# OFA-Sys/OFASys

Hardware: AMD Instinct MI355X
Metric: multimodal tokens/sec (enc+dec train step) (higher is better)
Workload: dtype bf16

## Files before the change

include/ofasys_amd.h:

```cpp
#ifndef OFASYS_AMD_H
#define OFASYS_AMD_H

#include <stdint.h>

#ifdef __cplusplus
extern "C" {
#endif

typedef enum { OFA_F32 = 0, OFA_BF16 = 1, OFA_F16 = 2 } ofa_dtype;

enum {
  OFA_OK = 0,
  OFA_ERR_INVALID = 1,
  OFA_ERR_UNSUPPORTED = 2,
  OFA_ERR_LAUNCH = 3
};

enum {
  OFA_GEMM_BIAS_COL = 1,
  OFA_GEMM_BIAS_ROW = 2,
  OFA_GEMM_ACCUM = 4,
  OFA_GEMM_FORCE_SIMPLE = 8,
  OFA_GEMM_OUT_F32 = 16,
  OFA_GEMM_A_KPAD_ZERO = 32,
  OFA_GEMM_NO_LDS_DMA = 64,
  OFA_GEMM_DEFER_REDUCE = 128
};

int ofa_version(void);
const char* ofa_last_error(void);

int ofa_layernorm_fwd(const void* x, const void* gamma, const void* beta, void* y, float* mean, float* rstd,
                      int64_t rows, int cols, float eps, int dtype, void* stream);
int ofa_layernorm_bwd_ws_rows(void);
int ofa_layernorm_bwd(const void* dy, const void* x, const void* gamma, const float* mean, const float* rstd,
                      const void* dres, void* dx, void* dgamma, void* dbeta, float* ws, int64_t rows, int cols,
                      int accumulate, int dtype, void* stream);
int ofa_gelu_layernorm_fwd(const void* h, const void* gamma, const void* beta, void* y, float* mean, float* rstd,
                           int64_t rows, int cols, float eps, int dtype, void* stream);
int ofa_gelu_layernorm_bwd(const void* dy, const void* h, const void* gamma, const float* mean, const float* rstd,
                           void* dh, void* dgamma, void* dbeta, void* dbias, float* ws, int64_t rows, int cols,
                           int accumulate, int dtype, void* stream);

int64_t ofa_join_keep_bytes(int64_t rows, int cols, int dtype);
int ofa_join_fwd(const void* x, const void* residual, const void* gamma_a, const void* beta_a, const void* gamma_b,
                 const void* beta_b, void* y, void* z, float* stats, uint8_t* keep_bits, int64_t rows, int cols, float eps, float p,
                 uint64_t seed, uint64_t offset, const int64_t* offset_base, int dtype, void* stream);
int ofa_join_bwd_slots(int64_t rows, int cols, int dtype);
int ofa_join_bwd(const void* dy, const void* dz, const void* x, const void* y, const void* gamma_a, const void* gamma_b,
                 const float* stats, const uint8_t* keep_bits, void* dres, void* dx, float* ws, int64_t rows, int cols, float p,
                 uint64_t seed, uint64_t offset, const int64_t* offset_base, int want_dx_colsum, int dtype, void* stream);

int ofa_gemm(const void* A, const void* B, void* C, const void* bias, int M, int N, int K, int transA, int transB,
             int64_t lda, int64_t ldb, int64_t ldc, int batch, int64_t strideA, int64_t strideB, int64_t strideC,
             int batch_inner, int64_t strideA2, int64_t strideB2, int64_t strideC2,
             float alpha, int flags, int dtype, void* ws, int64_t ws_bytes, void* stream);

int ofa_gemm_colstat(const void* A, const void* B, void* C, const void* bias, int M, int N, int K, int transA, int transB,
                     int64_t lda, int64_t ldb, int64_t ldc, float alpha, int flags, int dtype, void* ws, int64_t ws_bytes,
                     double* partial, int max_groups, int* groups, void* stream);

typedef struct ofa_gemm_group_item {
  const void* a;
  const void* b;
  float* slabs;
  int64_t lda, ldb;
  int32_t m, n, k;
  int32_t splits;
  void* out;
  int64_t ldo;
  float out_alpha;
} ofa_gemm_group_item;
int ofa_gemm_group_plan(ofa_gemm_group_item* items, int n, int dtype);
int ofa_gemm_group_tn(const ofa_gemm_group_item* items, int n, int dtype, void* stream);

int ofa_scaled_softmax_fwd(const void* x, void* y, float scale, int b, int np, int sq, int sk, int dtype, void* stream);
int ofa_scaled_softmax_bwd(const void* dy, const void* y, void* dx, float scale, int b, int np, int sq, int sk,
                           int dtype, void* stream);
int ofa_scaled_masked_softmax_fwd(const void* x, const uint8_t* mask, void* y, float scale, int b, int np, int sq,
                                  int sk, int mask_b, int dtype, void* stream);
int ofa_scaled_masked_softmax_bwd(const void* dy, const void* y, void* dx, float scale, int b, int np, int sq, int sk,
                                  int dtype, void* stream);
int ofa_scaled_upper_triang_masked_softmax_fwd(const void* x, void* y, float scale, int attn_batches, int sq,
                                               int dtype, void* stream);
int ofa_scaled_upper_triang_masked_softmax_bwd(const void* dy, const void* y, void* dx, float scale, int attn_batches,
                                               int sq, int dtype, void* stream);
int ofa_get_batch_per_block(int sq, int sk, int b, int np);

int ofa_attn_softmax_fwd(const void* x, const void* bias, const uint8_t* kpm, void* p, float scale, int BA, int heads,
                         int T, int S, int causal, int dtype, void* stream);

int ofa_attn_fwd(const void* q, const void* k, const void* v, const void* bias, const uint8_t* kpm,
                 const void* c_attn, int c_attn_dtype, void* out, float* lse, int B, int heads, int T, int S, int Tpad,
                 int64_t ldq, int64_t ldk, int64_t ldo, float scale, int causal, const int32_t* seg, int rows_q, int rows_k,
                 int dtype, void* stream);
int ofa_attn_bwd_prep(const void* dout, const void* out, float* delta, int B, int heads, int T, int Tpad, int64_t ldo,
                      int dtype, void* stream);
int ofa_attn_bwd(const void* q, const void* k, const void* v, const void* dout, const void* bias, const uint8_t* kpm,
                 const void* c_attn, int c_attn_dtype, const float* lse, float* delta, const void* out, void* dq, void* dk,
                 void* dv, void* dbias, int B, int heads, int T, int S, int Tpad, int64_t ldq, int64_t ldk, int64_t ldo,
                 float scale, int causal, const int32_t* seg, int rows_q, int rows_k, int dtype, void* stream);

int ofa_attn_cs_slots(int B, int rows);
int ofa_attn_bwd_cs(const void* q, const void* k, const void* v, const void* dout, const void* bias, const uint8_t* kpm,
                    const void* c_attn, int c_attn_dtype, const float* lse, float* delta, const void* out, void* dq, void* dk,
                    void* dv, void* dbias, int B, int heads, int T, int S, int Tpad, int64_t ldq, int64_t ldk, int64_t ldo,
                    float scale, int causal, const int32_t* seg, int rows_q, int rows_k, int dtype, float* cs_q, int64_t cs_ldq,
                    float* cs_k, float* cs_v, int64_t cs_ldk, float* cs_c, void* stream);

int ofa_attn_sbias_fwd(const void* q, const void* k, const void* v, const void* bias_swz_row, int Tb, int Sb, const uint8_t* kpm,
                       const void* c_attn, int c_attn_dtype, void* out, float* lse, int B, int heads, int T, int S, int Tpad,
                       int64_t ldq, int64_t ldk, int64_t ldo, float scale, int causal, const int32_t* seg, int rows_q, int rows_k,
                       int dtype, void* stream);
int ofa_attn_sbias_bwd(const void* q, const void* k, const void* v, const void* dout, const void* bias, const void* bias_swz_row,
                       const void* bias_swz_col, int Tb, int Sb, const uint8_t* kpm, const void* c_attn, int c_attn_dtype,
                       const float* lse, float* delta, const void* out, void* dq, void* dk, void* dv, void* dbias_sum, int dbias_dtype,
                       float* ws, int64_t ws_bytes, int B, int heads, int T, int S, int Tpad, int64_t ldq, int64_t ldk, int64_t ldo, float scale,
                       int causal, const int32_t* seg, int rows_q, int rows_k, int dtype, void* stream);
int ofa_attn_sbias_bwd_cs(const void* q, const void* k, const void* v, const void* dout, const void* bias, const void* bias_swz_row,
                          const void* bias_swz_col, int Tb, int Sb, const uint8_t* kpm, const void* c_attn, int c_attn_dtype,
                          const float* lse, float* delta, const void* out, void* dq, void* dk, void* dv, void* dbias_sum, int dbias_dtype,
                          float* ws, int64_t ws_bytes, int B, int heads, int T, int S, int Tpad, int64_t ldq, int64_t ldk, int64_t ldo, float scale,
                          int causal, const int32_t* seg, int rows_q, int rows_k, int dtype, float* cs_q, int64_t cs_ldq, float* cs_k,
                          float* cs_v, int64_t cs_ldk, float* cs_c, void* stream);
int ofa_attn_sbias_chunks(int B, int heads, int Tb, int Sb);
int ofa_c_attn_grad(const float* delta, const void* c_attn, void* dc, int B, int heads, int T, int64_t ld, int accumulate,
                    int c_attn_dtype, void* stream);
int ofa_attn_decode(const void* q, const void* k, const void* v, const void* bias, const uint8_t* kpm, const void* c_attn,
                    int c_attn_dtype, void* out, void* probs, int B, int heads, int head_dim, int S, int64_t ldk,
                    int64_t k_batch_stride, int64_t kpm_ld, float scale, int dtype, void* stream);
int ofa_mean_heads(const void* p, void* out, int B, int heads, int64_t n, int dtype, void* stream);
int ofa_transpose_heads(const void* x, void* xt, int B, int T, int C, int Tpad, int64_t ld, int dtype, void* stream);

int ofa_gather_rows(const void* src, const int64_t* index, void* out, int64_t n, int D, int64_t src_rows, int dtype,
                    void* stream);
int ofa_gather_rows_parts(const void* const* srcs, const int* lens, int nparts, const int64_t* index, void* out, int64_t n, int D,
                          int64_t batch, int dtype, void* stream);
int ofa_scatter_rows_part(const void* src, const int64_t* inverse, void* out, int64_t batch, int nk, int Ttot, int start, int D,
                          int64_t src_rows, int dtype, void* stream);
int ofa_embedding_fwd(const void* weight, const int64_t* ids, void* out, int64_t n, int D, int64_t V, uint8_t* is_pad, int64_t pad_id,
                      int dtype, void* stream);
int ofa_segment_rowsum(const void* dout, const int32_t* order, const int32_t* seg_off, const int32_t* seg_row, void* dweight, int nseg,
                       int D, int accumulate, int dtype, void* stream);
int ofa_embedding_bwd_slices(int64_t V, int D);
int ofa_embedding_bwd(const void* dout, const int64_t* ids, void* dweight, int64_t n, int D, int64_t V,
                      int64_t padding_idx, uint8_t* present_ws, float* slice_ws, int dtype, void* stream);

int ofa_gelu_fwd(const void* x, void* y, int64_t n, int dtype, void* stream);
int ofa_gelu_bwd(const void* dy, const void* x, void* dx, int64_t n, int dtype, void* stream);
int ofa_dropout_add_fwd(const void* x, const void* residual, void* y, int64_t n, float p, uint64_t seed,
                        uint64_t offset, const int64_t* offset_base, int dtype, void* stream);
int ofa_dropout_bwd(const void* dy, void* dx, int64_t n, float p, uint64_t seed, uint64_t offset,
                    const int64_t* offset_base, int dtype, void* stream);
int ofa_add_rowvec_mask(const void* a, const void* b, const void* vec, const uint8_t* rowmask, void* y, int64_t rows,
                        int cols, int64_t b_period, int dtype, void* stream);
int ofa_batch_sum(const void* x, void* out, int batch, int64_t n, int accumulate, int dtype, void* stream);

int ofa_colsum_ws_floats(int cols);
int ofa_colsum(const void* x, void* out, float* ws, int64_t rows, int cols, int64_t ld, float alpha, int accumulate,
               int dtype, int out_dtype, void* stream);

int ofa_add_n(const void* const* inputs, int n, void* out, int64_t numel, int dtype, void* stream);
int ofa_mul(const void* a, const void* b, void* y, int64_t rows, int cols, int b_rowvec, int dtype, void* stream);
int ofa_scale_row_groups(const void* x, const float* scale, void* y, int64_t rows, int cols, int64_t group, int dtype,
                         void* stream);
int ofa_reduce_sum_f32(const float* x, float* out, int64_t n, void* stream);
int ofa_head_sum_f32(const float* x, float* out, int B, int heads, int T, int ld, void* stream);

typedef struct ofa_bias_slots {
  const void* values[8];
  const void* values2[8];
  int32_t start[8];
  int32_t n[8];
  int32_t inner[8];
  int32_t count;
} ofa_bias_slots;
int64_t ofa_bias_swz_elems(int heads, int Tb, int Sb);
int ofa_bias_build(const void* abs_bias, const ofa_bias_slots* slots, void* out, void* swz_row, void* swz_col, int heads, int Tb,
                   int Sb, int dtype, void* stream);
int ofa_bias_outer_grad(const void* dbias, void* d_frames, void* d_patches, int heads, int T, int start, int F, int P, int dtype,
                        void* stream);
int ofa_bias_block_add(void* bias, const void* values, int B, int A, int T, int start, int n, int dtype, void* stream);
int ofa_bias_block_grad(const void* dbias, void* dvalues, int B, int A, int T, int start, int n, int dtype, void* stream);
int ofa_bias_block_add_batch(void* bias, const void* values, int B, int A, int T, int start, int n, int dtype, void* stream);
int ofa_bias_block_slice(const void* dbias, void* dvalues, int B, int A, int T, int start, int n, int dtype, void* stream);

int ofa_im2col_patch(const void* img, void* col, int B, int C, int H, int W, int p, int Kpad, int lead, int dtype, void* stream);

int ofa_cross_entropy_fwd(const void* logits, const int64_t* target, float* lse, float* row_loss, int64_t rows,
                          int64_t V, int64_t ld, int64_t ignore_index, int dtype, void* stream);
int ofa_cross_entropy_fwd_grad_ok(int64_t V, int64_t ld, int dtype);
int ofa_cross_entropy_fwd_grad(const void* logits, const int64_t* target, const float* grad_scale, float* lse, float* row_loss,
                               void* dlogits, int64_t rows, int64_t V, int64_t ld, int64_t ignore_index, int dtype, void* stream);
int ofa_cross_entropy_bwd(const void* logits, const int64_t* target, const float* lse, const float* grad_scale,
                          void* dlogits, int64_t rows, int64_t V, int64_t ld, int64_t ignore_index, int dtype,
                          void* stream);

int ofa_ls_cross_entropy_fwd(const void* logits, const int64_t* target, float* lse, float* row_loss, float* row_nll,
                             float* row_cnt, int64_t rows, int64_t V, int64_t ld, int64_t ignore_index, float eps,
                             int64_t cstart, int64_t cend, const uint8_t* cmask, int dtype, void* stream);
int ofa_ls_cross_entropy_bwd(const void* logits, const int64_t* target, const float* lse, const float* row_cnt,
                             const float* row_w, const float* grad_scale, void* dlogits, int64_t rows, int64_t V, int64_t ld,
                             int64_t ignore_index, float eps, int64_t cstart, int64_t cend, const uint8_t* cmask, int dtype,
                             void* stream);
int ofa_probs_fwd(const void* logits, float* out, int64_t rows, int64_t V, int64_t ld, int log_probs, int dtype,
                  void* stream);
int ofa_probs_bwd(const float* dy, const float* y, void* dlogits, int64_t rows, int64_t V, int64_t ld, int log_probs,
                  int dtype, void* stream);

int ofa_sumsq_ws_floats(void);
int ofa_sumsq(const void* x, float* out , float* ws ,
              int64_t n, int dtype, void* stream);
int ofa_step_schedule(const float* gsq, const double* sample_size, double* step, const double* lr, float* sched,
                      float* gnorm, float clip_norm, double beta1, double beta2, void* stream);
int ofa_step_stats_add(double* stats, const float* loss, const int64_t* target, int64_t n, int64_t pad, void* stream);
int ofa_step_schedule_scaled(const float* gsq, const double* sample_size, double* step, const double* lr, float* sched,
                             float* gnorm, double* loss_scaler, float clip_norm, double beta1, double beta2, double scale_factor,
                             double scale_window, double tolerance, double threshold, double min_loss_scale, void* stream);
int ofa_adam_step(float* master, float* exp_avg, float* exp_avg_sq, const void* grad, void* model_param,
                  const float* coef, int64_t n, float lr, float beta1, float beta2, float eps, float weight_decay,
                  int step, int dtype, void* stream);

int ofa_conv_out_size(int in, int k, int stride, int pad);
int ofa_im2col(const void* x, void* col, int B, int H, int W, int C, int KH, int KW, int stride, int pad, int Kpad,
               int x_nchw, int dtype, void* stream);
int ofa_col2im(const void* dcol, void* dx, int B, int H, int W, int C, int KH, int KW, int stride, int pad, int Kpad,
               int dtype, void* stream);
int ofa_batchnorm_ws_floats(int C);
int ofa_batchnorm_fwd(const void* x, const void* gamma, const void* beta, const void* residual, void* y, float* mean,
                      float* rstd, float* running_mean, float* running_var, float* ws, int64_t rows, int C, float eps,
                      float momentum, int use_running, int relu, int dtype, void* stream);
int ofa_batchnorm_bwd(const void* dy, const void* y, const void* x, const void* gamma, const float* mean, const float* rstd,
                      void* dx, void* dres, void* dgamma, void* dbeta, float* ws, int64_t rows, int C, int batch_stats,
                      int relu, int accumulate, const void* beta, int dtype, void* stream);
int ofa_batchnorm_fwd_stats(const void* x, double* sums, float* ws, int64_t rows, int C, int dtype, void* stream);
int ofa_batchnorm_fwd_apply(const void* x, const void* gamma, const void* beta, const void* residual, void* y, float* mean,
                            float* rstd, float* running_mean, float* running_var, const double* sums, int groups, int64_t rows,
                            int C, float eps, float momentum, int relu, int dtype, void* stream);
int ofa_batchnorm_bwd_stats(const void* dy, const void* y, const void* x, const void* gamma, const float* mean, const float* rstd,
                            float* sums, void* dgamma, void* dbeta, float* ws, int64_t rows, int C, int relu, int accumulate,
                            const void* beta, int dtype, void* stream);
int ofa_batchnorm_bwd_dx(const void* dy, const void* y, const void* x, const void* gamma, const float* mean, const float* rstd,
                         const float* sums, void* dx, void* dres, int64_t rows, const double* total_rows, int C, int relu,
                         const void* beta, int dtype, void* stream);
int ofa_maxpool_fwd(const void* x, void* y, uint8_t* arg, int B, int H, int W, int C, int K, int stride, int pad, int dtype,
                    void* stream);
int ofa_maxpool_bwd(const void* dy, const uint8_t* arg, void* dx, int B, int H, int W, int C, int K, int stride, int pad,
                    int dtype, void* stream);
int ofa_relu(const void* x, const void* gate, void* y, int64_t n, int dtype, void* stream);

typedef struct ofa_fold_job {
  const float* part;
  void* out;
  int64_t cols;
  int64_t stride;
  int32_t nslots;
  int32_t accumulate;
  float alpha;
  int32_t out_dtype;
} ofa_fold_job;
int ofa_fold_batched(const ofa_fold_job* jobs, int njobs, void* stream);
typedef struct ofa_copy_job {
  const void* src;
  void* dst;
  int64_t bytes;
} ofa_copy_job;
int ofa_copy_batched(const ofa_copy_job* jobs, int njobs, void* stream);
#define OFA_DEFER_FOLD 2
int ofa_layernorm_bwd_slots(int64_t rows, int cols, int dtype, int gelu);
int ofa_colsum_slots(int64_t rows);
int ofa_gemm_splits(int M, int N, int K, int transA, int transB, int batch, int flags, int dtype, int64_t ws_bytes);
enum {
  OFA_GEMM_PLAN_KERNEL = 0,
  OFA_GEMM_PLAN_SIMPLE_WHY,
  OFA_GEMM_PLAN_WAVES_M,
  OFA_GEMM_PLAN_WAVES_N,
  OFA_GEMM_PLAN_WAVE_TM,
  OFA_GEMM_PLAN_WAVE_TN,
  OFA_GEMM_PLAN_TILE_M,
  OFA_GEMM_PLAN_TILE_N,
  OFA_GEMM_PLAN_SPLITS,
  OFA_GEMM_PLAN_KSPLIT,
  OFA_GEMM_PLAN_K,
  OFA_GEMM_PLAN_MIXED_TALL,
  OFA_GEMM_PLAN_MIXED_SHORT,
  OFA_GEMM_PLAN_COLSTAT_ROWS,
  OFA_GEMM_PLAN_REDUCE,
  OFA_GEMM_PLAN_LEN
};
enum {
  OFA_GEMM_KERNEL_SIMPLE = 0,
  OFA_GEMM_KERNEL_REG = 1,
  OFA_GEMM_KERNEL_LDS_DMA = 2,
  OFA_GEMM_KERNEL_RING = 3,
  OFA_GEMM_KERNEL_BIG = 4,
  OFA_GEMM_KERNEL_PP = 5,
  OFA_GEMM_KERNEL_MIXED = 6
};
int ofa_gemm_plan(int M, int N, int K, int transA, int transB, int batch, int flags, int dtype, int64_t ws_bytes, int* plan);

int64_t ofa_beam_ws_bytes(int rows, int V, int K);
int ofa_beam_topk(const void* logits, int64_t ld, int rows, int V, int K, float temperature, int cstart, int cend, int step,
                  int min_len, int max_len, int pad, int unk, int eos, float unk_penalty, int ngram, const int64_t* tokens,
                  int64_t tok_ld, const int* done, void* ws, int dtype, void* stream);
int ofa_beam_select(const void* ws, int bsz, int K, int V, int step, int max_len, int eos, int unk, float unk_penalty,
                    int normalize, float len_penalty, int64_t* tokens, int64_t tok_ld, int tok_cap, float* scores,
                    int64_t score_ld, int* ignore, int* done, int* nfin, int64_t* reorder, int64_t* fin_tok, float* fin_pos,
                    int64_t fin_ld, float* fin_score, int* fin_len, int* fin_cnt, void* stream);

int64_t ofa_closed_set_ws_bytes(int bsz, int E, int N);
int ofa_closed_set_edge_logits(const void* h, int64_t ld_h, int dtype, const void* W, int64_t ld_w, const void* bias, int D, int V,
                               int bsz, int chunk, int T, int c0, const int* items, int n_items, const int* edge_token,
                               const int* rep_ans, const int* rep_pos, int N, int E, void* ws, void* stream);
int ofa_closed_set_reduce(int bsz, int C, int N, int E, int P, const int* node_edge_off, const int* edge_node, const int* path_off,
                          const int* path_edge, void* ws, float* scores, void* stream);
int ofa_closed_set_score(const void* h, int64_t ld_h, int dtype, const void* W, int64_t ld_w, const void* bias, int D, int V,
                         int bsz, int C, int Tmax, int N, int E, int P, const int* items, int n_items, const int* node_edge_off,
                         const int* edge_token, const int* edge_node, const int* rep_ans, const int* rep_pos, const int* path_off,
                         const int* path_edge, void* ws, float* scores, void* stream);

int ofa_trie_beam_splits(int max_degree, int V);
int ofa_trie_beam_topk(const void* h, int64_t ld_h, int dtype, const void* W, int64_t ld_w, const void* bias, int D, int V,
                       int rows, int K, const int* node, const int* node_edge_off, const int* edge_token, int N, int E,
                       int max_degree, float temperature, int step, int min_len, int max_len, int pad, int unk, int eos,
                       float unk_penalty, int ngram, const int64_t* tokens, int64_t tok_ld, const int* done, void* ws,
                       void* stream);
int ofa_trie_beam_advance(int* node, const int* node_edge_off, const int* edge_token, const int* edge_child, int N, int E,
                          int bsz, int K, int step, const int64_t* tokens, int64_t tok_ld, int tok_cap, const float* scores,
                          int64_t score_ld, const int* ignore, const int64_t* reorder, int* done, int* nfin, void* stream);

#ifdef __cplusplus
}
#endif
#endif
```

ofasys_amd/adaptor/image_patch_embed.py:

```python
from dataclasses import dataclass, field

import torch
import torch.nn as nn

from .. import ops
from ..configure import register_config
from ..module import Embedding
from ..preprocessor import Dictionary, ModalityType, Slot
from .base import AdaptorOutput, BaseAdaptor, BaseAdaptorConfig


@dataclass
class ImagePatchEmbedAdaptorConfig(BaseAdaptorConfig):
    image_size_width: int = 224
    image_size_height: int = 224
    patch_size_width: int = 14
    patch_size_height: int = 14
    embed_dim: int = 768
    add_cls_token: bool = True


@register_config("ofasys.adaptor", "image_patch_embed", ImagePatchEmbedAdaptorConfig)
class ImagePatchEmbedAdaptor(BaseAdaptor):
    pos_batch_invariant = True

    def __init__(self, embed_tokens: Embedding, dictionary: Dictionary, is_src: bool, general_adaptor,
                 cfg: ImagePatchEmbedAdaptorConfig):
        super().__init__(embed_tokens, dictionary, is_src, general_adaptor, cfg)
        image_size = (cfg.image_size_height, cfg.image_size_width)
        patch_size = (cfg.patch_size_height, cfg.patch_size_width)
        assert patch_size[0] == patch_size[1], "square patches only"
        num_patches = (image_size[1] // patch_size[1]) * (image_size[0] // patch_size[0])
        self.image_size, self.patch_size, self.num_patches = image_size, patch_size, num_patches
        self.embed_image_positions = Embedding(num_patches + 1 if cfg.add_cls_token else num_patches, cfg.embed_dim)
        if cfg.add_cls_token:
            self.cls_token = nn.Parameter(torch.zeros(1, 1, cfg.embed_dim))
        self.proj = nn.Conv2d(3, cfg.embed_dim, kernel_size=patch_size, stride=patch_size)

    def _ofa_plain_conv_weights(self):
        return (self.proj.weight,)

    def forward(self, slot: Slot, **kwargs) -> AdaptorOutput:
        assert slot.modality == ModalityType.IMAGE
        image: torch.Tensor = slot.value
        batch_size, _, height, width = image.shape
        assert height == self.image_size[0] and width == self.image_size[1], \
            f"Input image size ({height}*{width}) doesn't match model ({self.image_size[0]}*{self.image_size[1]})."
        x = ops.patch_embed(image, self.proj.weight, self.proj.bias, self.patch_size[0],
                            cls_token=self.cls_token if self.cfg.add_cls_token else None)
        n = x.size(1)
        mask = ops.cached_index(self, ("nomask", batch_size, n), lambda: torch.zeros((batch_size, n), dtype=torch.bool, device=image.device))
        pos = ops.cached_index(self, ("arange", n), lambda: torch.arange(n, dtype=torch.long, device=image.device).unsqueeze(0))
        return AdaptorOutput(x, mask, self.embed_image_positions(pos).expand(batch_size, -1, -1), None)
```

ofasys_amd/adaptor/text.py:

```python
import math
from dataclasses import dataclass, field
from typing import Any, Dict, Optional

import torch
import torch.nn as nn
from torch import Tensor

from .. import ops
from ..configure import register_config
from ..module import Embedding, OfaLinear
from ..preprocessor import Dictionary, Slot
from .base import AdaptorOutput, BaseAdaptor, BaseAdaptorConfig


def make_token_bucket_position(bucket_size, max_position):
    mid = bucket_size // 2
    dist = torch.arange(max_position, dtype=torch.long)
    band = torch.ceil(torch.log(dist.clamp_min(1) / mid) / math.log((max_position - 1) / mid) * (mid - 1)).long()
    magnitude = torch.where(dist <= mid, dist, mid + band)
    rel = dist[:, None] - dist[None, :]
    return torch.sign(rel) * magnitude[rel.abs()] + (bucket_size - 1)


@dataclass
class TextAdaptorConfig(BaseAdaptorConfig):
    token_bucket_size: int = field(default=256, metadata={"help": "token bucket size"})
    share_input_output_embed: bool = True
    output_embed_dim: Optional[int] = 512
    output_dim: Optional[int] = None
    output_bias: bool = False


@register_config("ofasys.adaptor", "text", TextAdaptorConfig)
class TextAdaptor(BaseAdaptor):
    pos_batch_invariant = True

    def __init__(self, embed_tokens: Embedding, dictionary: Dictionary, is_src: bool, general_adaptor,
                 cfg: TextAdaptorConfig):
        super().__init__(embed_tokens, dictionary, is_src, general_adaptor, cfg)
        self.embed_positions = Embedding(cfg.max_position + 2, cfg.embed_dim)
        token_num_rel_dis = 2 * cfg.token_bucket_size - 1
        token_rp_bucket = make_token_bucket_position(cfg.token_bucket_size, cfg.max_position)
        num_rel_pos_tables = 1 if self.cfg.share_attn_bias else self.num_layers
        self.token_rel_pos_table_list = nn.ModuleList(
            [Embedding(token_num_rel_dis, cfg.num_attention_heads, zero_init=True) for _ in range(num_rel_pos_tables)])
        self.register_buffer("token_rp_bucket", token_rp_bucket)
        self.share_input_output_embed = bool(cfg.share_input_output_embed)
        self.output_dim = cfg.output_dim if cfg.output_dim is not None else len(dictionary)
        self.output_embed_dim = cfg.output_embed_dim
        self.output_embed_bias = cfg.output_bias
        self.output_projection = None
        self.build_output_projection(dictionary)

    def build_output_projection(self, dictionary):
        if self.share_input_output_embed:
            self.output_projection = self.embed_tokens_T
        else:
            self.output_projection = OfaLinear(self.output_embed_dim, self.output_dim, bias=self.output_embed_bias)
            nn.init.normal_(self.output_projection.weight, mean=0, std=self.output_embed_dim ** -0.5)

    def get_rel_pos_bias(self, batch_size, seq_length, idx, **kwargs):
        if seq_length > self.token_rp_bucket.size(0):
            raise ValueError(f"sequence length {seq_length} exceeds the {self.token_rp_bucket.size(0)} positions of token_rp_bucket")
        rp_bucket = ops.cached_index(self, ("text", seq_length), lambda: self.token_rp_bucket[:seq_length, :seq_length].contiguous())
        return ops.embedding(rp_bucket, self.token_rel_pos_table_list[idx].weight, plan_key=("text", ops.owner_token(self)))

    def forward(self, slot: Slot, **kwargs) -> AdaptorOutput:
        src_tokens = slot.value
        bsz, seq_len = src_tokens.shape
        pad = self.dictionary.pad()
        if pad is not None and src_tokens.is_cuda:
            token_embedding, padding_masks = self.embed_tokens_and_pad_mask(src_tokens, pad)
        else:
            token_embedding = self.embed_tokens(src_tokens)
            padding_masks = src_tokens.eq(pad) if pad is not None else torch.zeros_like(src_tokens, dtype=torch.bool)
        positions = ops.cached_index(self, ("arange", seq_len), lambda: torch.arange(seq_len, device=src_tokens.device).unsqueeze(0))
        pos_embed = self.embed_positions(positions).expand(bsz, -1, -1)
        return AdaptorOutput(token_embedding, padding_masks, pos_embed, [])

    def forward_output(self, x: Tensor, extra: Dict[str, Any], slot: Slot, **kwargs):
        return self.output_projection(x), extra
```

ofasys_amd/csrc/elementwise.hip:

```cpp
#include "common.h"

namespace ofa {

template <typename T, bool BWD>
__global__ __launch_bounds__(256) void gelu_kernel(const T* __restrict__ dy, const T* __restrict__ x, T* __restrict__ y,
                                                   int64_t nvec, int64_t n) {
  constexpr int N = Vec<T>::N;
  for (int64_t v = (int64_t)blockIdx.x * 256 + threadIdx.x; v < nvec; v += (int64_t)gridDim.x * 256) {
    float a[N], g[N], o[N];
    load_vec<T>(x + v * N, a);
    if (BWD) load_vec<T>(dy + v * N, g);
#pragma unroll
    for (int j = 0; j < N; ++j) o[j] = BWD ? g[j] * gelu_grad_f(a[j]) : gelu_f(a[j]);
    store_vec<T>(y + v * N, o);
  }
  if (blockIdx.x == 0) {
    for (int64_t e = nvec * N + threadIdx.x; e < n; e += 256) {
      const float a = ld1<T>(x + e);
      st1<T>(y + e, BWD ? ld1<T>(dy + e) * gelu_grad_f(a) : gelu_f(a));
    }
  }
}

template <typename T, bool ADD>
__global__ __launch_bounds__(256) void dropout_kernel(const T* __restrict__ x, const T* __restrict__ res, T* __restrict__ y,
                                                      int64_t n, float p, uint64_t seed, uint64_t offset,
                                                      const int64_t* __restrict__ offset_base) {
  if (offset_base) offset += (uint64_t)offset_base[0];
  const Philox rng(seed);
  const float keep_scale = 1.0f / (1.0f - p);
  const uint32_t thresh = philox_thresh(p);
  const int64_t nq = (n + 7) / 8;
  for (int64_t q = (int64_t)blockIdx.x * 256 + threadIdx.x; q < nq; q += (int64_t)gridDim.x * 256) {
    const uint4 r = rng(offset + (uint64_t)q);
#pragma unroll
    for (int j = 0; j < 8; ++j) {
      const int64_t e = q * 8 + j;
      if (e < n) {
        float v = philox_keep(r, j, thresh) ? ld1<T>(x + e) * keep_scale : 0.f;
        if (ADD) v += ld1<T>(res + e);
        st1<T>(y + e, v);
      }
    }
  }
}

template <typename T>
__global__ __launch_bounds__(256) void add_rowvec_mask_kernel(const T* __restrict__ a, const T* __restrict__ b,
                                                              const T* __restrict__ vec, const uint8_t* __restrict__ rowmask,
                                                              T* __restrict__ y, int64_t rows, int cols, int64_t b_period) {
  constexpr int N = Vec<T>::N;
  const int vpr = cols / N;
  const int64_t total = rows * vpr;
  for (int64_t v = (int64_t)blockIdx.x * 256 + threadIdx.x; v < total; v += (int64_t)gridDim.x * 256) {
    const int64_t r = v / vpr;
    const int c = (int)(v % vpr) * N;
    float x[N], t[N];
    load_vec<T>(a + r * cols + c, x);
    if (b) {
      load_vec<T>(b + (b_period ? r % b_period : r) * cols + c, t);
#pragma unroll
      for (int j = 0; j < N; ++j) x[j] += t[j];
    }
    if (vec) {
      load_vec<T>(vec + c, t);
#pragma unroll
      for (int j = 0; j < N; ++j) x[j] += t[j];
    }
    if (rowmask && rowmask[r]) {
#pragma unroll
      for (int j = 0; j < N; ++j) x[j] = 0.f;
    }
    store_vec<T>(y + r * cols + c, x);
  }
}

template <typename T>
__global__ __launch_bounds__(256) void embedding_fwd_kernel(const T* __restrict__ w, const int64_t* __restrict__ ids,
                                                            T* __restrict__ out, int64_t n, int D, int64_t V,
                                                            uint8_t* __restrict__ is_pad, int64_t pad_id) {
  constexpr int N = Vec<T>::N;
  const int vpr = D / N;
  const int64_t total = n * vpr;
  for (int64_t v = (int64_t)blockIdx.x * 256 + threadIdx.x; v < total; v += (int64_t)gridDim.x * 256) {
    const int64_t r = v / vpr;
    const int c = (int)(v % vpr) * N;
    int64_t id = ids[r];
    if (is_pad && c == 0) is_pad[r] = id == pad_id;
    id = id < 0 ? 0 : (id >= V ? V - 1 : id);
    *reinterpret_cast<typename Vec<T>::type*>(out + r * D + c) =
        *reinterpret_cast<const typename Vec<T>::type*>(w + id * D + c);
  }
}

template <typename T>
__global__ __launch_bounds__(256) void gather_rows_kernel(const T* __restrict__ src, const int64_t* __restrict__ index,
                                                          T* __restrict__ out, int64_t n, int D, int64_t src_rows) {
  constexpr int N = Vec<T>::N;
  const int vpr = D / N;
  const int64_t total = n * vpr;
  for (int64_t v = (int64_t)blockIdx.x * 256 + threadIdx.x; v < total; v += (int64_t)gridDim.x * 256) {
    const int64_t r = v / vpr;
    const int c = (int)(v % vpr) * N;
    const int64_t id = index[r];
    typename Vec<T>::type val = {};
    if (id >= 0 && id < src_rows) val = *reinterpret_cast<const typename Vec<T>::type*>(src + id * D + c);
    *reinterpret_cast<typename Vec<T>::type*>(out + r * D + c) = val;
  }
}

struct GatherParts { const void* src[8]; int start[9]; int n; };
template <typename T>
__global__ __launch_bounds__(256) void gather_rows_parts_kernel(GatherParts gp, const int64_t* __restrict__ index, T* __restrict__ out,
                                                                int64_t n, int D, int Ttot, int64_t batch) {
  constexpr int N = Vec<T>::N;
  const int vpr = D / N;
  const int64_t total = n * vpr;
  for (int64_t v = (int64_t)blockIdx.x * 256 + threadIdx.x; v < total; v += (int64_t)gridDim.x * 256) {
    const int64_t r = v / vpr;
    const int c = (int)(v % vpr) * N;
    const int64_t id = index[r];
    typename Vec<T>::type val = {};
    if (id >= 0 && id < batch * Ttot) {
      const int64_t b = id / Ttot;
      const int t = (int)(id - b * Ttot);
      int k = 0;
#pragma unroll
      for (int q = 1; q < 8; ++q)
        if (q < gp.n && t >= gp.start[q]) k = q;
      const int nk = gp.start[k + 1] - gp.start[k];
      val = *reinterpret_cast<const typename Vec<T>::type*>((const T*)gp.src[k] + ((b * nk + (t - gp.start[k])) * D + c));
    }
    *reinterpret_cast<typename Vec<T>::type*>(out + r * D + c) = val;
  }
}

template <typename T>
__global__ __launch_bounds__(256) void scatter_rows_part_kernel(const T* __restrict__ src, const int64_t* __restrict__ inverse,
                                                                T* __restrict__ out, int64_t batch, int nk, int Ttot, int start, int D,
                                                                int64_t src_rows) {
  constexpr int N = Vec<T>::N;
  const int vpr = D / N;
  const int64_t total = batch * nk * vpr;
  for (int64_t v = (int64_t)blockIdx.x * 256 + threadIdx.x; v < total; v += (int64_t)gridDim.x * 256) {
    const int64_t r = v / vpr;
    const int c = (int)(v % vpr) * N;
    const int64_t b = r / nk;
    const int j = (int)(r - b * nk);
    const int64_t id = inverse[b * Ttot + start + j];
    typename Vec<T>::type val = {};
    if (id >= 0 && id < src_rows) val = *reinterpret_cast<const typename Vec<T>::type*>(src + id * D + c);
    *reinterpret_cast<typename Vec<T>::type*>(out + r * D + c) = val;
  }
}

template <typename T>
__global__ __launch_bounds__(256) void embedding_fwd_scalar_kernel(const T* __restrict__ w, const int64_t* __restrict__ ids,
                                                                   T* __restrict__ out, int64_t n, int D, int64_t V) {
  const int64_t total = n * D;
  for (int64_t e = (int64_t)blockIdx.x * 256 + threadIdx.x; e < total; e += (int64_t)gridDim.x * 256) {
    const int64_t r = e / D;
    const int c = (int)(e % D);
    int64_t id = ids[r];
    id = id < 0 ? 0 : (id >= V ? V - 1 : id);
    out[e] = w[id * D + c];
  }
}

__global__ __launch_bounds__(256) void embedding_mark_kernel(const int64_t* __restrict__ ids, uint8_t* __restrict__ present,
                                                             int64_t n, int64_t V) {
  for (int64_t i = (int64_t)blockIdx.x * 256 + threadIdx.x; i < n; i += (int64_t)gridDim.x * 256) {
    const int64_t id = ids[i];
    if (id >= 0 && id < V) present[id] = 1;
  }
}

template <typename T, int NV>
__global__ __launch_bounds__(256) void embedding_bwd_kernel(const T* __restrict__ dout, const int64_t* __restrict__ ids,
                                                            T* __restrict__ dw, float* __restrict__ part, int64_t n, int D,
                                                            int64_t V, int64_t padding_idx,
                                                            const uint8_t* __restrict__ present, int S) {
  constexpr int N = Vec<T>::N;
  const int lane = threadIdx.x & 63;
  const int64_t v = (int64_t)blockIdx.x * 4 + (threadIdx.x >> 6);
  const int sl = blockIdx.y;
  if (v >= V || v == padding_idx) return;
  if (present && !present[v]) return;
  float acc[NV][N];
#pragma unroll
  for (int i = 0; i < NV; ++i)
#pragma unroll
    for (int j = 0; j < N; ++j) acc[i][j] = 0.f;
  const int64_t per = ((n + S - 1) / S + 63) / 64 * 64;
  const int64_t lo = sl * per, hi = lo + per < n ? lo + per : n;
  bool any = false;
  for (int64_t base = lo; base < hi; base += 64) {
    const int64_t idx = base + lane;
    const bool hit = idx < hi && ids[idx] == v;
    unsigned long long m = __ballot(hit);
    while (m) {
      const int src = __ffsll((long long)m) - 1;
      m &= m - 1;
      any = true;
      const T* row = dout + (base + src) * D;
#pragma unroll
      for (int i = 0; i < NV; ++i) {
        const int c = (i * 64 + lane) * N;
        if (c < D) {
          float x[N];
          load_vec<T>(row + c, x);
#pragma unroll
          for (int j = 0; j < N; ++j) acc[i][j] += x[j];
        }
      }
    }
  }
  if (S == 1) {
    if (!any) return;
    T* wr = dw + v * D;
#pragma unroll
    for (int i = 0; i < NV; ++i) {
      const int c = (i * 64 + lane) * N;
      if (c < D) {
        float o[N];
        load_vec<T>(wr + c, o);
#pragma unroll
        for (int j = 0; j < N; ++j) o[j] += acc[i][j];
        store_vec<T>(wr + c, o);
      }
    }
  } else {
    float* pr = part + ((int64_t)sl * V + v) * D;
#pragma unroll
    for (int i = 0; i < NV; ++i) {
      const int c = (i * 64 + lane) * N;
      if (c < D)
#pragma unroll
        for (int j = 0; j < N; ++j) pr[c + j] = acc[i][j];
    }
  }
}

template <typename T>
__global__ __launch_bounds__(256) void embedding_bwd_scalar_kernel(const T* __restrict__ dout, const int64_t* __restrict__ ids,
                                                                   T* __restrict__ dw, float* __restrict__ part, int64_t n,
                                                                   int D, int64_t V, int64_t padding_idx,
                                                                   const uint8_t* __restrict__ present, int S) {
  const int lane = threadIdx.x & 63;
  const int64_t v = (int64_t)blockIdx.x * 4 + (threadIdx.x >> 6);
  const int sl = blockIdx.y;
  if (v >= V || v == padding_idx) return;
  if (present && !present[v]) return;
  constexpr int MAXC = 32;
  float acc[MAXC];
#pragma unroll
  for (int j = 0; j < MAXC; ++j) acc[j] = 0.f;
  const int64_t per = ((n + S - 1) / S + 63) / 64 * 64;
  const int64_t lo = sl * per, hi = lo + per < n ? lo + per : n;
  bool any = false;
  for (int64_t base = lo; base < hi; base += 64) {
    const int64_t idx = base + lane;
    const bool hit = idx < hi && ids[idx] == v;
    unsigned long long m = __ballot(hit);
    while (m) {
      const int src = __ffsll((long long)m) - 1;
      m &= m - 1;
      any = true;
      const T* row = dout + (base + src) * D;
#pragma unroll
      for (int j = 0; j < MAXC; ++j) {
        const int c = j * 64 + lane;
        if (c < D) acc[j] += ld1<T>(row + c);
      }
    }
  }
  if (S == 1 && !any) return;
#pragma unroll
  for (int j = 0; j < MAXC; ++j) {
    const int c = j * 64 + lane;
    if (c < D) {
      if (S == 1) st1<T>(dw + v * D + c, ld1<T>(dw + v * D + c) + acc[j]);
      else part[((int64_t)sl * V + v) * D + c] = acc[j];
    }
  }
}

template <typename T>
__global__ __launch_bounds__(256) void embedding_fold_kernel(const float* __restrict__ part, T* __restrict__ dw, int D,
                                                             int64_t V, int64_t padding_idx,
                                                             const uint8_t* __restrict__ present, int S) {
  const int64_t v = blockIdx.x;
  if (v == padding_idx || (present && !present[v])) return;
  for (int c = threadIdx.x; c < D; c += 256) {
    float a = 0.f;
    for (int s = 0; s < S; ++s) a += part[((int64_t)s * V + v) * D + c];
    st1<T>(dw + v * D + c, ld1<T>(dw + v * D + c) + a);
  }
}

template <typename T>
__global__ __launch_bounds__(256) void im2col_patch_kernel(const T* __restrict__ img, T* __restrict__ col, int B, int C, int H,
                                                           int W, int p, int Kpad, int lead) {
  const int nph = H / p, npw = W / p, K = C * p * p;
  const int64_t per = (int64_t)lead + (int64_t)nph * npw;
  const int64_t total = (int64_t)B * per * Kpad;
  for (int64_t e = (int64_t)blockIdx.x * 256 + threadIdx.x; e < total; e += (int64_t)gridDim.x * 256) {
    const int k = (int)(e % Kpad);
    const int64_t r = e / Kpad;
    const int64_t b = r / per, rs = r % per - lead;
    float v = 0.f;
    if (k < K && rs >= 0) {
      const int j = k % p, i = (k / p) % p, c = k / (p * p);
      const int pw = (int)(rs % npw), ph = (int)(rs / npw);
      v = ld1<T>(img + ((b * C + c) * H + ph * p + i) * W + pw * p + j);
    }
    st1<T>(col + e, v);
  }
}

template <typename T>
__global__ __launch_bounds__(256) void colsum_partial_kernel(const T* __restrict__ x, float* __restrict__ partial,
                                                             int64_t rows, int cols, int64_t ld) {
  constexpr int N = Vec<T>::N;
  __shared__ float red[8][32][N];
  const int cx = threadIdx.x & 31, ry = threadIdx.x >> 5;
  const int c = (blockIdx.x * 32 + cx) * N;
  float acc[N];
#pragma unroll
  for (int j = 0; j < N; ++j) acc[j] = 0.f;
  if (c < cols) {
    for (int64_t r = (int64_t)blockIdx.y * 8 + ry; r < rows; r += (int64_t)gridDim.y * 8) {
      float v[N];
      load_vec<T>(x + r * ld + c, v);
#pragma unroll
      for (int j = 0; j < N; ++j) acc[j] += v[j];
    }
  }
#pragma unroll
  for (int j = 0; j < N; ++j) red[ry][cx][j] = acc[j];
  __syncthreads();
  if (ry == 0 && c < cols) {
#pragma unroll
    for (int j = 0; j < N; ++j) {
      float t = 0.f;
#pragma unroll
      for (int r = 0; r < 8; ++r) t += red[r][cx][j];
      partial[(int64_t)blockIdx.y * cols + c + j] = t;
    }
  }
}
template <typename TO>
__global__ __launch_bounds__(1024) void colsum_final_kernel(const float* __restrict__ partial, TO* __restrict__ out,
                                                            int cols, int groups, float alpha, int accumulate) {
  __shared__ float sm[16][64];
  const int cx = threadIdx.x & 63, ry = threadIdx.x >> 6;
  const int c = blockIdx.x * 64 + cx;
  float s = 0.f;
  if (c < cols)
    for (int g = ry; g < groups; g += 16) s += partial[(int64_t)g * cols + c];
  sm[ry][cx] = s;
  __syncthreads();
  if (ry == 0 && c < cols) {
    float t = 0.f;
#pragma unroll
    for (int r = 0; r < 16; ++r) t += sm[r][cx];
    t *= alpha;
    if (accumulate) t += ld1<TO>(out + c);
    st1<TO>(out + c, t);
  }
}

static inline int grid_for(int64_t work) {
  int64_t g = (work + 255) / 256;
  return (int)(g < 1 ? 1 : (g > 2048 ? 2048 : g));
}

}
using namespace ofa;

#define OFA_DT_CHECK(name) OFA_REQUIRE(OFA_DT_OK(dtype), OFA_ERR_INVALID, name ": bad dtype %d", dtype)

extern "C" int ofa_gelu_fwd(const void* x, void* y, int64_t n, int dtype, void* stream) {
  OFA_DT_CHECK("gelu_fwd");
  OFA_REQUIRE(n >= 0 && (n == 0 || (x && y)), OFA_ERR_INVALID, "gelu_fwd: bad argument");
  if (n == 0) return 0;
  hipStream_t st = (hipStream_t)stream;
  if (dtype == OFA_F32)
    hipLaunchKernelGGL((gelu_kernel<float, false>), dim3(grid_for(n / 4)), dim3(256), 0, st, (const float*)nullptr,
                       (const float*)x, (float*)y, n / 4, n);
  else if (dtype == OFA_BF16)
    hipLaunchKernelGGL((gelu_kernel<bf16_t, false>), dim3(grid_for(n / 8)), dim3(256), 0, st, (const bf16_t*)nullptr,
                       (const bf16_t*)x, (bf16_t*)y, n / 8, n);
  else
    hipLaunchKernelGGL((gelu_kernel<f16_t, false>), dim3(grid_for(n / 8)), dim3(256), 0, st, (const f16_t*)nullptr,
                       (const f16_t*)x, (f16_t*)y, n / 8, n);
  return check_launch("gelu_fwd");
}

extern "C" int ofa_gelu_bwd(const void* dy, const void* x, void* dx, int64_t n, int dtype, void* stream) {
  OFA_DT_CHECK("gelu_bwd");
  OFA_REQUIRE(n >= 0 && (n == 0 || (dy && x && dx)), OFA_ERR_INVALID, "gelu_bwd: bad argument");
  if (n == 0) return 0;
  hipStream_t st = (hipStream_t)stream;
  if (dtype == OFA_F32)
    hipLaunchKernelGGL((gelu_kernel<float, true>), dim3(grid_for(n / 4)), dim3(256), 0, st, (const float*)dy,
                       (const float*)x, (float*)dx, n / 4, n);
  else if (dtype == OFA_BF16)
    hipLaunchKernelGGL((gelu_kernel<bf16_t, true>), dim3(grid_for(n / 8)), dim3(256), 0, st, (const bf16_t*)dy,
                       (const bf16_t*)x, (bf16_t*)dx, n / 8, n);
  else
    hipLaunchKernelGGL((gelu_kernel<f16_t, true>), dim3(grid_for(n / 8)), dim3(256), 0, st, (const f16_t*)dy,
                       (const f16_t*)x, (f16_t*)dx, n / 8, n);
  return check_launch("gelu_bwd");
}

extern "C" int ofa_dropout_add_fwd(const void* x, const void* residual, void* y, int64_t n, float p, uint64_t seed,
                                   uint64_t offset, const int64_t* offset_base, int dtype, void* stream) {
  OFA_DT_CHECK("dropout_add_fwd");
  OFA_REQUIRE(n >= 0 && p >= 0.f && p < 1.f && (n == 0 || (x && y)), OFA_ERR_INVALID, "dropout_add_fwd: bad argument");
  if (n == 0) return 0;
  hipStream_t st = (hipStream_t)stream;
  dim3 grid(grid_for((n + 7) / 8)), block(256);
  if (dtype == OFA_F32) {
    if (residual) hipLaunchKernelGGL((dropout_kernel<float, true>), grid, block, 0, st, (const float*)x, (const float*)residual, (float*)y, n, p, seed, offset, offset_base);
    else hipLaunchKernelGGL((dropout_kernel<float, false>), grid, block, 0, st, (const float*)x, (const float*)nullptr, (float*)y, n, p, seed, offset, offset_base);
  } else if (dtype == OFA_BF16) {
    if (residual) hipLaunchKernelGGL((dropout_kernel<bf16_t, true>), grid, block, 0, st, (const bf16_t*)x, (const bf16_t*)residual, (bf16_t*)y, n, p, seed, offset, offset_base);
    else hipLaunchKernelGGL((dropout_kernel<bf16_t, false>), grid, block, 0, st, (const bf16_t*)x, (const bf16_t*)nullptr, (bf16_t*)y, n, p, seed, offset, offset_base);
  }
  else {
    if (residual) hipLaunchKernelGGL((dropout_kernel<f16_t, true>), grid, block, 0, st, (const f16_t*)x, (const f16_t*)residual, (f16_t*)y, n, p, seed, offset, offset_base);
    else hipLaunchKernelGGL((dropout_kernel<f16_t, false>), grid, block, 0, st, (const f16_t*)x, (const f16_t*)nullptr, (f16_t*)y, n, p, seed, offset, offset_base);
  }
  return check_launch("dropout_add_fwd");
}

extern "C" int ofa_dropout_bwd(const void* dy, void* dx, int64_t n, float p, uint64_t seed, uint64_t offset,
                               const int64_t* offset_base, int dtype, void* stream) {
  return ofa_dropout_add_fwd(dy, nullptr, dx, n, p, seed, offset, offset_base, dtype, stream);
}

extern "C" int ofa_add_rowvec_mask(const void* a, const void* b, const void* vec, const uint8_t* rowmask, void* y,
                                   int64_t rows, int cols, int64_t b_period, int dtype, void* stream) {
  OFA_DT_CHECK("add_rowvec_mask");
  OFA_REQUIRE(rows >= 0 && cols > 0 && a && y && b_period >= 0, OFA_ERR_INVALID, "add_rowvec_mask: bad argument");
  OFA_REQUIRE(cols % (dtype == OFA_F32 ? 4 : 8) == 0, OFA_ERR_UNSUPPORTED, "add_rowvec_mask: cols=%d not vectorizable", cols);
  if (rows == 0) return 0;
  hipStream_t st = (hipStream_t)stream;
  if (dtype == OFA_F32)
    hipLaunchKernelGGL((add_rowvec_mask_kernel<float>), dim3(grid_for(rows * cols / 4)), dim3(256), 0, st, (const float*)a,
                       (const float*)b, (const float*)vec, rowmask, (float*)y, rows, cols, b_period);
  else if (dtype == OFA_BF16)
    hipLaunchKernelGGL((add_rowvec_mask_kernel<bf16_t>), dim3(grid_for(rows * cols / 8)), dim3(256), 0, st,
                       (const bf16_t*)a, (const bf16_t*)b, (const bf16_t*)vec, rowmask, (bf16_t*)y, rows, cols, b_period);
  else
    hipLaunchKernelGGL((add_rowvec_mask_kernel<f16_t>), dim3(grid_for(rows * cols / 8)), dim3(256), 0, st,
                       (const f16_t*)a, (const f16_t*)b, (const f16_t*)vec, rowmask, (f16_t*)y, rows, cols, b_period);
  return check_launch("add_rowvec_mask");
}

extern "C" int ofa_embedding_fwd(const void* weight, const int64_t* ids, void* out, int64_t n, int D, int64_t V, uint8_t* is_pad,
                                 int64_t pad_id, int dtype, void* stream) {
  OFA_DT_CHECK("embedding_fwd");
  OFA_REQUIRE(!is_pad || D % (dtype == OFA_F32 ? 4 : 8) == 0, OFA_ERR_UNSUPPORTED, "embedding_fwd: the pad mask rides with the vector kernel (D = %d)", D);
  OFA_REQUIRE(n >= 0 && D > 0 && V > 0 && weight && ids && out, OFA_ERR_INVALID, "embedding_fwd: bad argument");
  if (n == 0) return 0;
  hipStream_t st = (hipStream_t)stream;
  if (D % (dtype == OFA_F32 ? 4 : 8) != 0) {
    if (dtype == OFA_F32)
// ... 54 lines not shown
      gp.start[k + 1] = gp.start[k] + lens[k];
    } else {
      gp.start[k + 1] = gp.start[k];
    }
  }
  const int Ttot = gp.start[nparts];
  hipStream_t st = (hipStream_t)stream;
  if (dtype == OFA_F32)
    hipLaunchKernelGGL((gather_rows_parts_kernel<float>), dim3(grid_for(n * D / 4)), dim3(256), 0, st, gp, index, (float*)out, n, D, Ttot, batch);
  else if (dtype == OFA_BF16)
    hipLaunchKernelGGL((gather_rows_parts_kernel<bf16_t>), dim3(grid_for(n * D / 8)), dim3(256), 0, st, gp, index, (bf16_t*)out, n, D, Ttot, batch);
  else
    hipLaunchKernelGGL((gather_rows_parts_kernel<f16_t>), dim3(grid_for(n * D / 8)), dim3(256), 0, st, gp, index, (f16_t*)out, n, D, Ttot, batch);
  return check_launch("gather_rows_parts");
}

extern "C" int ofa_scatter_rows_part(const void* src, const int64_t* inverse, void* out, int64_t batch, int nk, int Ttot, int start, int D,
                                     int64_t src_rows, int dtype, void* stream) {
  OFA_DT_CHECK("scatter_rows_part");
  OFA_REQUIRE(src && inverse && out && batch > 0 && nk > 0 && start >= 0 && start + nk <= Ttot && D > 0 && src_rows > 0, OFA_ERR_INVALID,
              "scatter_rows_part: bad argument");
  OFA_REQUIRE(D % (dtype == OFA_F32 ? 4 : 8) == 0, OFA_ERR_UNSUPPORTED, "scatter_rows_part: D=%d not vectorizable", D);
  hipStream_t st = (hipStream_t)stream;
  const int64_t work = batch * nk * D / (dtype == OFA_F32 ? 4 : 8);
  if (dtype == OFA_F32)
    hipLaunchKernelGGL((scatter_rows_part_kernel<float>), dim3(grid_for(work)), dim3(256), 0, st, (const float*)src, inverse, (float*)out, batch, nk, Ttot, start, D, src_rows);
  else if (dtype == OFA_BF16)
    hipLaunchKernelGGL((scatter_rows_part_kernel<bf16_t>), dim3(grid_for(work)), dim3(256), 0, st, (const bf16_t*)src, inverse, (bf16_t*)out, batch, nk, Ttot, start, D, src_rows);
  else
    hipLaunchKernelGGL((scatter_rows_part_kernel<f16_t>), dim3(grid_for(work)), dim3(256), 0, st, (const f16_t*)src, inverse, (f16_t*)out, batch, nk, Ttot, start, D, src_rows);
  return check_launch("scatter_rows_part");
}

template <typename T, int CPL>
__global__ __launch_bounds__(256) void segment_rowsum_kernel(const T* __restrict__ dout, const int* __restrict__ order,
                                                             const int* __restrict__ seg_off, const int* __restrict__ seg_row,
                                                             T* __restrict__ dw, int nseg, int D, int accumulate) {
  const int lane = threadIdx.x & 63;
  const int sg = blockIdx.x * 4 + (threadIdx.x >> 6);
  if (sg >= nseg) return;
  constexpr int G = 64 / CPL;
  const int g = lane / CPL, c = lane % CPL;
  const int lo = seg_off[sg], hi = seg_off[sg + 1];
  float acc = 0.f;
  int p = lo + g;
  for (; p + 3 * G < hi; p += 4 * G) {
    const int64_t r0 = order[p], r1 = order[p + G], r2 = order[p + 2 * G], r3 = order[p + 3 * G];
    float v0 = 0.f, v1 = 0.f, v2 = 0.f, v3 = 0.f;
    if (c < D) {
      v0 = ld1<T>(dout + r0 * D + c);
      v1 = ld1<T>(dout + r1 * D + c);
      v2 = ld1<T>(dout + r2 * D + c);
      v3 = ld1<T>(dout + r3 * D + c);
    }
    acc += (v0 + v1) + (v2 + v3);
  }
  for (; p < hi; p += G) {
    const int64_t row = order[p];
    if (c < D) acc += ld1<T>(dout + row * D + c);
  }
#pragma unroll
  for (int off = CPL; off < 64; off <<= 1) acc += __shfl_xor(acc, off);
  if (g == 0 && c < D) {
    T* o = dw + (int64_t)seg_row[sg] * D + c;
    st1<T>(o, (accumulate ? ld1<T>(o) : 0.f) + acc);
  }
}

extern "C" int ofa_embedding_bwd_slices(int64_t V, int D) {
  if (V <= 0 || D <= 0) return 1;
  const int64_t by_rows = 8192 / V;
  const int64_t by_bytes = ((int64_t)1 << 21) / (V * D);
  int64_t s = by_rows > by_bytes ? by_rows : by_bytes;
  return (int)(s < 1 ? 1 : (s > 64 ? 64 : s));
}

template <typename T>
static void launch_segment_rowsum(const void* dout, const int32_t* order, const int32_t* seg_off, const int32_t* seg_row, void* dw, int nseg,
                                  int D, int accumulate, hipStream_t st) {
  const dim3 grid(cdiv(nseg, 4)), block(256);
  if (D <= 8) hipLaunchKernelGGL((segment_rowsum_kernel<T, 8>), grid, block, 0, st, (const T*)dout, order, seg_off, seg_row, (T*)dw, nseg, D, accumulate);
  else if (D <= 16) hipLaunchKernelGGL((segment_rowsum_kernel<T, 16>), grid, block, 0, st, (const T*)dout, order, seg_off, seg_row, (T*)dw, nseg, D, accumulate);
  else if (D <= 32) hipLaunchKernelGGL((segment_rowsum_kernel<T, 32>), grid, block, 0, st, (const T*)dout, order, seg_off, seg_row, (T*)dw, nseg, D, accumulate);
  else hipLaunchKernelGGL((segment_rowsum_kernel<T, 64>), grid, block, 0, st, (const T*)dout, order, seg_off, seg_row, (T*)dw, nseg, D, accumulate);
}

extern "C" int ofa_segment_rowsum(const void* dout, const int32_t* order, const int32_t* seg_off, const int32_t* seg_row, void* dweight,
                                  int nseg, int D, int accumulate, int dtype, void* stream) {
  OFA_DT_CHECK("segment_rowsum");
  OFA_REQUIRE(dout && order && seg_off && seg_row && dweight && nseg >= 0 && D > 0 && D <= 64, OFA_ERR_INVALID,
              "segment_rowsum: bad argument (D = %d, at most 64 columns)", D);
  if (nseg == 0) return 0;
  hipStream_t st = (hipStream_t)stream;
  if (dtype == OFA_F32) launch_segment_rowsum<float>(dout, order, seg_off, seg_row, dweight, nseg, D, accumulate, st);
  else if (dtype == OFA_BF16) launch_segment_rowsum<bf16_t>(dout, order, seg_off, seg_row, dweight, nseg, D, accumulate, st);
  else launch_segment_rowsum<f16_t>(dout, order, seg_off, seg_row, dweight, nseg, D, accumulate, st);
  return check_launch("segment_rowsum");
}

extern "C" int ofa_embedding_bwd(const void* dout, const int64_t* ids, void* dweight, int64_t n, int D, int64_t V,
                                 int64_t padding_idx, uint8_t* present_ws, float* slice_ws, int dtype, void* stream) {
  OFA_DT_CHECK("embedding_bwd");
  OFA_REQUIRE(n >= 0 && D > 0 && V > 0 && dout && ids && dweight, OFA_ERR_INVALID, "embedding_bwd: bad argument");
  const int vecn = dtype == OFA_F32 ? 4 : 8;
  OFA_REQUIRE(D <= 2048, OFA_ERR_UNSUPPORTED, "embedding_bwd: D=%d exceeds 2048", D);
  const bool vec_ok = D % vecn == 0 && D <= 64 * vecn * 4 && (((uintptr_t)dout | (uintptr_t)dweight) & 15) == 0;
  if (n == 0) return 0;
  hipStream_t st = (hipStream_t)stream;
  if (present_ws) {
    (void)hipMemsetAsync(present_ws, 0, (size_t)V, st);
    hipLaunchKernelGGL(embedding_mark_kernel, dim3(grid_for(n)), dim3(256), 0, st, ids, present_ws, n, V);
  }
  const int S = slice_ws ? ofa_embedding_bwd_slices(V, D) : 1;
  const int nv = cdiv(D, 64 * vecn);
  dim3 grid((unsigned)((V + 3) / 4), S), block(256);
#define EMB_LAUNCH(T, NV)                                                                                               \
  hipLaunchKernelGGL((embedding_bwd_kernel<T, NV>), grid, block, 0, st, (const T*)dout, ids, (T*)dweight, slice_ws, n, D, V, \
                     padding_idx, (const uint8_t*)present_ws, S)
#define EMB_CASE(T)                  \
  do {                               \
    if (nv <= 1) EMB_LAUNCH(T, 1);   \
    else if (nv <= 2) EMB_LAUNCH(T, 2); \
    else EMB_LAUNCH(T, 4);           \
  } while (0)
  if (!vec_ok) {
    if (dtype == OFA_F32)
      hipLaunchKernelGGL((embedding_bwd_scalar_kernel<float>), grid, block, 0, st, (const float*)dout, ids, (float*)dweight,
                         slice_ws, n, D, V, padding_idx, (const uint8_t*)present_ws, S);
    else if (dtype == OFA_BF16)
      hipLaunchKernelGGL((embedding_bwd_scalar_kernel<bf16_t>), grid, block, 0, st, (const bf16_t*)dout, ids,
                         (bf16_t*)dweight, slice_ws, n, D, V, padding_idx, (const uint8_t*)present_ws, S);
    else
      hipLaunchKernelGGL((embedding_bwd_scalar_kernel<f16_t>), grid, block, 0, st, (const f16_t*)dout, ids,
                         (f16_t*)dweight, slice_ws, n, D, V, padding_idx, (const uint8_t*)present_ws, S);
  } else if (dtype == OFA_F32) EMB_CASE(float);
  else if (dtype == OFA_BF16) EMB_CASE(bf16_t);
         else EMB_CASE(f16_t);
#undef EMB_CASE
#undef EMB_LAUNCH
  int rc = check_launch("embedding_bwd");
  if (rc || S == 1) return rc;
  if (dtype == OFA_F32)
    hipLaunchKernelGGL((embedding_fold_kernel<float>), dim3((unsigned)V), dim3(256), 0, st, slice_ws, (float*)dweight, D, V,
                       padding_idx, (const uint8_t*)present_ws, S);
  else if (dtype == OFA_BF16)
    hipLaunchKernelGGL((embedding_fold_kernel<bf16_t>), dim3((unsigned)V), dim3(256), 0, st, slice_ws, (bf16_t*)dweight, D, V,
                       padding_idx, (const uint8_t*)present_ws, S);
  else
    hipLaunchKernelGGL((embedding_fold_kernel<f16_t>), dim3((unsigned)V), dim3(256), 0, st, slice_ws, (f16_t*)dweight, D, V,
                       padding_idx, (const uint8_t*)present_ws, S);
  return check_launch("embedding_fold");
}

extern "C" int ofa_im2col_patch(const void* img, void* col, int B, int C, int H, int W, int p, int Kpad, int lead, int dtype,
                                void* stream) {
  OFA_DT_CHECK("im2col_patch");
  OFA_REQUIRE(img && col && B > 0 && C > 0 && p > 0 && H % p == 0 && W % p == 0 && Kpad >= C * p * p && lead >= 0, OFA_ERR_INVALID,
              "im2col_patch: bad argument (H=%d W=%d p=%d Kpad=%d)", H, W, p, Kpad);
  hipStream_t st = (hipStream_t)stream;
  const int64_t total = (int64_t)B * (lead + (int64_t)(H / p) * (W / p)) * Kpad;
  if (dtype == OFA_F32)
    hipLaunchKernelGGL((im2col_patch_kernel<float>), dim3(grid_for(total)), dim3(256), 0, st, (const float*)img, (float*)col,
                       B, C, H, W, p, Kpad, lead);
  else if (dtype == OFA_BF16)
    hipLaunchKernelGGL((im2col_patch_kernel<bf16_t>), dim3(grid_for(total)), dim3(256), 0, st, (const bf16_t*)img,
                       (bf16_t*)col, B, C, H, W, p, Kpad, lead);
  else
    hipLaunchKernelGGL((im2col_patch_kernel<f16_t>), dim3(grid_for(total)), dim3(256), 0, st, (const f16_t*)img,
                       (f16_t*)col, B, C, H, W, p, Kpad, lead);
  return check_launch("im2col_patch");
}

extern "C" int ofa_colsum_ws_floats(int cols) { return 128 * cols; }

extern "C" int ofa_colsum_slots(int64_t rows) {
  int64_t groups = (rows + 63) / 64;
  return (int)(groups < 1 ? 1 : (groups > 128 ? 128 : groups));
}

extern "C" int ofa_colsum(const void* x, void* out, float* ws, int64_t rows, int cols, int64_t ld, float alpha,
                          int accumulate, int dtype, int out_dtype, void* stream) {
  OFA_DT_CHECK("colsum");
  OFA_REQUIRE(OFA_DT_OK(out_dtype), OFA_ERR_INVALID, "colsum: bad out dtype %d", out_dtype);
  OFA_REQUIRE(rows >= 0 && cols > 0 && ld >= cols && x && (out || accumulate == OFA_DEFER_FOLD) && ws, OFA_ERR_INVALID,
              "colsum: bad argument");
  const int n = dtype == OFA_F32 ? 4 : 8;
  OFA_REQUIRE(cols % n == 0 && ld % n == 0, OFA_ERR_UNSUPPORTED, "colsum: cols=%d / ld not vectorizable", cols);
  hipStream_t st = (hipStream_t)stream;
  const int groups = ofa_colsum_slots(rows);
  dim3 grid(cdiv(cols / n, 32), groups), block(256);
  if (dtype == OFA_F32)
    hipLaunchKernelGGL((colsum_partial_kernel<float>), grid, block, 0, st, (const float*)x, ws, rows, cols, ld);
  else if (dtype == OFA_BF16)
    hipLaunchKernelGGL((colsum_partial_kernel<bf16_t>), grid, block, 0, st, (const bf16_t*)x, ws, rows, cols, ld);
  else
    hipLaunchKernelGGL((colsum_partial_kernel<f16_t>), grid, block, 0, st, (const f16_t*)x, ws, rows, cols, ld);
  int rc = check_launch("colsum_partial");
  if (rc || accumulate == OFA_DEFER_FOLD) return rc;
  if (out_dtype == OFA_F32)
    hipLaunchKernelGGL((colsum_final_kernel<float>), dim3(cdiv(cols, 64)), dim3(1024), 0, st, (const float*)ws, (float*)out,
                       cols, groups, alpha, accumulate);
  else if (out_dtype == OFA_BF16)
    hipLaunchKernelGGL((colsum_final_kernel<bf16_t>), dim3(cdiv(cols, 64)), dim3(1024), 0, st, (const float*)ws,
                       (bf16_t*)out, cols, groups, alpha, accumulate);
  else
    hipLaunchKernelGGL((colsum_final_kernel<f16_t>), dim3(cdiv(cols, 64)), dim3(1024), 0, st, (const float*)ws,
                       (f16_t*)out, cols, groups, alpha, accumulate);
  return check_launch("colsum_final");
}

namespace ofa {
template <typename T>
__global__ __launch_bounds__(256) void mul_kernel(const T* __restrict__ a, const T* __restrict__ b, T* __restrict__ y,
                                                  int64_t rows, int cols, int b_rowvec) {
  constexpr int N = Vec<T>::N;
  const int vpr = cols / N;
  const int64_t total = rows * vpr;
  for (int64_t v = (int64_t)blockIdx.x * 256 + threadIdx.x; v < total; v += (int64_t)gridDim.x * 256) {
    const int64_t r = v / vpr;
    const int c = (int)(v % vpr) * N;
    float x[N], t[N];
    load_vec<T>(a + r * cols + c, x);
    load_vec<T>(b_rowvec ? b + c : b + r * cols + c, t);
#pragma unroll
    for (int j = 0; j < N; ++j) x[j] *= t[j];
    store_vec<T>(y + r * cols + c, x);
  }
}
template <typename T>
__global__ __launch_bounds__(256) void scale_row_groups_kernel(const T* __restrict__ x, const float* __restrict__ scale,
                                                               T* __restrict__ y, int64_t rows, int cols, int64_t group) {
  constexpr int N = Vec<T>::N;
  const int vpr = cols / N;
  const int64_t total = rows * vpr;
  for (int64_t v = (int64_t)blockIdx.x * 256 + threadIdx.x; v < total; v += (int64_t)gridDim.x * 256) {
    const int64_t r = v / vpr;
    const int c = (int)(v % vpr) * N;
    const float s = scale[r / group];
    float a[N];
    load_vec<T>(x + r * cols + c, a);
#pragma unroll
    for (int j = 0; j < N; ++j) a[j] *= s;
    store_vec<T>(y + r * cols + c, a);
  }
}
__global__ __launch_bounds__(256) void reduce_sum_f32_kernel(const float* __restrict__ x, float* __restrict__ out, int64_t n) {
  __shared__ float sw[4];
  float s = 0.f;
  for (int64_t i = threadIdx.x; i < n; i += 256) s += x[i];
  s = wave_sum(s);
  if ((threadIdx.x & 63) == 0) sw[threadIdx.x >> 6] = s;
  __syncthreads();
  if (threadIdx.x == 0) out[0] = sw[0] + sw[1] + sw[2] + sw[3];
}
__global__ __launch_bounds__(256) void head_sum_kernel(const float* __restrict__ x, float* __restrict__ out, int B, int heads,
                                                       int T, int ld) {
  __shared__ float sw[4];
  const int h = blockIdx.x;
  float s = 0.f;
  for (int b = 0; b < B; ++b)
    for (int t = threadIdx.x; t < T; t += 256) s += x[((int64_t)b * heads + h) * ld + t];
  s = wave_sum(s);
  if ((threadIdx.x & 63) == 0) sw[threadIdx.x >> 6] = s;
  __syncthreads();
  if (threadIdx.x == 0) out[h] = sw[0] + sw[1] + sw[2] + sw[3];
}
struct AddNArgs { const void* in[16]; int n; };
template <typename T>
__global__ __launch_bounds__(256) void add_n_kernel(AddNArgs a, T* __restrict__ out, int64_t numel) {
  constexpr int N = Vec<T>::N;
  const int64_t nvec = numel / N;
  for (int64_t v = (int64_t)blockIdx.x * 256 + threadIdx.x; v < nvec; v += (int64_t)gridDim.x * 256) {
    float acc[N];
#pragma unroll
    for (int j = 0; j < N; ++j) acc[j] = 0.f;
    for (int k = 0; k < a.n; ++k) {
      float t[N];
      load_vec<T>((const T*)a.in[k] + v * N, t);
#pragma unroll
      for (int j = 0; j < N; ++j) acc[j] += t[j];
    }
    store_vec<T>(out + v * N, acc);
  }
  if (blockIdx.x == 0) {
    for (int64_t i = nvec * N + threadIdx.x; i < numel; i += 256) {
      float t = 0.f;
      for (int k = 0; k < a.n; ++k) t += ld1<T>((const T*)a.in[k] + i);
      st1<T>(out + i, t);
    }
  }
}
}

extern "C" int ofa_add_n(const void* const* inputs, int n, void* out, int64_t numel, int dtype, void* stream) {
  OFA_DT_CHECK("add_n");
  OFA_REQUIRE(inputs && out && n >= 1 && n <= 16 && numel >= 0, OFA_ERR_INVALID, "add_n: 1..16 inputs (got %d)", n);
  if (numel == 0) return 0;
  AddNArgs a;
  for (int k = 0; k < 16; ++k) a.in[k] = inputs[k < n ? k : 0];
  for (int k = 0; k < n; ++k) OFA_REQUIRE(inputs[k] && !((uintptr_t)inputs[k] & 15), OFA_ERR_INVALID, "add_n: input %d is NULL or not 16-byte aligned", k);
  OFA_REQUIRE(!((uintptr_t)out & 15), OFA_ERR_INVALID, "add_n: out is not 16-byte aligned");
  a.n = n;
  hipStream_t st = (hipStream_t)stream;
  const int64_t work = numel / (dtype == OFA_F32 ? 4 : 8) + 1;
  if (dtype == OFA_F32) hipLaunchKernelGGL((add_n_kernel<float>), dim3(grid_for(work)), dim3(256), 0, st, a, (float*)out, numel);
  else if (dtype == OFA_BF16) hipLaunchKernelGGL((add_n_kernel<bf16_t>), dim3(grid_for(work)), dim3(256), 0, st, a, (bf16_t*)out, numel);
  else hipLaunchKernelGGL((add_n_kernel<f16_t>), dim3(grid_for(work)), dim3(256), 0, st, a, (f16_t*)out, numel);
  return check_launch("add_n");
}

template <typename T>
__global__ __launch_bounds__(256) void batch_sum_kernel(const T* __restrict__ x, T* __restrict__ out, int batch, int64_t n, int accumulate) {
  constexpr int N = Vec<T>::N;
// ... 70 lines not shown
```

ofasys_amd/csrc/fold.hip:

```cpp
#include "common.h"

namespace ofa {

constexpr int FOLD_MAX_JOBS = 56;

struct FoldJobs {
  const float* part[FOLD_MAX_JOBS];
  void* out[FOLD_MAX_JOBS];
  int64_t cols[FOLD_MAX_JOBS];
  int64_t stride[FOLD_MAX_JOBS];
  float alpha[FOLD_MAX_JOBS];
  int nslots[FOLD_MAX_JOBS];
  unsigned block0[FOLD_MAX_JOBS + 1];
  unsigned char flags[FOLD_MAX_JOBS];
  int njobs;
};

__device__ __forceinline__ void fold_store(const FoldJobs& J, int j, int64_t c, int64_t cols, const float (&t)[4]) {
  const float alpha = J.alpha[j];
  const bool acc = J.flags[j] & 1, f32 = J.flags[j] & 2, f16 = J.flags[j] & 8;
  if (c + 4 <= cols && (cols & 3) == 0) {
    if (f32) {
      float4* o = reinterpret_cast<float4*>((float*)J.out[j] + c);
      float4 v = make_float4(t[0] * alpha, t[1] * alpha, t[2] * alpha, t[3] * alpha);
      if (acc) { const float4 u = *o; v.x += u.x; v.y += u.y; v.z += u.z; v.w += u.w; }
      *o = v;
    } else if (f16) {
      uint2* o = reinterpret_cast<uint2*>((f16_t*)J.out[j] + c);
      float v[4] = {t[0] * alpha, t[1] * alpha, t[2] * alpha, t[3] * alpha};
      if (acc) {
        const uint2 u = *o;
        const f16x2_t a = __builtin_bit_cast(f16x2_t, u.x), b = __builtin_bit_cast(f16x2_t, u.y);
        v[0] += (float)a[0]; v[1] += (float)a[1]; v[2] += (float)b[0]; v[3] += (float)b[1];
      }
      uint2 w;
      w.x = pack_f16x2(v[0], v[1]);
      w.y = pack_f16x2(v[2], v[3]);
      *o = w;
    } else {
      uint2* o = reinterpret_cast<uint2*>((bf16_t*)J.out[j] + c);
      float v[4] = {t[0] * alpha, t[1] * alpha, t[2] * alpha, t[3] * alpha};
      if (acc) {
        const uint2 u = *o;
        v[0] += __uint_as_float(u.x << 16); v[1] += __uint_as_float(u.x & 0xffff0000u);
        v[2] += __uint_as_float(u.y << 16); v[3] += __uint_as_float(u.y & 0xffff0000u);
      }
      uint2 w;
      w.x = pack_bf16x2(v[0], v[1]);
      w.y = pack_bf16x2(v[2], v[3]);
      *o = w;
    }
    return;
  }
#pragma unroll
  for (int e = 0; e < 4; ++e) {
    if (c + e >= cols) break;
    const float v = t[e] * alpha;
    if (f32) {
      float* o = (float*)J.out[j] + c + e;
      *o = acc ? *o + v : v;
    } else if (f16) {
      f16_t* o = (f16_t*)J.out[j] + c + e;
      *o = (f16_t)(acc ? (float)*o + v : v);
    } else {
      bf16_t* o = (bf16_t*)J.out[j] + c + e;
      *o = f2bf(acc ? bf2f(*o) + v : v);
    }
  }
}

__global__ __launch_bounds__(256) void fold_batched_kernel(FoldJobs J) {
  __shared__ float4 red[8][32];
  int j = 0;
  while (j + 1 < J.njobs && blockIdx.x >= J.block0[j + 1]) ++j;
  const int64_t chunk = blockIdx.x - J.block0[j];
  const int64_t cols = J.cols[j], stride = J.stride[j];
  const float* __restrict__ p = J.part[j];
  const int ns = J.nslots[j];
  const bool vec = (cols & 3) == 0 && (stride & 3) == 0;
  if (J.flags[j] & 4) {
    const int64_t c = chunk * 1024 + threadIdx.x * 4;
    if (c >= cols) return;
    float t[4] = {0.f, 0.f, 0.f, 0.f};
    if (vec) {
      const float* r = p + c;
      int s = 0;
      for (; s + 4 <= ns; s += 4) {
        const float4 v0 = *reinterpret_cast<const float4*>(r + (int64_t)s * stride);
        const float4 v1 = *reinterpret_cast<const float4*>(r + (int64_t)(s + 1) * stride);
        const float4 v2 = *reinterpret_cast<const float4*>(r + (int64_t)(s + 2) * stride);
        const float4 v3 = *reinterpret_cast<const float4*>(r + (int64_t)(s + 3) * stride);
        t[0] = (((t[0] + v0.x) + v1.x) + v2.x) + v3.x;
        t[1] = (((t[1] + v0.y) + v1.y) + v2.y) + v3.y;
        t[2] = (((t[2] + v0.z) + v1.z) + v2.z) + v3.z;
        t[3] = (((t[3] + v0.w) + v1.w) + v2.w) + v3.w;
      }
      if (s < ns) {
        const int rem = ns - s;
        const float4 v0 = *reinterpret_cast<const float4*>(r + (int64_t)s * stride);
        const float4 v1 = *reinterpret_cast<const float4*>(r + (int64_t)(rem > 1 ? s + 1 : s) * stride);
        const float4 v2 = *reinterpret_cast<const float4*>(r + (int64_t)(rem > 2 ? s + 2 : s) * stride);
        t[0] += v0.x; t[1] += v0.y; t[2] += v0.z; t[3] += v0.w;
        if (rem > 1) { t[0] += v1.x; t[1] += v1.y; t[2] += v1.z; t[3] += v1.w; }
        if (rem > 2) { t[0] += v2.x; t[1] += v2.y; t[2] += v2.z; t[3] += v2.w; }
      }
    } else {
      for (int s = 0; s < ns; ++s)
        for (int e = 0; e < 4 && c + e < cols; ++e) t[e] += p[(int64_t)s * stride + c + e];
    }
    fold_store(J, j, c, cols, t);
    return;
  }
  const int q = threadIdx.x & 31, sl = threadIdx.x >> 5;
  const int64_t c = chunk * 128 + q * 4;
  float4 a = make_float4(0.f, 0.f, 0.f, 0.f);
  if (c < cols) {
    if (vec) {
      const float* r = p + c;
      int s = sl;
      for (; s + 24 < ns; s += 32) {
        const float4 v0 = *reinterpret_cast<const float4*>(r + (int64_t)s * stride);
        const float4 v1 = *reinterpret_cast<const float4*>(r + (int64_t)(s + 8) * stride);
        const float4 v2 = *reinterpret_cast<const float4*>(r + (int64_t)(s + 16) * stride);
        const float4 v3 = *reinterpret_cast<const float4*>(r + (int64_t)(s + 24) * stride);
        a.x = (((a.x + v0.x) + v1.x) + v2.x) + v3.x;
        a.y = (((a.y + v0.y) + v1.y) + v2.y) + v3.y;
        a.z = (((a.z + v0.z) + v1.z) + v2.z) + v3.z;
        a.w = (((a.w + v0.w) + v1.w) + v2.w) + v3.w;
      }
      for (; s < ns; s += 8) {
        const float4 v = *reinterpret_cast<const float4*>(r + (int64_t)s * stride);
        a.x += v.x; a.y += v.y; a.z += v.z; a.w += v.w;
      }
    } else {
      for (int s = sl; s < ns; s += 8) {
        const float* r = p + (int64_t)s * stride + c;
        a.x += r[0];
        if (c + 1 < cols) a.y += r[1];
        if (c + 2 < cols) a.z += r[2];
        if (c + 3 < cols) a.w += r[3];
      }
    }
  }
  red[sl][q] = a;
  __syncthreads();
  if (sl == 0 && c < cols) {
    float t[4] = {0.f, 0.f, 0.f, 0.f};
#pragma unroll
    for (int r = 0; r < 8; ++r) {
      t[0] += red[r][q].x; t[1] += red[r][q].y; t[2] += red[r][q].z; t[3] += red[r][q].w;
    }
    fold_store(J, j, c, cols, t);
  }
}

constexpr int COPY_MAX_JOBS = 96;
constexpr int COPY_CHUNK = 32768;
struct CopyJobs {
  const unsigned char* src[COPY_MAX_JOBS];
  unsigned char* dst[COPY_MAX_JOBS];
  int64_t bytes[COPY_MAX_JOBS];
  unsigned block0[COPY_MAX_JOBS + 1];
  int njobs;
};

__global__ __launch_bounds__(256) void copy_batched_kernel(CopyJobs J) {
  int lo = 0, hi = J.njobs - 1;
  while (lo < hi) {
    const int mid = (lo + hi + 1) >> 1;
    if (J.block0[mid] <= blockIdx.x) lo = mid; else hi = mid - 1;
  }
  const int64_t off = (int64_t)(blockIdx.x - J.block0[lo]) * COPY_CHUNK;
  const int64_t left = J.bytes[lo] - off;
  const int n = (int)(left < COPY_CHUNK ? left : COPY_CHUNK);
  const unsigned char* s = J.src[lo] + off;
  unsigned char* d = J.dst[lo] + off;
  if ((((uintptr_t)s | (uintptr_t)d) & 15) == 0) {
    const int nv = n >> 4;
    for (int i = threadIdx.x; i < nv; i += 256) reinterpret_cast<uint4*>(d)[i] = reinterpret_cast<const uint4*>(s)[i];
    for (int i = (nv << 4) + threadIdx.x; i < n; i += 256) d[i] = s[i];
  } else {
    for (int i = threadIdx.x; i < n; i += 256) d[i] = s[i];
  }
}

}
using namespace ofa;

extern "C" int ofa_copy_batched(const ofa_copy_job* jobs, int njobs, void* stream) {
  OFA_REQUIRE(njobs >= 0 && (njobs == 0 || jobs), OFA_ERR_INVALID, "copy_batched: bad argument");
  hipStream_t st = (hipStream_t)stream;
  for (int base = 0; base < njobs; base += COPY_MAX_JOBS) {
    CopyJobs J;
    const int n = njobs - base < COPY_MAX_JOBS ? njobs - base : COPY_MAX_JOBS;
    int m = 0;
    unsigned blocks = 0;
    for (int i = 0; i < n; ++i) {
      const ofa_copy_job& b = jobs[base + i];
      OFA_REQUIRE(b.bytes >= 0 && (b.bytes == 0 || (b.src && b.dst)), OFA_ERR_INVALID, "copy_batched: bad job %d", base + i);
      if (b.bytes == 0) continue;
      J.src[m] = (const unsigned char*)b.src; J.dst[m] = (unsigned char*)b.dst; J.bytes[m] = b.bytes;
      J.block0[m] = blocks;
      blocks += (unsigned)((b.bytes + COPY_CHUNK - 1) / COPY_CHUNK);
      ++m;
    }
    if (m == 0) continue;
    J.block0[m] = blocks;
    J.njobs = m;
    hipLaunchKernelGGL(copy_batched_kernel, dim3(blocks), dim3(256), 0, st, J);
    int rc = check_launch("copy_batched");
    if (rc) return rc;
  }
  return 0;
}

extern "C" int ofa_fold_batched(const ofa_fold_job* jobs, int njobs, void* stream) {
  OFA_REQUIRE(njobs >= 0 && (njobs == 0 || jobs), OFA_ERR_INVALID, "fold_batched: bad argument");
  hipStream_t st = (hipStream_t)stream;
  for (int base = 0; base < njobs; base += FOLD_MAX_JOBS) {
    FoldJobs J;
    const int n = njobs - base < FOLD_MAX_JOBS ? njobs - base : FOLD_MAX_JOBS;
    J.njobs = n;
    unsigned blocks = 0;
    for (int i = 0; i < n; ++i) {
      const ofa_fold_job& b = jobs[base + i];
      OFA_REQUIRE(b.part && b.out && b.cols > 0 && b.nslots > 0 && b.stride >= b.cols, OFA_ERR_INVALID, "fold_batched: bad job %d", base + i);
      OFA_REQUIRE(OFA_DT_OK(b.out_dtype), OFA_ERR_INVALID, "fold_batched: bad out dtype %d", b.out_dtype);
      J.part[i] = b.part; J.out[i] = b.out; J.cols[i] = b.cols; J.stride[i] = b.stride; J.alpha[i] = b.alpha;
      J.nslots[i] = b.nslots;
      const bool wide = b.nslots <= 16;
      J.flags[i] = (unsigned char)((b.accumulate ? 1 : 0) | (b.out_dtype == OFA_F32 ? 2 : 0) | (wide ? 4 : 0) | (b.out_dtype == OFA_F16 ? 8 : 0));
      J.block0[i] = blocks;
      blocks += (unsigned)(wide ? (b.cols + 1023) / 1024 : (b.cols + 127) / 128);
    }
    J.block0[n] = blocks;
    if (blocks == 0) continue;
    hipLaunchKernelGGL(fold_batched_kernel, dim3(blocks), dim3(256), 0, st, J);
    int rc = check_launch("fold_batched");
    if (rc) return rc;
  }
  return 0;
}
```

ofasys_amd/kernels.py:

```python
import contextlib
import ctypes

import torch

from .lib import (BF16, F32, GEMM_ACCUM, GEMM_BIAS_COL, GEMM_BIAS_ROW, GEMM_FORCE_SIMPLE, GEMM_OUT_F32, OfaError,
                  dptr, dtype_code, lib, ptr, stream)

_ws_cache = {}


def workspace(nbytes, device, tag="ws"):
    key = (tag, device, torch.cuda.current_stream().cuda_stream if device.type == "cuda" else 0)
    buf = _ws_cache.get(key)
    n = (nbytes + 3) // 4
    if buf is None or buf.numel() < n:
        buf = torch.empty(max(n, 1 << 20), dtype=torch.float32, device=device)
        _ws_cache[key] = buf
    return buf


@contextlib.contextmanager
def capture_workspaces(cache):
    global _ws_cache
    saved, _ws_cache = _ws_cache, dict(cache)
    added = {}
    try:
        yield added
    finally:
        added.update({k: v for k, v in _ws_cache.items() if cache.get(k) is not v})
        cache.update(added)
        _ws_cache = saved


class _FoldJob(ctypes.Structure):
    _fields_ = [("part", ctypes.c_void_p), ("out", ctypes.c_void_p), ("cols", ctypes.c_int64), ("stride", ctypes.c_int64),
                ("nslots", ctypes.c_int32), ("accumulate", ctypes.c_int32), ("alpha", ctypes.c_float),
                ("out_dtype", ctypes.c_int32)]


class _CopyJob(ctypes.Structure):
    _fields_ = [("src", ctypes.c_void_p), ("dst", ctypes.c_void_p), ("bytes", ctypes.c_int64)]


def copy_batched(pairs):
    jobs = []
    for dst, src in pairs:
        if (src.dtype == dst.dtype and src.shape == dst.shape and src.device == dst.device and dst.is_cuda
                and src.is_contiguous() and dst.is_contiguous()):
            jobs.append((dptr(src), dptr(dst), src.numel() * src.element_size()))
        else:
            dst.copy_(src, non_blocking=True)
    if jobs:
        arr = (_CopyJob * len(jobs))()
        for it, (s_, d_, n) in zip(arr, jobs):
            it.src, it.dst, it.bytes = s_, d_, n
        lib().call("ofa_copy_batched", ctypes.addressof(arr), len(jobs), stream())


DEFER_FOLD = 2
GEMM_DEFER_REDUCE = 128


class FoldQueue:

    MAX_PENDING_BYTES = 48 << 20

    def __init__(self):
        self.jobs, self.keep, self.bytes, self.outs, self.want_flush = [], [], 0, set(), False

    def add(self, part, part_off, out, cols, stride, nslots, alpha=1.0, accumulate=True, flush_ok=True):
        assert part.dtype == torch.float32 and out.is_contiguous()
        if out.data_ptr() in self.outs:
            self.flush()
        self.outs.add(out.data_ptr())
        self.jobs.append(_FoldJob(dptr(part) + part_off * 4, dptr(out), cols, stride, nslots, int(accumulate),
                                  float(alpha), dtype_code(out)))
        self.keep.append((part, out))
        self.bytes += nslots * stride * 4
        self.want_flush = self.bytes > self.MAX_PENDING_BYTES

    def flush_if_large(self):
        if getattr(self, "want_flush", False):
            self.flush()

    def flush(self):
        if not self.jobs:
            return
        arr = (_FoldJob * len(self.jobs))(*self.jobs)
        lib().call("ofa_fold_batched", ctypes.addressof(arr), len(self.jobs), stream())
        self.jobs, self.keep, self.bytes, self.want_flush = [], [], 0, False
        self.outs = set()


class ImmediateFold:

    def add(self, part, part_off, out, cols, stride, nslots, alpha=1.0, accumulate=True, flush_ok=True):
        assert part.dtype == torch.float32 and out.is_contiguous()
        job = (_FoldJob * 1)(_FoldJob(dptr(part) + part_off * 4, dptr(out), cols, stride, nslots, int(accumulate), float(alpha),
                                      dtype_code(out)))
        lib().call("ofa_fold_batched", ctypes.addressof(job), 1, stream())

    def flush_if_large(self):
        pass


def _u8(mask):
    mask = mask.contiguous()
    return mask.view(torch.uint8) if mask.dtype == torch.bool else mask.to(torch.uint8)


def _rows_cols(x):
    cols = x.shape[-1]
    return x.numel() // cols, cols


def layernorm_fwd(x, gamma, beta, eps=1e-5, fuse_gelu=False):
    x = x.contiguous()
    rows, cols = _rows_cols(x)
    y = torch.empty_like(x)
    mean = torch.empty(rows, dtype=torch.float32, device=x.device)
    rstd = torch.empty(rows, dtype=torch.float32, device=x.device)
    lib().call("ofa_gelu_layernorm_fwd" if fuse_gelu else "ofa_layernorm_fwd", ptr(x), ptr(gamma), ptr(beta), ptr(y),
               ptr(mean), ptr(rstd), rows, cols, eps, dtype_code(x), stream())
    return y, mean, rstd


def layernorm_bwd(dy, x, gamma, mean, rstd, fuse_gelu=False, dgamma=None, dbeta=None, dbias=None, want_dbias=False,
                  fold=None, dres=None):
    dy = dy.contiguous()
    x = x.contiguous()
    rows, cols = _rows_cols(x)
    dx = torch.empty_like(x)
    acc = dgamma is not None
    if not acc:
        dgamma = torch.empty(cols, dtype=gamma.dtype, device=x.device)
        dbeta = torch.empty(cols, dtype=gamma.dtype, device=x.device)
        if want_dbias:
            dbias = torch.empty(cols, dtype=gamma.dtype, device=x.device)
    assert dgamma.dtype == x.dtype and dbeta.dtype == x.dtype and (dbias is None or dbias.dtype == x.dtype)
    wsr = lib().cdll.ofa_layernorm_bwd_ws_rows()
    if fold is not None and acc:
        ns = lib().cdll.ofa_layernorm_bwd_slots(rows, cols, dtype_code(x), int(fuse_gelu))
        nq = 3 if (fuse_gelu and dbias is not None) else 2
        ws = torch.empty(nq * ns * cols, dtype=torch.float32, device=x.device)
        for q, o in enumerate((dgamma, dbeta, dbias)[:nq]):
            fold.add(ws, q * ns * cols, o, cols, cols, ns)
        acc = DEFER_FOLD
    else:
        ws = workspace(wsr * cols * 4, x.device, "ln")
    if fuse_gelu:
        lib().call("ofa_gelu_layernorm_bwd", ptr(dy), ptr(x), ptr(gamma), ptr(mean), ptr(rstd), ptr(dx), ptr(dgamma),
                   ptr(dbeta), ptr(dbias), ptr(ws), rows, cols, int(acc), dtype_code(x), stream())
    else:
        if dres is not None:
            dres = dres.contiguous()
            assert dres.shape == x.shape and dres.dtype == x.dtype
        lib().call("ofa_layernorm_bwd", ptr(dy), ptr(x), ptr(gamma), ptr(mean), ptr(rstd), ptr(dres), ptr(dx), ptr(dgamma),
                   ptr(dbeta), ptr(ws), rows, cols, int(acc), dtype_code(x), stream())
    if acc == DEFER_FOLD:
        fold.flush_if_large()
    return dx, dgamma, dbeta, (dbias if fuse_gelu else None)


def gemm(a, b, trans_a=False, trans_b=False, bias=None, bias_row=False, alpha=1.0, out=None, accumulate=False,
         out_f32=False, force_simple=False, a_kpad_zero=False, fold=None):
    assert a.dim() == b.dim() and a.dim() in (2, 3)
    batched = a.dim() == 3
    if a.stride(-1) != 1:
        a = a.contiguous()
    if b.stride(-1) != 1:
        b = b.contiguous()
    batch = a.shape[0] if batched else 1
    ar, ac = a.shape[-2], a.shape[-1]
    br, bc = b.shape[-2], b.shape[-1]
    M, K = (ac, ar) if trans_a else (ar, ac)
    N, Kb = (br, bc) if trans_b else (bc, br)
    if K != Kb:
        raise OfaError(f"gemm: inner dimensions differ ({K} vs {Kb})")
    dt = dtype_code(a)
    if b.dtype != a.dtype:
        raise OfaError("gemm: operand dtypes differ")
    if out is None:
        odt = torch.float32 if (out_f32 or a.dtype == torch.float32) else a.dtype
        out = torch.empty((batch, M, N) if batched else (M, N), dtype=odt, device=a.device)
    flags = 0
    if bias is not None:
        flags |= GEMM_BIAS_ROW if bias_row else GEMM_BIAS_COL
    if accumulate:
        flags |= GEMM_ACCUM
    if force_simple:
        flags |= GEMM_FORCE_SIMPLE
    if dt != F32 and out.dtype == torch.float32:
        flags |= GEMM_OUT_F32
    if a_kpad_zero:
        flags |= 32
    lda, ldb, ldc = a.stride(-2), b.stride(-2), out.stride(-2)
    sa = a.stride(0) if batched else 0
    sb = b.stride(0) if batched else 0
    sc = out.stride(0) if batched else 0
    ws = None
    if fold is not None and bias is None and not batched and ldc == N and N % 4 == 0 and _prof is None:
        nsp = lib().cdll.ofa_gemm_splits(M, N, K, int(trans_a), int(trans_b), 1, flags, dt, 256 << 20)
        if nsp > 1:
            ws = torch.empty(nsp * M * N, dtype=torch.float32, device=a.device)
            fold.add(ws, 0, out, M * N, M * N, nsp, alpha, accumulate)
            flags |= GEMM_DEFER_REDUCE
            ws_bytes = 256 << 20
    if ws is None:
        ws = workspace(256 << 20, a.device, "gemm")
        ws_bytes = ws.numel() * 4
    args = ("ofa_gemm", ptr(a), ptr(b), ptr(out), ptr(bias), M, N, K, int(trans_a), int(trans_b), lda, ldb, ldc, batch,
            sa, sb, sc, 0, 0, 0, 0, float(alpha), flags, dt, ptr(ws), ws_bytes, stream())
    if _prof is not None:
        e0 = torch.cuda.Event(enable_timing=True)
        e1 = torch.cuda.Event(enable_timing=True)
        e0.record()
        lib().call(*args)
        e1.record()
        _prof.append((2.0 * M * N * K * batch, e0, e1, batch * ((M * K + K * N) * a.element_size() + M * N * out.element_size())))
    else:
        lib().call(*args)
    if flags & GEMM_DEFER_REDUCE:
        fold.flush_if_large()
    return out


def gemm_colstat(a, b, bias=None, max_groups=512):
    assert a.dim() == 2 and b.dim() == 2 and a.shape[1] == b.shape[1] and a.dtype == b.dtype
    if a.stride(-1) != 1:
        a = a.contiguous()
    if b.stride(-1) != 1:
        b = b.contiguous()
    M, Kd, N = a.shape[0], a.shape[1], b.shape[0]
    out = torch.empty(M, N, dtype=a.dtype, device=a.device)
    if a.dtype == torch.float32 or N % 8:
        return gemm(a, b, False, True, bias=bias, out=out), None
    flags = GEMM_BIAS_COL if bias is not None else 0
    ws = workspace(256 << 20, a.device, "gemm")
    cap = min(max_groups, (M + 31) // 32)
    partial = torch.empty(cap, 2, N, dtype=torch.float64, device=a.device)
    groups = ctypes.c_int(0)
    args = ("ofa_gemm_colstat", ptr(a), ptr(b), ptr(out), ptr(bias), M, N, Kd, 0, 1, a.stride(0), b.stride(0), out.stride(0), 1.0,
            flags, dtype_code(a), ptr(ws), ws.numel() * 4, ptr(partial), cap, ctypes.addressof(groups), stream())
    if _prof is not None:
        e0 = torch.cuda.Event(enable_timing=True)
        e1 = torch.cuda.Event(enable_timing=True)
        e0.record()
        lib().call(*args)
        e1.record()
        _prof.append((2.0 * M * N * Kd, e0, e1, (M * Kd + Kd * N + M * N) * a.element_size()))
    else:
        lib().call(*args)
# ... 348 lines not shown
        Tb, Sb = bias.shape[1], bias.shape[2]
        swz_row, swz_col = _shared_swz(bias, bias_shared)
        dbias = torch.empty(heads, Tb, Sb, dtype=dbias_dtype, device=q.device) if need_dbias else None
        ws, ws_bytes = None, 0
        if need_dbias:
            nchunk = lib().cdll.ofa_attn_sbias_chunks(B if seg is None else seg.batch, heads, Tb, Sb)
            if nchunk > 1 or dbias_dtype not in (torch.float32, q.dtype):
                ws = torch.empty(nchunk, heads, Tb, Sb, dtype=torch.float32, device=q.device)
                ws_bytes = ws.numel() * 4
        if seg is not None:
            assert B == 1 and kpm is None and seg.rows_q == T and seg.rows_k == S
            dims = (seg.batch, heads, min(seg.max_q, Tb), min(seg.max_k, Sb), Tpad, ldq, ldk, ldo, float(scale), int(causal), ptr(seg.table), T, S)
            kp = None
        else:
            dims = (B, heads, T, S, Tpad, ldq, ldk, ldo, float(scale), int(causal), None, 0, 0)
            kp = ptr(kpm)
        lib().call("ofa_attn_sbias_bwd_cs" if cs else "ofa_attn_sbias_bwd", ptr(q), ptr(k), ptr(v), ptr(dout), ptr(bias), ptr(swz_row),
                   ptr(swz_col), Tb, Sb, kp, ptr(c_attn), _c_dtype(c_attn), ptr(lse),
                   ptr(delta), ptr(out), ptr(dq), ptr(dk), ptr(dv), ptr(dbias), dtype_code(dbias) if dbias is not None else F32, ptr(ws),
                   ws_bytes, *dims, dtype_code(q), *csa, stream())
        return dq, dk, dv, dbias, delta
    if seg is not None:
        assert B == 1 and bias is None and kpm is None and not need_dbias and seg.rows_q == T and seg.rows_k == S
        lib().call(fn, ptr(q), ptr(k), ptr(v), ptr(dout), None, None, ptr(c_attn), _c_dtype(c_attn), ptr(lse),
                   ptr(delta), ptr(out), ptr(dq), ptr(dk), ptr(dv), None, seg.batch, heads, seg.max_q, seg.max_k, Tpad, ldq, ldk, ldo,
                   float(scale), int(causal), ptr(seg.table), T, S, dtype_code(q), *csa, stream())
        return dq, dk, dv, None, delta
    lib().call(fn, ptr(q), ptr(k), ptr(v), ptr(dout), ptr(bias), ptr(kpm), ptr(c_attn), _c_dtype(c_attn), ptr(lse),
               ptr(delta), ptr(out), ptr(dq), ptr(dk), ptr(dv), ptr(dbias), B, heads, T, S, Tpad, ldq, ldk, ldo, float(scale),
               int(causal), None, 0, 0, dtype_code(q), *csa, stream())
    return dq, dk, dv, dbias, delta


def attn_decode(q, k_cache, v_cache, S, heads, scale, bias=None, kpm=None, c_attn=None, need_probs=False):
    B, D = q.shape
    q = q.contiguous()
    assert k_cache.dim() == 3 and k_cache.shape == v_cache.shape and k_cache.stride() == v_cache.stride()
    assert k_cache.stride(2) == 1 and k_cache.shape[0] == B and k_cache.shape[1] >= S and k_cache.dtype == q.dtype
    out = torch.empty(B, D, dtype=q.dtype, device=q.device)
    probs = torch.empty(B * heads, S, dtype=q.dtype, device=q.device) if need_probs else None
    if bias is not None:
        bias = bias.reshape(B * heads, S).to(q.dtype).contiguous()
    kpm_ld = 0
    if kpm is not None:
        kpm = _u8(kpm)
        kpm_ld = kpm.stride(0)
    lib().call("ofa_attn_decode", ptr(q), ptr(k_cache), ptr(v_cache), ptr(bias), ptr(kpm), ptr(c_attn), _c_dtype(c_attn),
               ptr(out), ptr(probs), B, heads, D // heads, S, k_cache.stride(1), k_cache.stride(0), kpm_ld, float(scale),
               dtype_code(q), stream())
    return out, probs


def gelu_fwd(x):
    x = x.contiguous()
    y = torch.empty_like(x)
    lib().call("ofa_gelu_fwd", ptr(x), ptr(y), x.numel(), dtype_code(x), stream())
    return y


def gelu_bwd(dy, x):
    dy, x = dy.contiguous(), x.contiguous()
    dx = torch.empty_like(x)
    lib().call("ofa_gelu_bwd", ptr(dy), ptr(x), ptr(dx), x.numel(), dtype_code(x), stream())
    return dx


def dropout_add(x, residual, p, seed, offset, offset_base=None):
    x = x.contiguous()
    if residual is not None:
        residual = residual.contiguous()
    y = torch.empty_like(x)
    lib().call("ofa_dropout_add_fwd", ptr(x), ptr(residual), ptr(y), x.numel(), float(p), seed, offset, ptr(offset_base),
               dtype_code(x), stream())
    return y


def dropout_bwd(dy, p, seed, offset, offset_base=None):
    dy = dy.contiguous()
    dx = torch.empty_like(dy)
    lib().call("ofa_dropout_bwd", ptr(dy), ptr(dx), dy.numel(), float(p), seed, offset, ptr(offset_base), dtype_code(dy),
               stream())
    return dx


def add_rowvec_mask(a, b=None, vec=None, rowmask=None):
    a = a.contiguous()
    rows, cols = _rows_cols(a)
    period = 0
    if b is not None:
        b = b.contiguous()
        brows = b.numel() // cols
        if brows != rows:
            assert brows > 0 and rows % brows == 0, (rows, brows)
            period = brows
    if rowmask is not None:
        rowmask = _u8(rowmask)
    y = torch.empty_like(a)
    lib().call("ofa_add_rowvec_mask", ptr(a), ptr(b), ptr(vec), ptr(rowmask), ptr(y), rows, cols, period, dtype_code(a), stream())
    return y


def batch_sum(x, batch, out=None, accumulate=False):
    x = x.contiguous()
    n = x.numel() // batch
    if out is None:
        out = torch.empty(n, dtype=x.dtype, device=x.device)
        accumulate = False
    lib().call("ofa_batch_sum", ptr(x), ptr(out), int(batch), n, int(bool(accumulate)), dtype_code(x), stream())
    return out


def embedding_fwd(weight, ids, pad_mask_of=None):
    ids = ids.contiguous()
    V, D = weight.shape
    out = torch.empty(*ids.shape, D, dtype=weight.dtype, device=weight.device)
    mask = None
    if pad_mask_of is not None and D % (4 if weight.dtype == torch.float32 else 8) == 0:
        mask = torch.empty(ids.shape, dtype=torch.bool, device=weight.device)
    lib().call("ofa_embedding_fwd", ptr(weight), ptr(ids), ptr(out), ids.numel(), D, V, ptr(mask), int(pad_mask_of) if mask is not None else 0,
               dtype_code(weight), stream())
    if pad_mask_of is None:
        return out
    return out, (mask if mask is not None else ids.eq(pad_mask_of))


def gather_rows(src2d, index):
    assert src2d.dim() == 2 and src2d.is_contiguous() and index.dtype == torch.int64 and index.is_contiguous()
    out = torch.empty(index.numel(), src2d.shape[1], dtype=src2d.dtype, device=src2d.device)
    lib().call("ofa_gather_rows", ptr(src2d), ptr(index), ptr(out), index.numel(), src2d.shape[1], src2d.shape[0],
               dtype_code(src2d), stream())
    return out


def gather_rows_parts(parts, index):
    assert 1 <= len(parts) <= 8 and index.dtype == torch.int64 and index.is_contiguous()
    B, D = parts[0].shape[0], parts[0].shape[2]
    assert all(t.dim() == 3 and t.is_contiguous() and t.shape[0] == B and t.shape[2] == D and t.dtype == parts[0].dtype for t in parts)
    out = torch.empty(index.numel(), D, dtype=parts[0].dtype, device=parts[0].device)
    srcs = (ctypes.c_void_p * len(parts))(*[dptr(t) for t in parts])
    lens = (ctypes.c_int * len(parts))(*[int(t.shape[1]) for t in parts])
    lib().call("ofa_gather_rows_parts", ctypes.addressof(srcs), ctypes.addressof(lens), len(parts), ptr(index), ptr(out), index.numel(), D, B,
               dtype_code(parts[0]), stream())
    return out


def scatter_rows_part(dpacked, inverse, B, nk, Ttot, start):
    assert dpacked.dim() == 2 and dpacked.is_contiguous() and inverse.dtype == torch.int64 and inverse.is_contiguous()
    D = dpacked.shape[1]
    out = torch.empty(B, nk, D, dtype=dpacked.dtype, device=dpacked.device)
    lib().call("ofa_scatter_rows_part", ptr(dpacked), ptr(inverse), ptr(out), B, nk, Ttot, start, D, dpacked.shape[0], dtype_code(dpacked), stream())
    return out


def embedding_bwd(dout, ids, V, padding_idx=-1, dweight=None):
    dout = dout.contiguous()
    ids = ids.contiguous()
    D = dout.shape[-1]
    if dweight is None:
        dweight = torch.zeros(V, D, dtype=dout.dtype, device=dout.device)
    present = workspace(V, dout.device, "embed_present") if V > 4096 else None
    S = lib().cdll.ofa_embedding_bwd_slices(V, D)
    slices = workspace(S * V * D * 4, dout.device, "embed_slices") if S > 1 else None
    lib().call("ofa_embedding_bwd", ptr(dout), ptr(ids), ptr(dweight), ids.numel(), D, V,
               -1 if padding_idx is None else padding_idx, ptr(present), ptr(slices), dtype_code(dout), stream())
    return dweight


def segment_rowsum(dout2d, plan, dweight, accumulate):
    assert dout2d.dim() == 2 and dout2d.is_contiguous() and dweight.is_contiguous() and dout2d.dtype == dweight.dtype
    lib().call("ofa_segment_rowsum", ptr(dout2d), ptr(plan.order), ptr(plan.seg_off), ptr(plan.seg_row), ptr(dweight), plan.nseg,
               dout2d.shape[1], int(accumulate), dtype_code(dout2d), stream())
    return dweight


def im2col_patch(img, p, Kpad, lead=0):
    img = img.contiguous()
    B, C, H, W = img.shape
    col = torch.empty(B * (lead + (H // p) * (W // p)), Kpad, dtype=img.dtype, device=img.device)
    lib().call("ofa_im2col_patch", ptr(img), ptr(col), B, C, H, W, p, Kpad, int(lead), dtype_code(img), stream())
    return col


def step_stats_add(stats, loss, target, pad):
    assert stats.dtype == torch.float64 and stats.numel() >= 3 and loss.dtype == torch.float32 and loss.numel() == 1
    t = target.reshape(-1)
    assert t.dtype == torch.int64 and t.is_contiguous()
    lib().call("ofa_step_stats_add", ptr(stats), ptr(loss), ptr(t), t.numel(), int(pad), stream())


def cross_entropy_fwd(logits2d, target, V, ignore_index):
    rows, ld = logits2d.shape[0], logits2d.stride(0)
    lse = torch.empty(rows, dtype=torch.float32, device=logits2d.device)
    row_loss = torch.empty(rows, dtype=torch.float32, device=logits2d.device)
    lib().call("ofa_cross_entropy_fwd", ptr(logits2d), ptr(target), ptr(lse), ptr(row_loss), rows, V, ld, ignore_index,
               dtype_code(logits2d), stream())
    return lse, row_loss


def cross_entropy_fwd_grad_ok(logits2d, V):
    return logits2d.is_cuda and bool(lib().cdll.ofa_cross_entropy_fwd_grad_ok(int(V), int(logits2d.stride(0)), dtype_code(logits2d)))


def cross_entropy_fwd_grad(logits2d, target, grad_scale, V, ignore_index):
    rows, ld = logits2d.shape[0], logits2d.stride(0)
    lse = torch.empty(rows, dtype=torch.float32, device=logits2d.device)
    row_loss = torch.empty(rows, dtype=torch.float32, device=logits2d.device)
    dlogits = torch.empty(rows, ld, dtype=logits2d.dtype, device=logits2d.device)
    lib().call("ofa_cross_entropy_fwd_grad", ptr(logits2d), ptr(target), ptr(grad_scale), ptr(lse), ptr(row_loss), ptr(dlogits), rows, V,
               ld, ignore_index, dtype_code(logits2d), stream())
    return lse, row_loss, dlogits


def cross_entropy_bwd(logits2d, target, lse, grad_scale, V, ignore_index, dlogits=None):
    rows, ld = logits2d.shape[0], logits2d.stride(0)
    if dlogits is None:
        dlogits = torch.empty(rows, ld, dtype=logits2d.dtype, device=logits2d.device)
    lib().call("ofa_cross_entropy_bwd", ptr(logits2d), ptr(target), ptr(lse), ptr(grad_scale), ptr(dlogits), rows, V, ld,
               ignore_index, dtype_code(logits2d), stream())
    return dlogits


def ls_cross_entropy_fwd(logits2d, target, V, ignore_index, eps, cstart=-1, cend=-1, cmask=None):
    rows, ld = logits2d.shape[0], logits2d.stride(0)
    out = [torch.empty(rows, dtype=torch.float32, device=logits2d.device) for _ in range(4)]
    if cmask is not None:
        cmask = _u8(cmask)
    lib().call("ofa_ls_cross_entropy_fwd", ptr(logits2d), ptr(target), *[ptr(o) for o in out], rows, V, ld, ignore_index,
               float(eps), int(cstart), int(cend), ptr(cmask), dtype_code(logits2d), stream())
    return out


def ls_cross_entropy_bwd(logits2d, target, lse, row_cnt, row_w, grad_scale, V, ignore_index, eps, cstart=-1, cend=-1,
                         cmask=None):
    rows, ld = logits2d.shape[0], logits2d.stride(0)
    dlogits = torch.empty(rows, ld, dtype=logits2d.dtype, device=logits2d.device)
    if cmask is not None:
        cmask = _u8(cmask)
    lib().call("ofa_ls_cross_entropy_bwd", ptr(logits2d), ptr(target), ptr(lse), ptr(row_cnt), ptr(row_w), ptr(grad_scale),
               ptr(dlogits), rows, V, ld, ignore_index, float(eps), int(cstart), int(cend), ptr(cmask),
               dtype_code(logits2d), stream())
    return dlogits


def probs_fwd(logits2d, V, ld, log_probs):
    rows = logits2d.shape[0]
    y = torch.empty(rows, V, dtype=torch.float32, device=logits2d.device)
    lib().call("ofa_probs_fwd", ptr(logits2d), ptr(y), rows, V, ld, int(log_probs), dtype_code(logits2d), stream())
    return y


def probs_bwd(dy, y, V, dtype, log_probs):
    rows = y.shape[0]
    ld = (V + 7) // 8 * 8
    d = torch.empty(rows, ld, dtype=dtype, device=y.device)
    lib().call("ofa_probs_bwd", ptr(dy), ptr(y), ptr(d), rows, V, ld, int(log_probs), dtype_code(d), stream())
    return d


def sumsq(x, out):
    x = x.contiguous()
    ws = workspace(lib().cdll.ofa_sumsq_ws_floats() * 4, x.device, "sumsq")
    lib().call("ofa_sumsq", ptr(x), ptr(out), ptr(ws), x.numel(), dtype_code(x), stream())
    return out


def step_schedule(gsq, sample_size, step, lr, sched, gnorm, clip_norm, beta1, beta2):
    lib().call("ofa_step_schedule", ptr(gsq), ptr(sample_size), ptr(step), ptr(lr), ptr(sched), ptr(gnorm), float(clip_norm),
               float(beta1), float(beta2), stream())


def step_schedule_scaled(gsq, sample_size, step, lr, sched, gnorm, loss_scaler, clip_norm, beta1, beta2, scale_factor=2.0,
                         scale_window=2000, tolerance=0.0, threshold=None, min_loss_scale=1e-4):
    lib().call("ofa_step_schedule_scaled", ptr(gsq), ptr(sample_size), ptr(step), ptr(lr), ptr(sched), ptr(gnorm), ptr(loss_scaler),
               float(clip_norm), float(beta1), float(beta2), float(scale_factor), float(scale_window), float(tolerance),
               float(threshold or 0.0), float(min_loss_scale), stream())


def adam_step(master, exp_avg, exp_avg_sq, grad, model_param, coef, lr, beta1, beta2, eps, weight_decay, step):
    lib().call("ofa_adam_step", ptr(master), ptr(exp_avg), ptr(exp_avg_sq), ptr(grad), ptr(model_param), ptr(coef),
               master.numel(), float(lr), float(beta1), float(beta2), float(eps), float(weight_decay), int(step),
               dtype_code(grad), stream())


def colsum(x, alpha=1.0, out=None, accumulate=False, out_dtype=torch.float32, fold=None):
    if x.stride(-1) != 1:
        x = x.contiguous()
    rows, cols = x.shape
    if out is None:
        out = torch.empty(cols, dtype=out_dtype, device=x.device)
        fold = None
    if fold is not None and out.is_contiguous():
        ns = lib().cdll.ofa_colsum_slots(rows)
        ws = torch.empty(ns * cols, dtype=torch.float32, device=x.device)
        fold.add(ws, 0, out, cols, cols, ns, alpha, accumulate)
        lib().call("ofa_colsum", ptr(x), ptr(out), ptr(ws), rows, cols, x.stride(0), float(alpha), DEFER_FOLD,
                   dtype_code(x), dtype_code(out), stream())
        fold.flush_if_large()
        return out
    ws = workspace(lib().cdll.ofa_colsum_ws_floats(cols) * 4, x.device, "colsum")
    lib().call("ofa_colsum", ptr(x), ptr(out), ptr(ws), rows, cols, x.stride(0), float(alpha), int(accumulate),
               dtype_code(x), dtype_code(out), stream())
    return out


def mul(a, b):
    a, b = a.contiguous(), b.contiguous()
    rows, cols = _rows_cols(a)
    y = torch.empty_like(a)
    lib().call("ofa_mul", ptr(a), ptr(b), ptr(y), rows, cols, 0, dtype_code(a), stream())
    return y


def add_n(tensors):
    ts = [t.contiguous() for t in tensors]
    assert 1 <= len(ts) <= 16 and all(t.shape == ts[0].shape and t.dtype == ts[0].dtype for t in ts)
    if len(ts) == 1:
        return ts[0]
    out = torch.empty_like(ts[0])
    arr = (ctypes.c_void_p * len(ts))(*[dptr(t) for t in ts])
    lib().call("ofa_add_n", ctypes.addressof(arr), len(ts), ptr(out), out.numel(), dtype_code(out), stream())
    return out


def mul_rowvec(a, vec):
    a, vec = a.contiguous(), vec.contiguous()
    rows, cols = _rows_cols(a)
    y = torch.empty_like(a)
    lib().call("ofa_mul", ptr(a), ptr(vec), ptr(y), rows, cols, 1, dtype_code(a), stream())
    return y


def scale_row_groups(x, scale, group):
    x = x.contiguous()
    rows, cols = _rows_cols(x)
    assert scale.dtype == torch.float32 and scale.numel() * group == rows
    y = torch.empty_like(x)
    lib().call("ofa_scale_row_groups", ptr(x), ptr(scale.contiguous()), ptr(y), rows, cols, group, dtype_code(x), stream())
    return y


def sum_f32(x):
    x = x.contiguous()
    out = torch.empty((), dtype=torch.float32, device=x.device)
    lib().call("ofa_reduce_sum_f32", ptr(x), ptr(out), x.numel(), stream())
    return out


def bias_block_add_(bias, values, start):
    B, A, T, _ = bias.shape
    n = values.shape[0]
    values = values.contiguous()
    assert bias.is_contiguous() and values.dtype == bias.dtype
    lib().call("ofa_bias_block_add", ptr(bias), ptr(values), B, A, T, start, n, dtype_code(bias), stream())
    return bias


def bias_block_add_batch_(bias, values, start):
    B, A, T, _ = bias.shape
    n = values.shape[-1]
    values = values.contiguous()
    assert bias.is_contiguous() and values.dtype == bias.dtype and tuple(values.shape) == (B, A, n, n)
    lib().call("ofa_bias_block_add_batch", ptr(bias), ptr(values), B, A, T, start, n, dtype_code(bias), stream())
    return bias


def bias_block_slice(dbias, start, n):
    dbias = dbias.contiguous()
    B, A, T, _ = dbias.shape
    out = torch.empty(B, A, n, n, dtype=dbias.dtype, device=dbias.device)
    lib().call("ofa_bias_block_slice", ptr(dbias), ptr(out), B, A, T, start, n, dtype_code(dbias), stream())
    return out


def bias_outer_grad(dbias, start, F, P):
    dbias = dbias.contiguous()
    A, T = dbias.shape[-3], dbias.shape[-1]
    assert dbias.numel() == A * T * T
    dvf = torch.empty(F, F, A, dtype=dbias.dtype, device=dbias.device)
    dvi = torch.empty(P, P, A, dtype=dbias.dtype, device=dbias.device)
    lib().call("ofa_bias_outer_grad", ptr(dbias), ptr(dvf), ptr(dvi), A, T, start, F, P, dtype_code(dbias), stream())
    return dvf, dvi


def bias_block_grad(dbias, start, n):
    dbias = dbias.contiguous()
    B, A, T, _ = dbias.shape
    dvalues = torch.empty(n, n, A, dtype=dbias.dtype, device=dbias.device)
    lib().call("ofa_bias_block_grad", ptr(dbias), ptr(dvalues), B, A, T, start, n, dtype_code(dbias), stream())
    return dvalues


def mean_heads(p, B, heads):
    p = p.contiguous()
    T, S = p.shape[1], p.shape[2]
    out = torch.empty(B, T, S, dtype=p.dtype, device=p.device)
    lib().call("ofa_mean_heads", ptr(p), ptr(out), B, heads, T * S, dtype_code(p), stream())
    return out


def head_sum(x, B, heads, T):
    out = torch.empty(heads, dtype=torch.float32, device=x.device)
    lib().call("ofa_head_sum_f32", ptr(x), ptr(out), B, heads, T, x.stride(0), stream())
    return out


def conv_out_size(n, k, stride, pad):
    return (n + 2 * pad - k) // stride + 1


def im2col(x, B, H, W, C, kh, kw, stride, pad, nchw=False):
    x = x.contiguous()
    Ho, Wo = conv_out_size(H, kh, stride, pad), conv_out_size(W, kw, stride, pad)
    K = kh * kw * C
    Kpad = (K + 7) // 8 * 8
    col = torch.empty(B * Ho * Wo, Kpad, dtype=x.dtype, device=x.device)
    lib().call("ofa_im2col", ptr(x), ptr(col), B, H, W, C, kh, kw, stride, pad, Kpad, int(nchw), dtype_code(x), stream())
    return col, Ho, Wo


def col2im(dcol, B, H, W, C, kh, kw, stride, pad):
    dcol = dcol.contiguous()
    dx = torch.empty(B * H * W, C, dtype=dcol.dtype, device=dcol.device)
    lib().call("ofa_col2im", ptr(dcol), ptr(dx), B, H, W, C, kh, kw, stride, pad, dcol.shape[1], dtype_code(dcol), stream())
    return dx


def batchnorm_fwd(x, gamma, beta, running_mean, running_var, training, momentum, eps, relu=False, residual=None):
    x = x.contiguous()
    rows, C = x.shape
    y = torch.empty_like(x)
    mean = torch.empty(C, dtype=torch.float32, device=x.device)
    rstd = torch.empty(C, dtype=torch.float32, device=x.device)
    ws = workspace(lib().cdll.ofa_batchnorm_ws_floats(C) * 4, x.device, "bn")
    if residual is not None:
        residual = residual.contiguous()
    lib().call("ofa_batchnorm_fwd", ptr(x), ptr(gamma), ptr(beta), ptr(residual), ptr(y), ptr(mean), ptr(rstd),
               ptr(running_mean), ptr(running_var), ptr(ws), rows, C, float(eps), float(momentum), int(not training),
               int(relu), dtype_code(x), stream())
    return y, mean, rstd


def batchnorm_bwd(dy, y, x, gamma, mean, rstd, batch_stats, relu, want_dres=False, dgamma=None, dbeta=None, beta=None):
    dy = dy.contiguous()
    rows, C = x.shape
    dx = torch.empty_like(x)
    dres = torch.empty_like(x) if want_dres else None
    acc = dgamma is not None
# ... 215 lines not shown
```

ofasys_amd/module/layers.py:

```python
import torch
import torch.nn as nn

from .. import ops


class OfaLayerNorm(nn.LayerNorm):
    def forward(self, x):
        return ops.layer_norm(x, self.weight, self.bias, self.eps)

    def fork(self, x):
        return ops.layer_norm_fork(x, self.weight, self.bias, self.eps)


def LayerNorm(normalized_shape, eps=1e-5, elementwise_affine=True, export=False):
    assert elementwise_affine, "the hot path only uses affine LayerNorm"
    return OfaLayerNorm(normalized_shape, eps, elementwise_affine)


class OfaLinear(nn.Linear):
    def forward(self, x, alpha=1.0, skip_bias_grad=False):
        return ops.linear(x, self.weight, self.bias, alpha, skip_bias_grad)


def Linear(in_features, out_features, bias=True):
    m = OfaLinear(in_features, out_features, bias)
    nn.init.xavier_uniform_(m.weight)
    if bias:
        nn.init.constant_(m.bias, 0.0)
    return m


class OfaEmbedding(nn.Embedding):
    def forward(self, ids):
        return ops.embedding(ids, self.weight, self.padding_idx)


def Embedding(num_embeddings, embedding_dim, padding_idx=None, zero_init=False):
    m = OfaEmbedding(num_embeddings, embedding_dim, padding_idx=padding_idx)
    nn.init.normal_(m.weight, mean=0, std=embedding_dim ** -0.5)
    if padding_idx is not None:
        nn.init.constant_(m.weight[padding_idx], 0)
    if zero_init:
        nn.init.constant_(m.weight, 0)
    return m


class Dropout(nn.Module):

    def __init__(self, p, module_name=None):
        super().__init__()
        self.p = p
        self.module_name = module_name
        self.apply_during_inference = False

    def forward(self, x, inplace: bool = False):
        if self.p > 0 and (self.training or self.apply_during_inference):
            return ops.dropout_add(x, None, self.p, True)
        return x


class DropPath(nn.Module):

    def __init__(self, drop_prob: float = 0.0, batch_axis: int = 0, scale_by_keep: bool = True):
        super().__init__()
        if drop_prob < 0 or drop_prob > 1:
            raise ValueError("droppath probability has to be between 0 and 1, but got {}".format(drop_prob))
        self.drop_prob = float(drop_prob)
        self.batch_axis = batch_axis
        self.scale_by_keep = scale_by_keep

    def forward(self, x):
        if self.drop_prob == 0.0 or not self.training:
            return x
        if self.batch_axis >= x.ndim:
            raise ValueError("droppath batch_axis has to be less than input.ndim, but got {} >= {}".format(self.batch_axis, x.ndim))
        if x.ndim != 3 or self.batch_axis not in (0, 1):
            raise NotImplementedError("DropPath is implemented for [T,B,C] / [B,T,C] activations")
        return ops.drop_path(x, self.drop_prob, self.batch_axis, self.scale_by_keep)

    def extra_repr(self):
        return "p={}".format(self.drop_prob)


def init_bert_params(module):
    from .multihead_attention import MultiheadAttention

    def normal_(data):
        data.copy_(data.cpu().normal_(mean=0.0, std=0.02).to(data.device))

    if isinstance(module, nn.Linear):
        normal_(module.weight.data)
        if module.bias is not None:
            module.bias.data.zero_()
    if isinstance(module, nn.Embedding):
        normal_(module.weight.data)
        if module.padding_idx is not None:
            module.weight.data[module.padding_idx].zero_()
    if isinstance(module, MultiheadAttention):
        normal_(module.q_proj.weight.data)
        normal_(module.k_proj.weight.data)
        normal_(module.v_proj.weight.data)
```

ofasys_amd/ops.py:

```python

import weakref

import torch

from . import kernels as K
from .lib import OfaError


def rows_view(x):
    C = x.shape[-1]
    if x.is_contiguous():
        lead = x.shape[:-1]
        return x.view(-1, C), lambda y: y.view(*lead, y.shape[-1])
    if x.dim() == 3:
        xt = x.transpose(0, 1)
        if xt.is_contiguous():
            b, t = xt.shape[0], xt.shape[1]
            return xt.view(-1, C), lambda y: y.view(b, t, y.shape[-1]).transpose(0, 1)
    xc = x.contiguous()
    lead = xc.shape[:-1]
    return xc.view(-1, C), lambda y: y.view(*lead, y.shape[-1])


def like_layout(x, ref):
    if x.dim() != 3 or x.shape != ref.shape:
        return x
    ref_bm = ref.transpose(0, 1).is_contiguous() and not ref.is_contiguous()
    x_bm = x.transpose(0, 1).is_contiguous() and not x.is_contiguous()
    if ref_bm == x_bm and (x_bm or x.is_contiguous() == ref.is_contiguous()):
        return x
    if ref_bm:
        return x.transpose(0, 1).contiguous().transpose(0, 1)
    return x.contiguous()


def batch_major(x):
    xt = x.transpose(0, 1)
    return xt if xt.is_contiguous() else xt.contiguous()


class _Rng:
    seed = 0x5EED0FA
    offset = 0
    base = {}

    @classmethod
    def manual_seed(cls, seed):
        cls.seed, cls.offset = int(seed) & (2 ** 63 - 1), 0
        for b in cls.base.values():
            b.zero_()

    @classmethod
    def reserve(cls, n, device):
        o = cls.offset
        cls.offset += (n + 3) // 4 + 1
        b = cls.base.get(device)
        if b is None:
            b = cls.base[device] = torch.zeros(1, dtype=torch.int64, device=device)
        return cls.seed, o, b

    @classmethod
    def advance(cls):
        if cls.offset:
            for b in cls.base.values():
                b.add_(cls.offset)
            cls.offset = 0


manual_seed = _Rng.manual_seed
rng_advance = _Rng.advance


def _sink(param):
    return getattr(param, "_ofa_grad", None) if param is not None else None


def _sink_done(param):
    cb = getattr(param, "_ofa_grad_ready", None)
    if cb is not None:
        cb()


class _Fold:
    queue = None
    queued = False


def defer_reductions(flag):
    if flag and _Fold.queue is None:
        _Fold.queue = K.FoldQueue()
    elif not flag and _Fold.queue is not None:
        flush_folds()
        _Fold.queue = None


def drop_pending():
    _Wgrads.items, _Wgrads.fillers, _Wgrads.queued, _Fold.queued = [], [], False, False
    if _Fold.queue is not None:
        _Fold.queue.__init__()


def flush_folds():
    flush_wgrads()
    _Fold.queued = False
    if _Fold.queue is not None:
        _Fold.queue.flush()


def _fold():
    q = _Fold.queue
    if q is not None and not _Fold.queued:
        try:
            torch.autograd.Variable._execution_engine.queue_callback(flush_folds)
            _Fold.queued = True
        except RuntimeError:
            return None
    return q


class _Wgrads:
    enabled = True
    items = []
    fillers = []
    queued = False
    FLUSH_TILES = 128
    FILLER_TILES = 40
    use_fillers = True


def _tiles_of(dy, x2d):
    return ((dy.shape[1] + 255) // 256) * ((x2d.shape[1] + 255) // 256)


def _queued_tiles():
    return sum(_tiles_of(it[0], it[1]) for it in _Wgrads.items)


def _wgrad(dy, x2d, gw, alpha, *weights, filler=False):
    if _Wgrads.enabled and K.gemm_group_ok(dy, x2d, gw) and _flush_at_end_of_backward():
        tn = (x2d.shape[1] + 255) // 256
        if (filler and _Wgrads.use_fillers and _Fold.queue is not None and gw.dim() == 2 and dy.shape[1] % 256 == 0
                and tn <= _Wgrads.FILLER_TILES and _tiles_of(dy, x2d) > _Wgrads.FILLER_TILES):
            rows = max(1, _Wgrads.FILLER_TILES // tn) * 256
            record = [0, weights]
            for r0 in range(0, dy.shape[1], rows):
                r1 = min(r0 + rows, dy.shape[1])
                _Wgrads.fillers.append((dy[:, r0:r1], x2d, gw[r0:r1], float(alpha), (), record))
                record[0] += 1
            return
        if _Wgrads.items and _Wgrads.items[0][0].shape[0] != dy.shape[0]:
            flush_wgrads()
        _Wgrads.items.append((dy, x2d, gw, float(alpha), weights, None))
        if len(_Wgrads.items) == K.GROUP_MAX:
            flush_wgrads()
        return
    K.gemm(dy, x2d, True, False, alpha=alpha, out=gw, accumulate=True, fold=_fold())
    for w in weights:
        _sink_done(w)


def _flush_at_end_of_backward():
    if not _Wgrads.queued:
        try:
            torch.autograd.Variable._execution_engine.queue_callback(_end_of_backward)
            _Wgrads.queued = True
        except RuntimeError:
            return False
    return True


def _end_of_backward():
    _Wgrads.queued = False
    flush_wgrads()
    while _Wgrads.fillers:
        rows = _Wgrads.fillers[0][0].shape[0]
        take = [f for f in _Wgrads.fillers if f[0].shape[0] == rows][:K.GROUP_MAX]
        _Wgrads.fillers = [f for f in _Wgrads.fillers if all(f is not t for t in take)]
        _Wgrads.items = take
        flush_wgrads(fill=False)


def flush_wgrads(fill=True):
    items, _Wgrads.items = _Wgrads.items, []
    if not items:
        return
    if fill and _Wgrads.fillers:
        rows, tiles = items[0][0].shape[0], sum(_tiles_of(it[0], it[1]) for it in items)
        rest = []
        for f in _Wgrads.fillers:
            t = _tiles_of(f[0], f[1])
            if f[0].shape[0] == rows and tiles + t <= 256 and len(items) < K.GROUP_MAX:
                items.append(f)
                tiles += t
            else:
                rest.append(f)
        _Wgrads.fillers = rest
    if len(items) == 1:
        dy, x2d, gw, alpha = items[0][:4]
        K.gemm(dy, x2d, True, False, alpha=alpha, out=gw, accumulate=True, fold=_fold())
    else:
        fold = _fold()
        q = fold if fold is not None else K.FoldQueue()
        K.gemm_group_tn([it[:4] for it in items], q)
        if fold is None:
            q.flush()
        else:
            q.flush_if_large()
    for it in items:
        for w in it[4]:
            _sink_done(w)
        if it[5] is not None:
            it[5][0] -= 1
            if it[5][0] == 0:
                for w in it[5][1]:
                    _sink_done(w)


class _WgradBoundaryFn(torch.autograd.Function):
    @staticmethod
    def forward(ctx, x):
        return x.view_as(x)

    @staticmethod
    def backward(ctx, dy):
        if _queued_tiles() > _Wgrads.FLUSH_TILES or 2 * len(_Wgrads.items) > K.GROUP_MAX:
            flush_wgrads()
        return dy


def wgrad_boundary(x):
    if _Wgrads.enabled and torch.is_grad_enabled() and x.requires_grad:
        return _WgradBoundaryFn.apply(x)
    return x


class LayerNormFn(torch.autograd.Function):
    @staticmethod
    def forward(ctx, x2d, weight, bias, eps, fuse_gelu):
        y, mean, rstd = K.layernorm_fwd(x2d, weight, bias, eps, fuse_gelu)
        ctx.save_for_backward(x2d, weight, mean, rstd)
        ctx.fuse_gelu = fuse_gelu
        ctx.bias_ref = bias
        return y

    @staticmethod
    def backward(ctx, dy):
        x2d, weight, mean, rstd = ctx.saved_tensors
        bias = ctx.bias_ref
        gw, gb = _sink(weight), _sink(bias)
        if gw is not None and gb is not None:
            dx = K.layernorm_bwd(dy, x2d, weight, mean, rstd, ctx.fuse_gelu, dgamma=gw, dbeta=gb, fold=_fold())[0]
            _sink_done(weight)
            _sink_done(bias)
            return dx, None, None, None, None
        dx, dg, db, _ = K.layernorm_bwd(dy, x2d, weight, mean, rstd, ctx.fuse_gelu)
        return dx, dg, db, None, None


class LayerNormForkFn(torch.autograd.Function):

    @staticmethod
    def forward(ctx, x2d, weight, bias, eps):
        y, mean, rstd = K.layernorm_fwd(x2d, weight, bias, eps, False)
        ctx.save_for_backward(x2d, weight, mean, rstd)
        ctx.bias_ref = bias
        return x2d.view_as(x2d), y

    @staticmethod
    def backward(ctx, dres, dy):
        x2d, weight, mean, rstd = ctx.saved_tensors
# ... 58 lines not shown
        if xb_sink is not None:
            _sink_done(x_bias)
        elif x_bias is not None:
            raise OfaError("residual_join: x_bias needs gradient sinks (the Linear skipped its own bias gradient)")
        if use_sinks:
            for t in params:
                if t is not None:
                    _sink_done(t)
            return dx, dres, None, None, None, None, None, None, None
        return dx, dres, grads[0], grads[1], grads[2], grads[3], None, None, None


def join_takes_bias_grad(*params):
    return torch.is_grad_enabled() and all(p is not None and p.requires_grad and _sink(p) is not None for p in params)


def residual_join(x, residual, ln_a, p, training, ln_b, eps=1e-5, x_bias=None):
    x2d, restore = rows_view(x)
    r2d = None
    if residual is not None:
        r2d, _ = rows_view(residual)
        if r2d.shape != x2d.shape:
            raise OfaError("residual_join: shape mismatch")
    wa, ba = (ln_a.weight, ln_a.bias) if ln_a is not None else (None, None)
    wb, bb = (ln_b.weight, ln_b.bias) if ln_b is not None else (None, None)
    y, z = ResidualJoinFn.apply(x2d, r2d, wa, ba, wb, bb, p if training else 0.0, eps, x_bias)
    return restore(y), (restore(z) if z is not None else None)


def layer_norm(x, weight, bias, eps=1e-5, fuse_gelu=False):
    x2d, restore = rows_view(x)
    return restore(LayerNormFn.apply(x2d, weight, bias, eps, fuse_gelu))


class LinearFn(torch.autograd.Function):
    @staticmethod
    def forward(ctx, x2d, weight, bias, alpha, skip_bias_grad=False):
        ctx.save_for_backward(x2d, weight)
        ctx.alpha = alpha
        ctx.has_bias = bias is not None and not skip_bias_grad
        ctx.bias_ref = bias
        N = weight.shape[0]
        out = None
        ctx.padded = False
        if N % 8 != 0:
            store = torch.empty(x2d.shape[0], (N + 63) // 64 * 64, dtype=x2d.dtype, device=x2d.device)
            out = store[:, :N]
            ctx.padded = True
        return K.gemm(x2d, weight, False, True, bias=bias, alpha=alpha, out=out)

    @staticmethod
    def backward(ctx, dy):
        x2d, weight = ctx.saved_tensors
        dy = dy if dy.stride(-1) == 1 else dy.contiguous()
        dx = dw = db = None
        N = weight.shape[0]
        kpad = ctx.padded and dy.stride(0) >= (N + 7) // 8 * 8 and dy.stride(0) % 8 == 0
        if ctx.needs_input_grad[0]:
            dx = K.gemm(dy, weight, False, False, alpha=ctx.alpha, a_kpad_zero=kpad)
        if ctx.needs_input_grad[1]:
            gw = _sink(weight)
            if gw is not None:
                _wgrad(dy, x2d, gw, ctx.alpha, weight)
            else:
                dw = K.gemm(dy, x2d, True, False, alpha=ctx.alpha)
        if ctx.has_bias and ctx.needs_input_grad[2]:
            gb = _sink(ctx.bias_ref)
            if gb is not None:
                K.colsum(dy, alpha=ctx.alpha, out=gb, accumulate=True, fold=_fold())
                _sink_done(ctx.bias_ref)
            else:
                db = K.colsum(dy, alpha=ctx.alpha, out_dtype=weight.dtype)
        return dx, dw, db, None, None


def linear(x, weight, bias=None, alpha=1.0, skip_bias_grad=False):
    x2d, restore = rows_view(x)
    return restore(LinearFn.apply(x2d, weight, bias, alpha, skip_bias_grad))


class LinearGeluLayerNormFn(torch.autograd.Function):

    @staticmethod
    def forward(ctx, x2d, weight, bias, ln_w, ln_b, eps):
        h = K.gemm(x2d, weight, False, True, bias=bias)
        y, mean, rstd = K.layernorm_fwd(h, ln_w, ln_b, eps, True)
        ctx.save_for_backward(x2d, weight, h, ln_w, mean, rstd)
        ctx.refs = (bias, ln_b)
        return y

    @staticmethod
    def backward(ctx, dy):
        x2d, weight, h, ln_w, mean, rstd = ctx.saved_tensors
        bias, ln_b = ctx.refs
        gg, gb, gbias = _sink(ln_w), _sink(ln_b), _sink(bias)
        sunk = gg is not None and gb is not None and gbias is not None
        if sunk:
            dh = K.layernorm_bwd(dy, h, ln_w, mean, rstd, True, dgamma=gg, dbeta=gb, dbias=gbias, fold=_fold())[0]
            for p in (ln_w, ln_b, bias):
                _sink_done(p)
            dg = db = dbias = None
        else:
            dh, dg, db, dbias = K.layernorm_bwd(dy, h, ln_w, mean, rstd, True, want_dbias=True)
        dx = K.gemm(dh, weight, False, False) if ctx.needs_input_grad[0] else None
        gw = _sink(weight)
        dw = None
        if gw is not None:
            _wgrad(dh, x2d, gw, 1.0, weight)
        else:
            dw = K.gemm(dh, x2d, True, False)
        return dx, dw, dbias, dg, db, None


def linear_gelu_layer_norm(x, weight, bias, ln_w, ln_b, eps=1e-5):
    x2d, restore = rows_view(x)
    return restore(LinearGeluLayerNormFn.apply(x2d, weight, bias, ln_w, ln_b, eps))


class GeluFn(torch.autograd.Function):
    @staticmethod
    def forward(ctx, x):
        ctx.save_for_backward(x)
        return K.gelu_fwd(x)

    @staticmethod
    def backward(ctx, dy):
        (x,) = ctx.saved_tensors
        return K.gelu_bwd(dy, x)


def gelu(x):
    x2d, restore = rows_view(x)
    return restore(GeluFn.apply(x2d))


class DropoutAddFn(torch.autograd.Function):

    @staticmethod
    def forward(ctx, x, residual, p):
        seed, off, base = _Rng.reserve(x.numel(), x.device)
        ctx.p, ctx.seed, ctx.off, ctx.base = p, seed, off, base
        ctx.has_res = residual is not None
        return K.dropout_add(x, residual, p, seed, off, base)

    @staticmethod
    def backward(ctx, dy):
        dx = K.dropout_bwd(dy, ctx.p, ctx.seed, ctx.off, ctx.base)
        return dx, (dy if ctx.has_res else None), None


class AddFn(torch.autograd.Function):

    @staticmethod
    def forward(ctx, a, b, vec, rowmask, vec_param=None):
        ctx.save_for_backward(rowmask)
        ctx.has = (b is not None, vec is not None)
        ctx.vdtype = vec.dtype if vec is not None else None
        ctx.b_shape = tuple(b.shape) if (b is not None and b.numel() != a.numel()) else None
        ctx.vec_param = vec_param
        return K.add_rowvec_mask(a, b, vec, rowmask)

    @staticmethod
    def backward(ctx, dy):
        (rowmask,) = ctx.saved_tensors
        g = K.add_rowvec_mask(dy, None, None, rowmask) if rowmask is not None else dy
        dvec = None
        if ctx.has[1]:
            gv = _sink(ctx.vec_param)
            if gv is not None and gv.is_contiguous():
                K.colsum(g, out=gv.view(-1), accumulate=True)
                _sink_done(ctx.vec_param)
            else:
                dvec = K.colsum(g, out_dtype=ctx.vdtype)
        db = None
        if ctx.has[0]:
            if ctx.b_shape is None:
                db = g
            else:
                nb = 1
                for d in ctx.b_shape:
                    nb *= d
                db = K.batch_sum(g, g.numel() // nb).view(ctx.b_shape)
        return g, db, dvec, None, None


def dropout_add(x, residual, p, training):
    if residual is not None:
        x = like_layout(x, residual)
    x2d, restore = rows_view(x)
    r2d = None
    if residual is not None:
        r2d, _ = rows_view(residual)
        if r2d.shape != x2d.shape:
            raise OfaError("dropout_add: shape mismatch")
    if training and p > 0:
        return restore(DropoutAddFn.apply(x2d, r2d, p))
    if r2d is None:
        return x
    return restore(AddFn.apply(x2d, r2d, None, None))


def shared_rows(x):
    if x is not None and x.dim() == 3 and x.shape[0] > 1 and x.stride(0) == 0:
        base = x._base
        if (base is not None and base.dim() == 3 and base.shape[0] == 1 and tuple(base.shape[1:]) == tuple(x.shape[1:])
                and base.data_ptr() == x.data_ptr() and base.stride()[1:] == x.stride()[1:]):
            return base
        return x[:1]
    return None


def first_sample(x):
    base = shared_rows(x)
    return base if base is not None else x[:1]


def add_rowvec_mask(a, b=None, vec=None, rowmask=None, vec_param=None):
    if vec_param is not None and not (vec is not None and vec.requires_grad and torch.is_grad_enabled() and _sink(vec_param) is not None):
        vec_param = None
    if vec_param is not None:
        vec = vec.detach()
    if b is not None:
        base = shared_rows(b)
        if base is not None and a.dim() == 3 and a.is_contiguous() and tuple(a.shape[1:]) == tuple(base.shape[1:]):
            b = base
        if b.shape[0] == 1 and a.dim() == 3 and a.shape[0] > 1 and a.is_contiguous() and tuple(a.shape[1:]) == tuple(b.shape[1:]):
            m = rowmask.reshape(-1) if rowmask is not None else None
            return AddFn.apply(a.view(-1, a.shape[-1]), b.reshape(-1, b.shape[-1]), vec, m, vec_param).view(a.shape)
        b = like_layout(b, a)
    a2d, restore = rows_view(a)
    b2d = rows_view(b)[0] if b is not None else None
    m = rowmask.reshape(-1) if rowmask is not None else None
    return restore(AddFn.apply(a2d, b2d, vec, m, vec_param))


class DropPathFn(torch.autograd.Function):

    @staticmethod
    def forward(ctx, x2d, scale, group):
        ctx.save_for_backward(scale)
        ctx.group = group
        return K.scale_row_groups(x2d, scale, group)

    @staticmethod
    def backward(ctx, dy):
        (scale,) = ctx.saved_tensors
        return K.scale_row_groups(dy.contiguous(), scale, ctx.group), None, None


def _drop_path_uniform(B, device):
    return torch.rand(B, dtype=torch.float32, device=device)


def drop_path(x, drop_prob, batch_axis=1, scale_by_keep=True):
    keep = 1.0 - drop_prob
    B = x.shape[batch_axis]
    mask = (keep + _drop_path_uniform(B, x.device)).floor_()
    if keep > 0.0 and scale_by_keep:
        mask = mask / keep
    xb = batch_major(x) if batch_axis == 1 else x.contiguous()
    T, C = xb.shape[1], xb.shape[2]
    y = DropPathFn.apply(xb.view(B * T, C), mask, T).view(B, T, C)
    return y.transpose(0, 1) if batch_axis == 1 else y


def cached_index(owner, key, make):
    cache = owner.__dict__.setdefault("_ofa_index_cache", {})
    hit = cache.get(key)
    if hit is not None:
        ref = next(owner.buffers(), None)
        ref = ref if ref is not None else next(owner.parameters(), None)
        if ref is None or hit.device == ref.device:
            return hit
    t = make()
    if not (t.is_cuda and torch.cuda.is_current_stream_capturing()):
        if len(cache) >= 64:
            cache.clear()
        cache[key] = t
    return t


def owner_token(owner):
    tok = owner.__dict__.get("_ofa_owner_token")
    if tok is None or tok.owner_id != id(owner):
        tok = owner.__dict__["_ofa_owner_token"] = _OwnerToken(id(owner))
        weakref.finalize(owner, _purge_owner_entries, tok)
    return tok


def _purge_owner_entries(tok):
    def mentions(key):
        return key is tok or (isinstance(key, tuple) and any(mentions(k) for k in key))
    for cache in _TOKEN_KEYED_CACHES:
        for key in [k for k in cache if mentions(k)]:
            del cache[key]


_TOKEN_KEYED_CACHES = []


class _OwnerToken:
    __slots__ = ("owner_id",)

    def __init__(self, owner_id):
        self.owner_id = owner_id

    def __deepcopy__(self, memo):
        return _OwnerToken(-1)


class SegmentPlan:
    _cache = {}

    def __init__(self, ids):
        flat = ids.reshape(-1)
        assert flat.numel() < 2 ** 31
        sorted_ids, order = torch.sort(flat, stable=True)
        rows, counts = torch.unique_consecutive(sorted_ids, return_counts=True)
        self.nseg = int(rows.numel())
        self.order = order.to(torch.int32)
        self.seg_row = rows.to(torch.int32)
        off = torch.zeros(self.nseg + 1, dtype=torch.int32, device=ids.device)
        off[1:] = torch.cumsum(counts, 0).to(torch.int32)
        self.seg_off = off
        self.min_row, self.max_row = (int(rows.min()), int(rows.max())) if self.nseg else (0, -1)

    @classmethod
    def get(cls, key, ids):
        plan = cls._cache.get(key)
        if plan is None:
            if ids.is_cuda and torch.cuda.is_current_stream_capturing():
                return None
            if len(cls._cache) > 512:
                cls._cache.clear()
            plan = cls._cache[key] = cls(ids)
        return plan


_TOKEN_KEYED_CACHES.append(SegmentPlan._cache)


class EmbeddingFn(torch.autograd.Function):
    @staticmethod
    def forward(ctx, ids, weight, padding_idx, plan_key=None, pad_mask_of=None):
        ctx.save_for_backward(ids)
        ctx.V, ctx.padding_idx = weight.shape[0], padding_idx
        ctx.weight_ref = weight
        ctx.plan_key = plan_key
        ctx.with_mask = pad_mask_of is not None
        if pad_mask_of is None:
            return K.embedding_fwd(weight, ids)
        out, mask = K.embedding_fwd(weight, ids, pad_mask_of)
        ctx.mark_non_differentiable(mask)
        return out, mask

    @staticmethod
    def backward(ctx, dout, *_unused):
        return EmbeddingFn._backward(ctx, dout) + (None,)

    @staticmethod
    def _backward(ctx, dout):
        (ids,) = ctx.saved_tensors
        pad = -1 if ctx.padding_idx is None else ctx.padding_idx
        gw = _sink(ctx.weight_ref)
        D = dout.shape[-1]
        plan = None
        if ctx.plan_key is not None and D <= 64 and ctx.padding_idx is None:
            plan = SegmentPlan.get((ctx.plan_key, tuple(ids.shape), str(ids.device)), ids)
            if plan is not None and not (0 <= plan.min_row and plan.max_row < ctx.V):
                plan = None
        if plan is not None:
            d2 = dout.reshape(-1, D)
            d2 = d2 if d2.is_contiguous() else d2.contiguous()
            if gw is not None:
                K.segment_rowsum(d2, plan, gw, True)
                _sink_done(ctx.weight_ref)
                return None, None, None, None
            return None, K.segment_rowsum(d2, plan, torch.zeros(ctx.V, D, dtype=dout.dtype, device=dout.device), False), None, None
        if gw is not None:
            K.embedding_bwd(dout, ids, ctx.V, pad, dweight=gw)
            _sink_done(ctx.weight_ref)
            return None, None, None, None
        dw = K.embedding_bwd(dout, ids, ctx.V, pad)
        return None, dw, None, None


def embedding(ids, weight, padding_idx=None, plan_key=None):
    return EmbeddingFn.apply(ids, weight, padding_idx, plan_key)


def embedding_with_pad_mask(ids, weight, padding_idx, pad):
    return EmbeddingFn.apply(ids, weight, padding_idx, None, int(pad))


def _c_attn_grad(delta, c_attn, B, heads, T):
    g = _sink(c_attn)
    if g is not None:
        K.c_attn_grad(delta, c_attn, B, heads, T, out=g, accumulate=True)
        _sink_done(c_attn)
        return None
    return K.c_attn_grad(delta, c_attn, B, heads, T)


def _split_seg(kpm):
    if kpm is not None and not torch.is_tensor(kpm):
        return None, kpm
    return kpm, None


class PackRowsFn(torch.autograd.Function):

    @staticmethod
    def forward(ctx, x2d, index, inverse):
        ctx.save_for_backward(inverse)
        return K.gather_rows(x2d, index)

    @staticmethod
    def backward(ctx, dout):
        (inverse,) = ctx.saved_tensors
        return K.gather_rows(dout.contiguous(), inverse), None, None


class PackPartsFn(torch.autograd.Function):

    @staticmethod
    def forward(ctx, index, inverse, *parts):
        ctx.save_for_backward(inverse)
        ctx.lens = [int(t.shape[1]) for t in parts]
        ctx.B = parts[0].shape[0]
        return K.gather_rows_parts([t.contiguous() for t in parts], index)

    @staticmethod
    def backward(ctx, dout):
        (inverse,) = ctx.saved_tensors
        d = dout.contiguous()
        T, grads, s = sum(ctx.lens), [], 0
        for i, n in enumerate(ctx.lens):
            grads.append(K.scatter_rows_part(d, inverse, ctx.B, n, T, s) if ctx.needs_input_grad[2 + i] else None)
            s += n
        return (None, None) + tuple(grads)


class LazyCat:

    def __init__(self, parts):
        self.parts = list(parts)
        B, _, D = self.parts[0].shape
        self.shape = torch.Size((B, sum(int(t.shape[1]) for t in self.parts), D))
        self.dtype, self.device = self.parts[0].dtype, self.parts[0].device

    def size(self, dim=None):
        return self.shape if dim is None else self.shape[dim]

    def materialize(self):
        return torch.cat(tuple(self.parts), dim=1)


def materialize(x):
    return x.materialize() if isinstance(x, LazyCat) else x


def pack_rows(x, index, inverse):
    B, T, D = x.shape
    if isinstance(x, LazyCat):
        if len(x.parts) <= 8 and D % 8 == 0 and all(t.is_cuda and t.dtype == x.parts[0].dtype and t.shape[0] == B and t.dim() == 3
                                                    for t in x.parts):
            return PackPartsFn.apply(index, inverse, *x.parts).view(1, -1, D)
        x = x.materialize()
    return PackRowsFn.apply(x.reshape(B * T, D), index, inverse).view(1, -1, D)


def _dbias_dtype(bias, shared):
    return bias.dtype if (shared and bias is not None) else torch.float32


def _shared_dbias(dbias, bias, shared):
    if dbias is None or not shared:
        return dbias
    return dbias.to(bias.dtype).view(bias.shape)


class FusedAttentionFn(torch.autograd.Function):

    @staticmethod
    def forward(ctx, q, k, v, bias, kpm, c_attn, heads, scale, causal, bias_shared=False):
        kpm, seg = _split_seg(kpm)
        out, lse = K.attn_fwd(q, k, v, heads, scale, bias=bias, kpm=kpm, c_attn=c_attn, causal=causal, seg=seg, bias_shared=bias_shared)
        ctx.save_for_backward(q, k, v, out, lse, bias, kpm, c_attn)
        ctx.c_ref = c_attn
        ctx.heads, ctx.scale, ctx.causal, ctx.seg, ctx.bias_shared = heads, scale, causal, seg, bias_shared
        return out

    @staticmethod
    def backward(ctx, dout):
        q, k, v, out, lse, bias, kpm, c_attn = ctx.saved_tensors
        need_dbias = bias is not None and ctx.needs_input_grad[3]
        dq, dk, dv, dbias, delta = K.attn_bwd(q, k, v, out, dout, lse, ctx.heads, ctx.scale, bias=bias, kpm=kpm,
                                              c_attn=c_attn, causal=ctx.causal, need_dbias=need_dbias, seg=ctx.seg,
                                              bias_shared=ctx.bias_shared, dbias_dtype=_dbias_dtype(bias, ctx.bias_shared))
        dbias = _shared_dbias(dbias, bias, ctx.bias_shared)
        dc = None
        if c_attn is not None and ctx.needs_input_grad[5]:
            dc = _c_attn_grad(delta, ctx.c_ref, q.shape[0], ctx.heads, q.shape[1])
        return dq, dk, dv, dbias, None, dc, None, None, None, None


def _packed(ws, arena_view):
    return arena_view if arena_view is not None else torch.cat([w.reshape(w.shape[0], -1) if w.dim() > 1 else w for w in ws])


def _packed_wgrads(ws, gview, dy2, x2):
    if gview is not None:
        _wgrad(dy2, x2, gview, 1.0, *ws)
        return [None] * len(ws)
    return _packed_grads(ws, None, lambda o, acc, f: K.gemm(dy2, x2, True, False, out=o, accumulate=acc, fold=f))


def _packed_grads(ws, gview, grad_packed_fn, inputs=()):
    if gview is not None:
        grad_packed_fn(gview, True, _fold())
        for w in ws:
            _sink_done(w)
        return [None] * len(ws)
    g = grad_packed_fn(None, False, None)
    outs, o = [], 0
    for w in ws:
        n = w.shape[0]
        outs.append(g[o:o + n].view(w.shape))
        o += n
    return outs


class _AttnCs:
    __slots__ = ("bufs", "bias_ws", "c_ws", "ns")


def _attn_cs_begin(gb, c_ref, B, T, S, seg, heads, dev, packed_kvq=False, want_q=True):
    fq = _fold() or K.ImmediateFold()
    D = heads * 64
    gc = _sink(c_ref) if c_ref is not None else None
    use_b = gb is not None and gb.is_contiguous() and want_q
# ... 446 lines not shown
        values = [None if k is None else ((next(it), next(it)) if k == "outer" else next(it)) for k in kinds]
        blocks = []
        for s, k, v in zip(starts, kinds, values):
            if k is None:
                blocks.append(None)
            elif k == "outer":
                blocks.append((s, v[0].shape[0], v[1].shape[0], v[0].dtype))
            elif k == "batch":
                blocks.append(("batch", s, v.shape[-1], v.dtype))
            else:
                blocks.append((s, v.shape[0], v.dtype))
        ctx.blocks = blocks
        ctx.set_materialize_grads(False)
        if abs_bias.shape[0] == 1 and abs_bias.is_cuda and abs_bias.dtype in (torch.bfloat16, torch.float16) and "batch" not in kinds:
            out, swz = K.bias_build(abs_bias[0], starts, values)
            ctx.mark_non_differentiable(*swz)
            return out.unsqueeze(0), swz[0], swz[1]
        out = abs_bias.clone(memory_format=torch.contiguous_format)
        for s, k, v in zip(starts, kinds, values):
            if v is None:
                continue
            if k == "batch":
                assert v.shape[0] == out.shape[0] and v.shape[1] == out.shape[1] and v.shape[2] == v.shape[3], \
                    f"per-sample self_attn_bias {tuple(v.shape)} does not fit the layer bias {tuple(out.shape)}"
                K.bias_block_add_batch_(out, v.to(out.dtype), s)
                continue
            if k == "outer":
                v = OuterRelPos(*v).dense()
            K.bias_block_add_(out, v.to(out.dtype), s)
        return out, None, None

    @staticmethod
    def backward(ctx, dout, _dr=None, _dc=None):
        if dout is None:
            return (None, None, None) + (None,) * sum(0 if b is None else (2 if (len(b) == 4 and b[0] != "batch") else 1) for b in ctx.blocks)
        grads = []
        for blk in ctx.blocks:
            if blk is None:
                continue
            if blk[0] == "batch":
                _, s, n, dt = blk
                grads.append(K.bias_block_slice(dout, s, n).to(dt))
            elif len(blk) == 4:
                s, Fr, P, dt = blk
                if dout.shape[0] == 1 and dout.is_cuda:
                    dvf, dvi = K.bias_outer_grad(dout, s, Fr, P)
                else:
                    d = K.bias_block_grad(dout, s, Fr * P).view(Fr, P, Fr, P, -1).float()
                    dvf, dvi = d.sum((1, 3)), d.sum((0, 2))
                grads += [dvf.to(dt), dvi.to(dt)]
            else:
                s, n, dt = blk
                grads.append(K.bias_block_grad(dout, s, n).to(dt))
        return (dout, None, None, *grads)


class MulRowvecFn(torch.autograd.Function):
    @staticmethod
    def forward(ctx, a, vec):
        ctx.save_for_backward(a, vec)
        return K.mul_rowvec(a, vec)

    @staticmethod
    def backward(ctx, dy):
        a, vec = ctx.saved_tensors
        return K.mul_rowvec(dy, vec), K.colsum(K.mul(dy, a), out_dtype=vec.dtype)


def mul_rowvec(a, vec):
    a2d, restore = rows_view(a)
    return restore(MulRowvecFn.apply(a2d, vec))


class ScaleFn(torch.autograd.Function):
    _scalars = {}

    @classmethod
    def _scalar(cls, value, like):
        key = (float(value), like.device)
        v = cls._scalars.get(key)
        if v is None:
            v = cls._scalars[key] = torch.full((1,), float(value), dtype=torch.float32, device=like.device)
        return v

    @staticmethod
    def forward(ctx, x2d, fwd, bwd):
        ctx.bwd = bwd
        if fwd == 1.0 or x2d.shape[0] == 0:
            return x2d.view_as(x2d)
        return K.scale_row_groups(x2d, ScaleFn._scalar(fwd, x2d), x2d.shape[0])

    @staticmethod
    def backward(ctx, dy):
        if ctx.bwd == 1.0 or dy.shape[0] == 0:
            return dy, None, None
        dy = dy.contiguous()
        return K.scale_row_groups(dy, ScaleFn._scalar(ctx.bwd, dy), dy.shape[0]), None, None


def scale(x, fwd=1.0, bwd=None):
    bwd = fwd if bwd is None else bwd
    if fwd == 1.0 and bwd == 1.0:
        return x
    x2d, restore = rows_view(x)
    return restore(ScaleFn.apply(x2d, float(fwd), float(bwd)))


class PatchEmbedFn(torch.autograd.Function):

    @staticmethod
    def forward(ctx, img, weight, bias, cls, p):
        B, C, H, W = img.shape
        D = weight.shape[0]
        Kc = C * p * p
        Kpad = (Kc + 7) // 8 * 8
        lead = 0 if cls is None else 1
        col = K.im2col_patch(img.to(weight.dtype), p, Kpad, lead)
        wp = weight.reshape(D, Kc)
        if Kpad != Kc:
            wp2 = getattr(weight, "_ofa_kpad", None)
            if wp2 is None or wp2.shape != (D, Kpad) or wp2.dtype != weight.dtype or wp2.device != weight.device:
                wp2 = weight.new_zeros(D, Kpad)
                if not (weight.is_cuda and torch.cuda.is_current_stream_capturing()):
                    weight._ofa_kpad = wp2
            wp2[:, :Kc].copy_(wp.detach())
            wp = wp2
        out = K.gemm(col, wp, False, True, bias=bias).view(B, lead + (H // p) * (W // p), D)
        if cls is not None:
            out[:, 0, :] = cls.reshape(1, D).to(out.dtype)
        ctx.save_for_backward(col)
        ctx.meta = (weight.shape, Kc, Kpad, lead)
        ctx.refs = (weight, bias, cls)
        return out

    @staticmethod
    def backward(ctx, dout):
        (col,) = ctx.saved_tensors
        wshape, Kc, Kpad, lead = ctx.meta
        weight, bias, cls = ctx.refs
        B, T, D = dout.shape
        d2 = dout.reshape(B * T, D)
        d2 = d2 if d2.is_contiguous() else d2.contiguous()
        dw = db = dcls = None
        gw = _sink(weight)
        if gw is not None and gw.is_contiguous() and Kc % 4 == 0:
            K.gemm(d2, col[:, :Kc], True, False, out=gw.view(wshape[0], Kc), accumulate=True)
            _sink_done(weight)
        else:
            dw = K.gemm(d2, col, True, False)[:, :Kc].reshape(wshape)
        first = dout[:, 0, :] if lead else None
        if cls is not None:
            gc = _sink(cls)
            if gc is not None:
                K.colsum(first, out=gc.view(-1), accumulate=True)
                _sink_done(cls)
            else:
                dcls = K.colsum(first, out_dtype=dout.dtype).view(cls.shape)
        if bias is not None:
            gb = _sink(bias)
            if gb is not None:
                K.colsum(d2, out=gb, accumulate=True)
                if lead:
                    K.colsum(first, alpha=-1.0, out=gb, accumulate=True)
                _sink_done(bias)
            else:
                db = K.colsum(d2, out_dtype=dout.dtype)
                if lead:
                    db = db - K.colsum(first, out_dtype=dout.dtype)
        return None, dw, db, dcls, None


def patch_embed(img, weight, bias, p, cls_token=None):
    return PatchEmbedFn.apply(img, weight, bias, cls_token, p)


class CrossEntropyFn(torch.autograd.Function):

    @staticmethod
    def forward(ctx, logits, target, ignore_index, seed=None):
        V = logits.shape[-1]
        if logits.is_contiguous():
            l2d = logits.reshape(-1, V)
        else:
            try:
                l2d = logits.view(-1, V)
            except RuntimeError:
                l2d = logits.contiguous().view(-1, V)
        if l2d.stride(1) != 1 or l2d.stride(0) % (4 if l2d.dtype == torch.float32 else 8) != 0:
            pad = (-V) % 8
            store = torch.zeros(l2d.shape[0], V + pad, dtype=l2d.dtype, device=l2d.device)
            store[:, :V].copy_(l2d)
            l2d = store[:, :V]
        t = target.reshape(-1).contiguous()
        ctx.ignore_index, ctx.shape = ignore_index, logits.shape
        ctx.seed = ctx.pre = None
        if (seed is not None and ctx.needs_input_grad[0] and seed.dtype == torch.float32 and seed.numel() == 1 and seed.device == l2d.device
                and K.cross_entropy_fwd_grad_ok(l2d, V)):
            lse, row_loss, d = K.cross_entropy_fwd_grad(l2d, t, seed, V, ignore_index)
            ctx.seed, ctx.pre = seed, d
            ctx.save_for_backward(t, lse)
            ctx.l2d = l2d
            return K.sum_f32(row_loss)
        lse, row_loss = K.cross_entropy_fwd(l2d, t, V, ignore_index)
        ctx.save_for_backward(l2d, t, lse)
        return K.sum_f32(row_loss)

    @staticmethod
    def backward(ctx, dloss):
        if ctx.pre is not None:
            t, lse = ctx.saved_tensors
            d, seed, l2d = ctx.pre, ctx.seed, ctx.l2d
            ctx.pre = ctx.seed = ctx.l2d = None
            V = ctx.shape[-1]
            if dloss.data_ptr() == seed.data_ptr() and dloss.dtype == seed.dtype:
                return d[:, :V].view(ctx.shape), None, None, None
            gs = dloss.reshape(1).float().contiguous()
            d = K.cross_entropy_bwd(l2d, t, lse, gs, V, ctx.ignore_index, dlogits=d)
            return d[:, :V].view(ctx.shape), None, None, None
        l2d, t, lse = ctx.saved_tensors
        V = l2d.shape[1]
        gs = dloss.reshape(1).float().contiguous()
        d = K.cross_entropy_bwd(l2d, t, lse, gs, V, ctx.ignore_index)
        return d[:, :V].view(ctx.shape), None, None, None


def cross_entropy_sum(logits, target, ignore_index, seed=None):
    return CrossEntropyFn.apply(logits, target, ignore_index, seed)


def _ce_rows(logits):
    V = logits.shape[-1]
    l2d = logits.reshape(-1, V) if logits.is_contiguous() else logits.view(-1, V)
    if l2d.stride(1) != 1 or l2d.stride(0) % (4 if l2d.dtype == torch.float32 else 8) != 0:
        pad = (-V) % 8
        store = torch.zeros(l2d.shape[0], V + pad, dtype=l2d.dtype, device=l2d.device)
        store[:, :V].copy_(l2d)
        l2d = store[:, :V]
    return l2d


class LabelSmoothedCrossEntropyFn(torch.autograd.Function):

    @staticmethod
    def forward(ctx, logits, target, ignore_index, eps, constraint_range, constraint_masks, drop_worst_ratio):
        V = logits.shape[-1]
        l2d = _ce_rows(logits)
        t = target.reshape(-1).contiguous()
        cs, ce = constraint_range if constraint_range is not None else (-1, -1)
        cm = constraint_masks.reshape(-1, V).contiguous() if constraint_masks is not None else None
        lse, row_loss, row_nll, row_cnt = K.ls_cross_entropy_fwd(l2d, t, V, ignore_index, eps, cs, ce, cm)
        valid = t.ne(ignore_index)
        row_w = None
        if drop_worst_ratio > 0:
            n = valid.sum()
            k = (n.double() * (1 - drop_worst_ratio)).floor().long()
            key = torch.where(valid, row_loss, torch.full_like(row_loss, float("inf")))
            order = torch.argsort(key, stable=True)
            rank = torch.empty_like(order)
            rank[order] = torch.arange(order.numel(), device=order.device)
            row_w = (rank < k).float()
            row_loss, row_nll = row_loss * row_w, row_nll * row_w
            ntok = k
        else:
            ntok = valid.sum()
        ctx.save_for_backward(l2d, t, lse, row_cnt, row_w, cm)
        ctx.cfg = (ignore_index, eps, cs, ce, logits.shape)
        ctx.mark_non_differentiable(ntok)
        return K.sum_f32(row_loss), K.sum_f32(row_nll).detach(), ntok

    @staticmethod
    def backward(ctx, dloss, dnll, dntok):
        l2d, t, lse, row_cnt, row_w, cm = ctx.saved_tensors
        ignore_index, eps, cs, ce, shape = ctx.cfg
        V = l2d.shape[1]
        gs = dloss.reshape(1).float().contiguous()
        d = K.ls_cross_entropy_bwd(l2d, t, lse, row_cnt, row_w, gs, V, ignore_index, eps, cs, ce, cm)
        return d[:, :V].view(shape), None, None, None, None, None, None


def label_smoothed_cross_entropy(logits, target, ignore_index, eps, constraint_range=None, constraint_masks=None,
                                 drop_worst_ratio=0.0):
    return LabelSmoothedCrossEntropyFn.apply(logits, target, ignore_index, eps, constraint_range, constraint_masks,
                                             drop_worst_ratio)


def _rows_padded(logits):
    V = logits.shape[-1]
    try:
        l2d = logits.view(-1, V)
    except RuntimeError:
        l2d = logits.reshape(-1, V)
    if l2d.stride(1) != 1:
        l2d = l2d.contiguous()
    return l2d, l2d.stride(0)


class ProbsFn(torch.autograd.Function):

    @staticmethod
    def forward(ctx, logits, log_probs):
        l2d, ld = _rows_padded(logits)
        rows, V = l2d.shape
        y = K.probs_fwd(l2d, V, ld, log_probs)
        ctx.save_for_backward(y)
        ctx.meta = (logits.shape, logits.dtype, log_probs)
        return y.view(*logits.shape)

    @staticmethod
    def backward(ctx, dy):
        (y,) = ctx.saved_tensors
        shape, dtype, log_probs = ctx.meta
        V = shape[-1]
        d = K.probs_bwd(dy.reshape(-1, V).float().contiguous(), y, V, dtype, log_probs)
        return d[:, :V].view(shape), None


# ... 272 lines not shown
```

Measured before the change: 1.400 million.

## Add range embedding backward, ids-based embedding backward, vectorized im2col, batched colsum folds

Adds a direct range-based backward for positional embeddings: when positions are an arange starting at a known row, the gradient is a batch sum written straight into the weight grad. This replaces the general scatter path and the separate broadcast-add backward. It also adds an LDS-based per-id embedding backward kernel, a dword-vectorized im2col kernel for 16-bit patch embedding, and routes bias/cls/vec colsums through the deferred batched fold with a new 16-lane mode. Each path carries env-gated fallbacks, and the new code adds alignment and shape preconditions.

```diff
diff --git a/include/ofasys_amd.h b/include/ofasys_amd.h
--- a/include/ofasys_amd.h
+++ b/include/ofasys_amd.h
@@ -145,6 +145,13 @@
 int ofa_embedding_bwd_slices(int64_t V, int D);
 int ofa_embedding_bwd(const void* dout, const int64_t* ids, void* dweight, int64_t n, int D, int64_t V,
                       int64_t padding_idx, uint8_t* present_ws, float* slice_ws, int dtype, void* stream);
+#define OFA_EMBEDDING_IDS_MAX 15360
+int ofa_embedding_bwd_ids_ok(int64_t n, int D, int64_t V, int dtype);
+int ofa_embedding_bwd_ids(const void* dout, const int64_t* ids, void* dweight, int64_t n, int D, int64_t V, int64_t padding_idx,
+                          int slices, int dtype, void* stream);
+int ofa_embedding_range_bwd(const void* dout, void* dweight, int batch, int64_t T, int D, int64_t V, int64_t r0, int dtype, void* stream);
+enum { OFA_EDGE_POS_RANGE = 0, OFA_EDGE_TOKEN_BWD = 1, OFA_EDGE_COLSUM_FOLD = 2, OFA_EDGE_IM2COL = 3 };
+int ofa_step_edges_old(int item);
 
 int ofa_gelu_fwd(const void* x, void* y, int64_t n, int dtype, void* stream);
 int ofa_gelu_bwd(const void* dy, const void* x, void* dx, int64_t n, int dtype, void* stream);
@@ -259,6 +266,7 @@
   float alpha;
   int32_t out_dtype;
 } ofa_fold_job;
+#define OFA_FOLD_LANES16 4
 int ofa_fold_batched(const ofa_fold_job* jobs, int njobs, void* stream);
 typedef struct ofa_copy_job {
   const void* src;
diff --git a/ofasys_amd/adaptor/image_patch_embed.py b/ofasys_amd/adaptor/image_patch_embed.py
--- a/ofasys_amd/adaptor/image_patch_embed.py
+++ b/ofasys_amd/adaptor/image_patch_embed.py
@@ -51,4 +51,4 @@
         n = x.size(1)
         mask = ops.cached_index(self, ("nomask", batch_size, n), lambda: torch.zeros((batch_size, n), dtype=torch.bool, device=image.device))
         pos = ops.cached_index(self, ("arange", n), lambda: torch.arange(n, dtype=torch.long, device=image.device).unsqueeze(0))
-        return AdaptorOutput(x, mask, self.embed_image_positions(pos).expand(batch_size, -1, -1), None)
+        return AdaptorOutput(x, mask, self.embed_image_positions(pos, range_start=0).expand(batch_size, -1, -1), None)
diff --git a/ofasys_amd/adaptor/text.py b/ofasys_amd/adaptor/text.py
--- a/ofasys_amd/adaptor/text.py
+++ b/ofasys_amd/adaptor/text.py
@@ -75,7 +75,7 @@
             token_embedding = self.embed_tokens(src_tokens)
             padding_masks = src_tokens.eq(pad) if pad is not None else torch.zeros_like(src_tokens, dtype=torch.bool)
         positions = ops.cached_index(self, ("arange", seq_len), lambda: torch.arange(seq_len, device=src_tokens.device).unsqueeze(0))
-        pos_embed = self.embed_positions(positions).expand(bsz, -1, -1)
+        pos_embed = self.embed_positions(positions, range_start=0).expand(bsz, -1, -1)
         return AdaptorOutput(token_embedding, padding_masks, pos_embed, [])
 
     def forward_output(self, x: Tensor, extra: Dict[str, Any], slot: Slot, **kwargs):
diff --git a/ofasys_amd/csrc/elementwise.hip b/ofasys_amd/csrc/elementwise.hip
--- a/ofasys_amd/csrc/elementwise.hip
+++ b/ofasys_amd/csrc/elementwise.hip
@@ -1,6 +1,11 @@
 #include "common.h"
 
 namespace ofa {
+
+template <typename T> __device__ __forceinline__ float round_to(float v);
+template <> __device__ __forceinline__ float round_to<float>(float v) { return v; }
+template <> __device__ __forceinline__ float round_to<bf16_t>(float v) { return bf2f(f2bf(v)); }
+template <> __device__ __forceinline__ float round_to<f16_t>(float v) { return (float)(f16_t)v; }
 
 template <typename T, bool BWD>
 __global__ __launch_bounds__(256) void gelu_kernel(const T* __restrict__ dy, const T* __restrict__ x, T* __restrict__ y,
@@ -295,6 +300,140 @@
     float a = 0.f;
     for (int s = 0; s < S; ++s) a += part[((int64_t)s * V + v) * D + c];
     st1<T>(dw + v * D + c, ld1<T>(dw + v * D + c) + a);
+  }
+}
+
+constexpr int EMB_IDS_WAVES = 8;
+template <typename T, int NV, bool SLICED>
+__global__ __launch_bounds__(EMB_IDS_WAVES * 64) void embedding_bwd_ids_kernel(const T* __restrict__ dout, const int64_t* __restrict__ ids,
+                                                                               T* __restrict__ dw, int n, int D, int64_t V,
+                                                                               int64_t padding_idx, int per) {
+  constexpr int N = Vec<T>::N;
+  constexpr int G = NV <= 1 ? 8 : 4;
+  typedef typename Vec<T>::type raw_t;
+  extern __shared__ int sid[];
+  const int npad = (n + 63) & ~63;
+  for (int i = threadIdx.x; i < npad; i += EMB_IDS_WAVES * 64) {
+    const int64_t id = i < n ? ids[i] : -1;
+    sid[i] = (id >= 0 && id < V && id != padding_idx) ? (int)id : -1;
+  }
+  __syncthreads();
+  const int lane = threadIdx.x & 63;
+  int* queue = sid + npad + (threadIdx.x >> 6) * 64;
+  for (int pos = blockIdx.x * EMB_IDS_WAVES + (threadIdx.x >> 6); pos < n; pos += gridDim.x * EMB_IDS_WAVES) {
+    const int v = sid[pos];
+    if (v < 0) continue;
+    const int base0 = pos & ~63;
+    bool earlier = false;
+    for (int base = 0; base <= base0; base += 64) earlier |= (base + lane < pos) && sid[base + lane] == v;
+    if (__ballot(earlier)) continue;
+    float acc[NV][N], tot[SLICED ? NV : 1][N];
+#pragma unroll
+    for (int i = 0; i < NV; ++i)
+#pragma unroll
+      for (int j = 0; j < N; ++j) acc[i][j] = 0.f;
+#pragma unroll
+    for (int i = 0; i < (SLICED ? NV : 1); ++i)
+#pragma unroll
+      for (int j = 0; j < N; ++j) tot[i][j] = 0.f;
+    int cnt = 0;
+    auto drain = [&]() {
+      __builtin_amdgcn_fence(__ATOMIC_RELEASE, "wavefront");
+      __builtin_amdgcn_wave_barrier();
+      __builtin_amdgcn_fence(__ATOMIC_ACQUIRE, "wavefront");
+      for (int k = 0; k < cnt; k += G) {
+        raw_t raw[G][NV];
+#pragma unroll
+        for (int g = 0; g < G; ++g) {
+          const T* row = dout + (int64_t)queue[k + g < cnt ? k + g : cnt - 1] * D;
+#pragma unroll
+          for (int i = 0; i < NV; ++i) {
+            const int c = (i * 64 + lane) * N;
+            if (c < D) raw[g][i] = *reinterpret_cast<const raw_t*>(row + c);
+          }
+        }
+#pragma unroll
+        for (int g = 0; g < G; ++g) {
+          if (k + g < cnt) {
+#pragma unroll
+            for (int i = 0; i < NV; ++i) {
+              if ((i * 64 + lane) * N < D) {
+                float x[N];
+                unpack16<T>(__builtin_bit_cast(uint4, raw[g][i]), x);
+#pragma unroll
+                for (int j = 0; j < N; ++j) acc[i][j] += x[j];
+              }
+            }
+          }
+        }
+      }
+      __builtin_amdgcn_wave_barrier();
+      cnt = 0;
+    };
+    auto push = [&](unsigned long long m, int base) {
+      if (!m) return;
+      const int c = __popcll(m);
+      if (cnt + c > 64) drain();
+      if ((m >> lane) & 1) queue[cnt + __popcll(m & ((1ull << lane) - 1))] = base + lane;
+      cnt += c;
+    };
+    int base = base0;
+    if (!SLICED) {
+      for (; base + 256 <= npad; base += 256) {
+        const int a0 = sid[base + lane], a1 = sid[base + 64 + lane], a2 = sid[base + 128 + lane], a3 = sid[base + 192 + lane];
+        const unsigned long long m0 = __ballot(a0 == v), m1 = __ballot(a1 == v), m2 = __ballot(a2 == v), m3 = __ballot(a3 == v);
+        if (m0 | m1 | m2 | m3) {
+          push(m0, base);
+          push(m1, base + 64);
+          push(m2, base + 128);
+          push(m3, base + 192);
+        }
+      }
+    }
+    for (; base < npad; base += 64) {
+      if (SLICED && base > base0 && base % per == 0) {
+        drain();
+#pragma unroll
+        for (int i = 0; i < NV; ++i)
+#pragma unroll
+          for (int j = 0; j < N; ++j) { tot[SLICED ? i : 0][j] += acc[i][j]; acc[i][j] = 0.f; }
+      }
+      push(__ballot(sid[base + lane] == v), base);
+    }
+    drain();
+    T* wr = dw + (int64_t)v * D;
+#pragma unroll
+    for (int i = 0; i < NV; ++i) {
+      const int c = (i * 64 + lane) * N;
+      if (c < D) {
+        float o[N];
+        load_vec<T>(wr + c, o);
+#pragma unroll
+        for (int j = 0; j < N; ++j) o[j] += SLICED ? tot[SLICED ? i : 0][j] + acc[i][j] : acc[i][j];
+        store_vec<T>(wr + c, o);
+      }
+    }
+  }
+}
+
+template <typename T>
+__global__ __launch_bounds__(256) void embedding_range_bwd_kernel(const T* __restrict__ dout, T* __restrict__ dw, int batch, int64_t n) {
+  constexpr int N = Vec<T>::N;
+  const int64_t total = n / N;
+  for (int64_t v = (int64_t)blockIdx.x * 256 + threadIdx.x; v < total; v += (int64_t)gridDim.x * 256) {
+    float acc[N], t[N], o[N];
+#pragma unroll
+    for (int j = 0; j < N; ++j) acc[j] = 0.f;
+#pragma unroll 8
+    for (int b = 0; b < batch; ++b) {
+      load_vec<T>(dout + (int64_t)b * n + v * N, t);
+#pragma unroll
+      for (int j = 0; j < N; ++j) acc[j] += t[j];
+    }
+    load_vec<T>(dw + v * N, o);
+#pragma unroll
+    for (int j = 0; j < N; ++j) o[j] += 0.f + round_to<T>(acc[j]);
+    store_vec<T>(dw + v * N, o);
   }
 }
 
@@ -315,6 +454,34 @@
       v = ld1<T>(img + ((b * C + c) * H + ph * p + i) * W + pw * p + j);
     }
     st1<T>(col + e, v);
+  }
+}
+template <typename T>
+__global__ __launch_bounds__(256) void im2col_patch_runs_kernel(const T* __restrict__ img, T* __restrict__ col, int B, int C, int H,
+                                                                int W, int p, int Kpad, int lead) {
+  static_assert(sizeof(T) == 2, "dword runs of 16-bit elements");
+  const int nph = H / p, npw = W / p, K = C * p * p, vpr = Kpad / 8;
+  const int per = lead + nph * npw;
+  const unsigned total = (unsigned)B * per * vpr;
+  const uint32_t* __restrict__ src = reinterpret_cast<const uint32_t*>(img);
+  for (unsigned v = blockIdx.x * 256 + threadIdx.x; v < total; v += gridDim.x * 256) {
+    const unsigned r = v / vpr;
+    const int k0 = (int)(v - r * vpr) * 8;
+    const int b = (int)(r / per), rs = (int)(r - (unsigned)b * per) - lead;
+    uint32_t w[4] = {0u, 0u, 0u, 0u};
+    if (rs >= 0 && k0 < K) {
+      const int ph = rs / npw, pw = rs - ph * npw;
+      int c = k0 / (p * p);
+      int i = (k0 - c * p * p) / p;
+      int j = k0 - c * p * p - i * p;
+#pragma unroll
+      for (int q = 0; q < 4; ++q) {
+        if (k0 + 2 * q < K) w[q] = src[((((int64_t)b * C + c) * H + ph * p + i) * W + pw * p + j) >> 1];
+        j += 2;
+        if (j >= p) { j = 0; if (++i >= p) { i = 0; ++c; } }
+      }
+    }
+    *reinterpret_cast<uint4*>(col + (int64_t)v * 8) = make_uint4(w[0], w[1], w[2], w[3]);
   }
 }
 
@@ -675,6 +842,79 @@
   return check_launch("embedding_fold");
 }
 
+extern "C" int ofa_step_edges_old(int item) {
+#ifdef OFA_DEBUG_SWITCHES
+  if (const char* e = getenv("OFA_STEP_EDGES_OLD")) return (atoi(e) >> item) & 1;
+#endif
+  return 0;
+}
+
+extern "C" int ofa_embedding_bwd_ids_ok(int64_t n, int D, int64_t V, int dtype) {
+  const int vecn = dtype == OFA_F32 ? 4 : 8;
+  return OFA_DT_OK(dtype) && n >= 0 && n <= OFA_EMBEDDING_IDS_MAX && V > 0 && V < ((int64_t)1 << 31) && D > 0 && D % vecn == 0 &&
+         D <= 64 * vecn * 4;
+}
+
+extern "C" int ofa_embedding_bwd_ids(const void* dout, const int64_t* ids, void* dweight, int64_t n, int D, int64_t V,
+                                     int64_t padding_idx, int slices, int dtype, void* stream) {
+  OFA_DT_CHECK("embedding_bwd_ids");
+  OFA_REQUIRE(n >= 0 && D > 0 && V > 0 && slices >= 1 && dout && ids && dweight, OFA_ERR_INVALID, "embedding_bwd_ids: bad argument");
+  OFA_REQUIRE(ofa_embedding_bwd_ids_ok(n, D, V, dtype), OFA_ERR_UNSUPPORTED,
+              "embedding_bwd_ids: n=%lld ids (at most %d), D=%d (whole 16-byte vectors, at most 256 of them): use ofa_embedding_bwd",
+              (long long)n, OFA_EMBEDDING_IDS_MAX, D);
+  OFA_REQUIRE((((uintptr_t)dout | (uintptr_t)dweight) & 15) == 0, OFA_ERR_UNSUPPORTED, "embedding_bwd_ids: buffers not 16-byte aligned");
+  if (n == 0) return 0;
+  hipStream_t st = (hipStream_t)stream;
+  const int vecn = dtype == OFA_F32 ? 4 : 8;
+  const int nv = cdiv(D, 64 * vecn);
+  const int per = (int)(((n + slices - 1) / slices + 63) / 64 * 64);
+  const int blocks = cdiv(n, EMB_IDS_WAVES) < 1024 ? cdiv(n, EMB_IDS_WAVES) : 1024;
+  const size_t lds = (size_t)((n + 63) / 64 * 64 + EMB_IDS_WAVES * 64) * sizeof(int);
+#define EMB_LAUNCH(T, NV, SL)                                                                                       \
+  hipLaunchKernelGGL((embedding_bwd_ids_kernel<T, NV, SL>), dim3(blocks), dim3(EMB_IDS_WAVES * 64), lds, st, (const T*)dout, ids, \
+                     (T*)dweight, (int)n, D, V, padding_idx, per)
+#define EMB_CASE(T, SL)                     \
+  do {                                      \
+    if (nv <= 1) EMB_LAUNCH(T, 1, SL);      \
+    else if (nv <= 2) EMB_LAUNCH(T, 2, SL); \
+    else EMB_LAUNCH(T, 4, SL);              \
+  } while (0)
+#define EMB_DT(SL)                            \
+  do {                                        \
+    if (dtype == OFA_F32) EMB_CASE(float, SL); \
+    else if (dtype == OFA_BF16) EMB_CASE(bf16_t, SL); \
+    else EMB_CASE(f16_t, SL);                 \
+  } while (0)
+  if (slices > 1) EMB_DT(true);
+  else EMB_DT(false);
+#undef EMB_DT
+#undef EMB_CASE
+#undef EMB_LAUNCH
+  return check_launch("embedding_bwd_ids");
+}
+
+extern "C" int ofa_embedding_range_bwd(const void* dout, void* dweight, int batch, int64_t T, int D, int64_t V, int64_t r0, int dtype,
+                                       void* stream) {
+  OFA_DT_CHECK("embedding_range_bwd");
+  OFA_REQUIRE(dout && dweight && batch >= 1 && T >= 0 && D > 0 && V > 0 && r0 >= 0 && r0 + T <= V, OFA_ERR_INVALID,
+              "embedding_range_bwd: bad argument (rows %lld .. %lld of %lld)", (long long)r0, (long long)(r0 + T), (long long)V);
+  OFA_REQUIRE(D % (dtype == OFA_F32 ? 4 : 8) == 0 && (((uintptr_t)dout | (uintptr_t)dweight) & 15) == 0, OFA_ERR_UNSUPPORTED,
+              "embedding_range_bwd: D=%d / buffers not whole 16-byte vectors: use ofa_embedding_bwd", D);
+  if (T == 0) return 0;
+  hipStream_t st = (hipStream_t)stream;
+  const int64_t n = T * D;
+  if (dtype == OFA_F32)
+    hipLaunchKernelGGL((embedding_range_bwd_kernel<float>), dim3(grid_for(n / 4)), dim3(256), 0, st, (const float*)dout,
+                       (float*)dweight + r0 * D, batch, n);
+  else if (dtype == OFA_BF16)
+    hipLaunchKernelGGL((embedding_range_bwd_kernel<bf16_t>), dim3(grid_for(n / 8)), dim3(256), 0, st, (const bf16_t*)dout,
+                       (bf16_t*)dweight + r0 * D, batch, n);
+  else
+    hipLaunchKernelGGL((embedding_range_bwd_kernel<f16_t>), dim3(grid_for(n / 8)), dim3(256), 0, st, (const f16_t*)dout,
+                       (f16_t*)dweight + r0 * D, batch, n);
+  return check_launch("embedding_range_bwd");
+}
+
 extern "C" int ofa_im2col_patch(const void* img, void* col, int B, int C, int H, int W, int p, int Kpad, int lead, int dtype,
                                 void* stream) {
   OFA_DT_CHECK("im2col_patch");
@@ -682,6 +922,17 @@
               "im2col_patch: bad argument (H=%d W=%d p=%d Kpad=%d)", H, W, p, Kpad);
   hipStream_t st = (hipStream_t)stream;
   const int64_t total = (int64_t)B * (lead + (int64_t)(H / p) * (W / p)) * Kpad;
+  if (total == 0) return 0;
+  if (dtype != OFA_F32 && p % 2 == 0 && Kpad % 8 == 0 && ((uintptr_t)img & 3) == 0 && ((uintptr_t)col & 15) == 0 &&
+      total / 8 < ((int64_t)1 << 31) && !ofa_step_edges_old(OFA_EDGE_IM2COL)) {
+    if (dtype == OFA_BF16)
+      hipLaunchKernelGGL((im2col_patch_runs_kernel<bf16_t>), dim3(grid_for(total / 8)), dim3(256), 0, st, (const bf16_t*)img,
+                         (bf16_t*)col, B, C, H, W, p, Kpad, lead);
+    else
+      hipLaunchKernelGGL((im2col_patch_runs_kernel<f16_t>), dim3(grid_for(total / 8)), dim3(256), 0, st, (const f16_t*)img,
+                         (f16_t*)col, B, C, H, W, p, Kpad, lead);
+    return check_launch("im2col_patch_runs");
+  }
   if (dtype == OFA_F32)
     hipLaunchKernelGGL((im2col_patch_kernel<float>), dim3(grid_for(total)), dim3(256), 0, st, (const float*)img, (float*)col,
                        B, C, H, W, p, Kpad, lead);
diff --git a/ofasys_amd/csrc/fold.hip b/ofasys_amd/csrc/fold.hip
--- a/ofasys_amd/csrc/fold.hip
+++ b/ofasys_amd/csrc/fold.hip
@@ -70,7 +70,7 @@
 }
 
 __global__ __launch_bounds__(256) void fold_batched_kernel(FoldJobs J) {
-  __shared__ float4 red[8][32];
+  __shared__ float4 red[16][32];
   int j = 0;
   while (j + 1 < J.njobs && blockIdx.x >= J.block0[j + 1]) ++j;
   const int64_t chunk = blockIdx.x - J.block0[j];
@@ -113,8 +113,39 @@
   }
   const int q = threadIdx.x & 31, sl = threadIdx.x >> 5;
   const int64_t c = chunk * 128 + q * 4;
-  float4 a = make_float4(0.f, 0.f, 0.f, 0.f);
-  if (c < cols) {
+  float4 a = make_float4(0.f, 0.f, 0.f, 0.f), a2 = a;
+  const bool l16 = J.flags[j] & 16;
+  if (c < cols && l16) {
+    if (vec) {
+      const float* r = p + c;
+      int s = sl;
+      for (; s + 24 < ns; s += 32) {
+        const float4 v0 = *reinterpret_cast<const float4*>(r + (int64_t)s * stride);
+        const float4 v1 = *reinterpret_cast<const float4*>(r + (int64_t)(s + 8) * stride);
+        const float4 v2 = *reinterpret_cast<const float4*>(r + (int64_t)(s + 16) * stride);
+        const float4 v3 = *reinterpret_cast<const float4*>(r + (int64_t)(s + 24) * stride);
+        a.x = (a.x + v0.x) + v2.x; a.y = (a.y + v0.y) + v2.y; a.z = (a.z + v0.z) + v2.z; a.w = (a.w + v0.w) + v2.w;
+        a2.x = (a2.x + v1.x) + v3.x; a2.y = (a2.y + v1.y) + v3.y; a2.z = (a2.z + v1.z) + v3.z; a2.w = (a2.w + v1.w) + v3.w;
+      }
+      for (; s < ns; s += 16) {
+        const float4 v = *reinterpret_cast<const float4*>(r + (int64_t)s * stride);
+        a.x += v.x; a.y += v.y; a.z += v.z; a.w += v.w;
+        if (s + 8 < ns) {
+          const float4 u = *reinterpret_cast<const float4*>(r + (int64_t)(s + 8) * stride);
+          a2.x += u.x; a2.y += u.y; a2.z += u.z; a2.w += u.w;
+        }
+      }
+    } else {
+      for (int s = sl; s < ns; s += 8) {
+        const float* r = p + (int64_t)s * stride + c;
+        float4& t = (s & 8) ? a2 : a;
+        t.x += r[0];
+        if (c + 1 < cols) t.y += r[1];
+        if (c + 2 < cols) t.z += r[2];
+        if (c + 3 < cols) t.w += r[3];
+      }
+    }
+  } else if (c < cols) {
     if (vec) {
       const float* r = p + c;
       int s = sl;
@@ -143,12 +174,19 @@
     }
   }
   red[sl][q] = a;
+  if (l16) red[sl + 8][q] = a2;
   __syncthreads();
   if (sl == 0 && c < cols) {
     float t[4] = {0.f, 0.f, 0.f, 0.f};
 #pragma unroll
     for (int r = 0; r < 8; ++r) {
       t[0] += red[r][q].x; t[1] += red[r][q].y; t[2] += red[r][q].z; t[3] += red[r][q].w;
+    }
+    if (l16) {
+#pragma unroll
+      for (int r = 8; r < 16; ++r) {
+        t[0] += red[r][q].x; t[1] += red[r][q].y; t[2] += red[r][q].z; t[3] += red[r][q].w;
+      }
     }
     fold_store(J, j, c, cols, t);
   }
@@ -229,7 +267,8 @@
       J.part[i] = b.part; J.out[i] = b.out; J.cols[i] = b.cols; J.stride[i] = b.stride; J.alpha[i] = b.alpha;
       J.nslots[i] = b.nslots;
       const bool wide = b.nslots <= 16;
-      J.flags[i] = (unsigned char)((b.accumulate ? 1 : 0) | (b.out_dtype == OFA_F32 ? 2 : 0) | (wide ? 4 : 0) | (b.out_dtype == OFA_F16 ? 8 : 0));
+      J.flags[i] = (unsigned char)(((b.accumulate & ~OFA_FOLD_LANES16) ? 1 : 0) | (b.out_dtype == OFA_F32 ? 2 : 0) | (wide ? 4 : 0) |
+                                   (b.out_dtype == OFA_F16 ? 8 : 0) | ((b.accumulate & OFA_FOLD_LANES16) ? 16 : 0));
       J.block0[i] = blocks;
       blocks += (unsigned)(wide ? (b.cols + 1023) / 1024 : (b.cols + 127) / 128);
     }
diff --git a/ofasys_amd/kernels.py b/ofasys_amd/kernels.py
--- a/ofasys_amd/kernels.py
+++ b/ofasys_amd/kernels.py
@@ -58,6 +58,7 @@
 
 
 DEFER_FOLD = 2
+FOLD_LANES16 = 4
 GEMM_DEFER_REDUCE = 128
 
 
@@ -68,13 +69,13 @@
     def __init__(self):
         self.jobs, self.keep, self.bytes, self.outs, self.want_flush = [], [], 0, set(), False
 
-    def add(self, part, part_off, out, cols, stride, nslots, alpha=1.0, accumulate=True, flush_ok=True):
+    def add(self, part, part_off, out, cols, stride, nslots, alpha=1.0, accumulate=True, flush_ok=True, lanes16=False):
         assert part.dtype == torch.float32 and out.is_contiguous()
         if out.data_ptr() in self.outs:
             self.flush()
         self.outs.add(out.data_ptr())
-        self.jobs.append(_FoldJob(dptr(part) + part_off * 4, dptr(out), cols, stride, nslots, int(accumulate),
-                                  float(alpha), dtype_code(out)))
+        self.jobs.append(_FoldJob(dptr(part) + part_off * 4, dptr(out), cols, stride, nslots,
+                                  int(bool(accumulate)) | (FOLD_LANES16 if lanes16 else 0), float(alpha), dtype_code(out)))
         self.keep.append((part, out))
         self.bytes += nslots * stride * 4
         self.want_flush = self.bytes > self.MAX_PENDING_BYTES
@@ -94,10 +95,10 @@
 
 class ImmediateFold:
 
-    def add(self, part, part_off, out, cols, stride, nslots, alpha=1.0, accumulate=True, flush_ok=True):
+    def add(self, part, part_off, out, cols, stride, nslots, alpha=1.0, accumulate=True, flush_ok=True, lanes16=False):
         assert part.dtype == torch.float32 and out.is_contiguous()
-        job = (_FoldJob * 1)(_FoldJob(dptr(part) + part_off * 4, dptr(out), cols, stride, nslots, int(accumulate), float(alpha),
-                                      dtype_code(out)))
+        job = (_FoldJob * 1)(_FoldJob(dptr(part) + part_off * 4, dptr(out), cols, stride, nslots,
+                                      int(bool(accumulate)) | (FOLD_LANES16 if lanes16 else 0), float(alpha), dtype_code(out)))
         lib().call("ofa_fold_batched", ctypes.addressof(job), 1, stream())
 
     def flush_if_large(self):
@@ -752,17 +753,44 @@
     return out
 
 
-def embedding_bwd(dout, ids, V, padding_idx=-1, dweight=None):
+EDGE_POS_RANGE, EDGE_TOKEN_BWD, EDGE_COLSUM_FOLD, EDGE_IM2COL = 0, 1, 2, 3
+
+
+def edge_old(item):
+    return bool(lib().cdll.ofa_step_edges_old(int(item)))
+
+
+def embedding_bwd(dout, ids, V, padding_idx=-1, dweight=None, id_major=None):
     dout = dout.contiguous()
     ids = ids.contiguous()
     D = dout.shape[-1]
     if dweight is None:
         dweight = torch.zeros(V, D, dtype=dout.dtype, device=dout.device)
+    S = lib().cdll.ofa_embedding_bwd_slices(V, D)
+    pad = -1 if padding_idx is None else padding_idx
+    if id_major is None:
+        id_major = S == 1 and not edge_old(EDGE_TOKEN_BWD)
+    if (id_major and lib().cdll.ofa_embedding_bwd_ids_ok(ids.numel(), D, V, dtype_code(dout))
+            and (dout.data_ptr() | dweight.data_ptr()) % 16 == 0):
+        lib().call("ofa_embedding_bwd_ids", ptr(dout), ptr(ids), ptr(dweight), ids.numel(), D, V, pad, S, dtype_code(dout), stream())
+        return dweight
     present = workspace(V, dout.device, "embed_present") if V > 4096 else None
-    S = lib().cdll.ofa_embedding_bwd_slices(V, D)
     slices = workspace(S * V * D * 4, dout.device, "embed_slices") if S > 1 else None
     lib().call("ofa_embedding_bwd", ptr(dout), ptr(ids), ptr(dweight), ids.numel(), D, V,
-               -1 if padding_idx is None else padding_idx, ptr(present), ptr(slices), dtype_code(dout), stream())
+               pad, ptr(present), ptr(slices), dtype_code(dout), stream())
+    return dweight
+
+
+def embedding_range_ok(x):
+    return x.shape[-1] % (4 if x.dtype == torch.float32 else 8) == 0 and not edge_old(EDGE_POS_RANGE)
+
+
+def embedding_range_bwd(dout, dweight, r0, T):
+    dout = dout.contiguous()
+    V, D = dweight.shape
+    batch = dout.numel() // (T * D)
+    assert dweight.is_contiguous() and dweight.dtype == dout.dtype and batch * T * D == dout.numel()
+    lib().call("ofa_embedding_range_bwd", ptr(dout), ptr(dweight), batch, T, D, V, int(r0), dtype_code(dout), stream())
     return dweight
 
 
@@ -882,7 +910,7 @@
                dtype_code(grad), stream())
 
 
-def colsum(x, alpha=1.0, out=None, accumulate=False, out_dtype=torch.float32, fold=None):
+def colsum(x, alpha=1.0, out=None, accumulate=False, out_dtype=torch.float32, fold=None, same_bits=False):
     if x.stride(-1) != 1:
         x = x.contiguous()
     rows, cols = x.shape
@@ -892,7 +920,7 @@
     if fold is not None and out.is_contiguous():
         ns = lib().cdll.ofa_colsum_slots(rows)
         ws = torch.empty(ns * cols, dtype=torch.float32, device=x.device)
-        fold.add(ws, 0, out, cols, cols, ns, alpha, accumulate)
+        fold.add(ws, 0, out, cols, cols, ns, alpha, accumulate, lanes16=same_bits)
         lib().call("ofa_colsum", ptr(x), ptr(out), ptr(ws), rows, cols, x.stride(0), float(alpha), DEFER_FOLD,
                    dtype_code(x), dtype_code(out), stream())
         fold.flush_if_large()
diff --git a/ofasys_amd/module/layers.py b/ofasys_amd/module/layers.py
--- a/ofasys_amd/module/layers.py
+++ b/ofasys_amd/module/layers.py
@@ -31,8 +31,8 @@
 
 
 class OfaEmbedding(nn.Embedding):
-    def forward(self, ids):
-        return ops.embedding(ids, self.weight, self.padding_idx)
+    def forward(self, ids, range_start=None):
+        return ops.embedding(ids, self.weight, self.padding_idx, range_start=range_start)
 
 
 def Embedding(num_embeddings, embedding_dim, padding_idx=None, zero_init=False):
diff --git a/ofasys_amd/ops.py b/ofasys_amd/ops.py
--- a/ofasys_amd/ops.py
+++ b/ofasys_amd/ops.py
@@ -116,6 +116,10 @@
         except RuntimeError:
             return None
     return q
+
+
+def _edge_fold():
+    return None if K.edge_old(K.EDGE_COLSUM_FOLD) else _fold()
 
 
 class _Wgrads:
@@ -480,12 +484,13 @@
 class AddFn(torch.autograd.Function):
 
     @staticmethod
-    def forward(ctx, a, b, vec, rowmask, vec_param=None):
+    def forward(ctx, a, b, vec, rowmask, vec_param=None, b_range=None):
         ctx.save_for_backward(rowmask)
         ctx.has = (b is not None, vec is not None)
         ctx.vdtype = vec.dtype if vec is not None else None
         ctx.b_shape = tuple(b.shape) if (b is not None and b.numel() != a.numel()) else None
         ctx.vec_param = vec_param
+        ctx.b_range = b_range
         return K.add_rowvec_mask(a, b, vec, rowmask)
 
     @staticmethod
@@ -496,12 +501,16 @@
         if ctx.has[1]:
             gv = _sink(ctx.vec_param)
             if gv is not None and gv.is_contiguous():
-                K.colsum(g, out=gv.view(-1), accumulate=True)
+                K.colsum(g, out=gv.view(-1), accumulate=True, fold=_edge_fold(), same_bits=True)
                 _sink_done(ctx.vec_param)
             else:
                 dvec = K.colsum(g, out_dtype=ctx.vdtype)
         db = None
-        if ctx.has[0]:
+        if ctx.b_range is not None:
+            table, r0 = ctx.b_range
+            K.embedding_range_bwd(g, _sink(table), r0, ctx.b_shape[0])
+            _sink_done(table)
+        elif ctx.has[0]:
             if ctx.b_shape is None:
                 db = g
             else:
@@ -509,7 +518,7 @@
                 for d in ctx.b_shape:
                     nb *= d
                 db = K.batch_sum(g, g.numel() // nb).view(ctx.b_shape)
-        return g, db, dvec, None, None
+        return g, db, dvec, None, None, None
 
 
 def dropout_add(x, residual, p, training):
@@ -543,6 +552,16 @@
     return base if base is not None else x[:1]
 
 
+def _range_sink(b):
+    rng = getattr(b, "_ofa_range", None)
+    if rng is None or not b.requires_grad or not b.is_contiguous():
+        return None
+    gw = _sink(rng[0])
+    if gw is None or not gw.is_contiguous() or gw.dtype != b.dtype or not K.embedding_range_ok(b):
+        return None
+    return rng
+
+
 def add_rowvec_mask(a, b=None, vec=None, rowmask=None, vec_param=None):
     if vec_param is not None and not (vec is not None and vec.requires_grad and torch.is_grad_enabled() and _sink(vec_param) is not None):
         vec_param = None
@@ -554,7 +573,10 @@
             b = base
         if b.shape[0] == 1 and a.dim() == 3 and a.shape[0] > 1 and a.is_contiguous() and tuple(a.shape[1:]) == tuple(b.shape[1:]):
             m = rowmask.reshape(-1) if rowmask is not None else None
-            return AddFn.apply(a.view(-1, a.shape[-1]), b.reshape(-1, b.shape[-1]), vec, m, vec_param).view(a.shape)
+            b_range = _range_sink(b) if (a.requires_grad and torch.is_grad_enabled()) else None
+            if b_range is not None:
+                b = b.detach()
+            return AddFn.apply(a.view(-1, a.shape[-1]), b.reshape(-1, b.shape[-1]), vec, m, vec_param, b_range).view(a.shape)
         b = like_layout(b, a)
     a2d, restore = rows_view(a)
     b2d = rows_view(b)[0] if b is not None else None
@@ -670,12 +692,14 @@
 
 class EmbeddingFn(torch.autograd.Function):
     @staticmethod
-    def forward(ctx, ids, weight, padding_idx, plan_key=None, pad_mask_of=None):
+    def forward(ctx, ids, weight, padding_idx, plan_key=None, pad_mask_of=None, range_start=None):
         ctx.save_for_backward(ids)
         ctx.V, ctx.padding_idx = weight.shape[0], padding_idx
         ctx.weight_ref = weight
         ctx.plan_key = plan_key
+        ctx.range_start = range_start
         ctx.with_mask = pad_mask_of is not None
+        ctx.set_materialize_grads(False)
         if pad_mask_of is None:
             return K.embedding_fwd(weight, ids)
         out, mask = K.embedding_fwd(weight, ids, pad_mask_of)
@@ -684,7 +708,9 @@
 
     @staticmethod
     def backward(ctx, dout, *_unused):
-        return EmbeddingFn._backward(ctx, dout) + (None,)
+        if dout is None:
+            return (None,) * 6
+        return EmbeddingFn._backward(ctx, dout) + (None, None)
 
     @staticmethod
     def _backward(ctx, dout):
@@ -692,6 +718,14 @@
         pad = -1 if ctx.padding_idx is None else ctx.padding_idx
         gw = _sink(ctx.weight_ref)
         D = dout.shape[-1]
+        if (ctx.range_start is not None and ctx.padding_idx is None and K.embedding_range_ok(dout)
+                and (gw is None or (gw.is_contiguous() and gw.dtype == dout.dtype))):
+            out = gw if gw is not None else torch.zeros(ctx.V, D, dtype=dout.dtype, device=dout.device)
+            K.embedding_range_bwd(dout.reshape(-1, D), out, ctx.range_start, ids.numel())
+            if gw is not None:
+                _sink_done(ctx.weight_ref)
+                return None, None, None, None
+            return None, out, None, None
         plan = None
         if ctx.plan_key is not None and D <= 64 and ctx.padding_idx is None:
             plan = SegmentPlan.get((ctx.plan_key, tuple(ids.shape), str(ids.device)), ids)
@@ -713,8 +747,13 @@
         return None, dw, None, None
 
 
-def embedding(ids, weight, padding_idx=None, plan_key=None):
-    return EmbeddingFn.apply(ids, weight, padding_idx, plan_key)
+def embedding(ids, weight, padding_idx=None, plan_key=None, range_start=None):
+    if range_start is None:
+        return EmbeddingFn.apply(ids, weight, padding_idx, plan_key)
+    out = EmbeddingFn.apply(ids, weight, padding_idx, plan_key, None, int(range_start))
+    if ids.dim() == 2 and ids.shape[0] == 1 and padding_idx is None:
+        out._ofa_range = (weight, int(range_start))
+    return out
 
 
 def embedding_with_pad_mask(ids, weight, padding_idx, pad):
@@ -1467,16 +1506,16 @@
         if cls is not None:
             gc = _sink(cls)
             if gc is not None:
-                K.colsum(first, out=gc.view(-1), accumulate=True)
+                K.colsum(first, out=gc.view(-1), accumulate=True, fold=_edge_fold(), same_bits=True)
                 _sink_done(cls)
             else:
                 dcls = K.colsum(first, out_dtype=dout.dtype).view(cls.shape)
         if bias is not None:
             gb = _sink(bias)
             if gb is not None:
-                K.colsum(d2, out=gb, accumulate=True)
+                K.colsum(d2, out=gb, accumulate=True, fold=_edge_fold(), same_bits=True)
                 if lead:
-                    K.colsum(first, alpha=-1.0, out=gb, accumulate=True)
+                    K.colsum(first, alpha=-1.0, out=gb, accumulate=True, fold=_edge_fold(), same_bits=True)
                 _sink_done(bias)
             else:
                 db = K.colsum(d2, out_dtype=dout.dtype)
```

After: 1.423 million (median of 6 runs). +1.7%, better.
